# shenyunhang/APE

Measured on AMD Instinct MI355X. Metric: images/sec @1024^2 APE-L_D fwd, higher is better.
Workload: dtype bf16

## Files before the change

### ape_amd/_lib.py

```python
import ctypes
import os
from ctypes import POINTER, Structure, c_char_p, c_double, c_float, c_int, c_int32, c_int64, c_void_p

_HERE = os.path.dirname(os.path.abspath(__file__))
LIB_PATH = os.path.join(_HERE, "lib", "libape_hip.so")

DT_F32 = 0
DT_BF16 = 1
DT_F16 = 2
ACT_NONE, ACT_RELU, ACT_GELU, ACT_SWIGLU, ACT_SILU = 0, 1, 2, 3, 4
MASK_NONE, MASK_ZERO_INPUT, MASK_ZERO_OUTPUT = 0, 1, 2


class GemmArgs(Structure):
    _fields_ = [
        ("A", c_void_p), ("W", c_void_p), ("C", c_void_p), ("bias", c_void_p), ("residual", c_void_p),
        ("rowmask", c_void_p), ("rope_cos", c_void_p), ("rope_sin", c_void_p),
        ("M", c_int32), ("N", c_int32), ("K", c_int32),
        ("lda", c_int32), ("ldw", c_int32), ("ldc", c_int32), ("ldr", c_int32),
        ("in_dt", c_int32), ("out_dt", c_int32), ("res_dt", c_int32),
        ("act", c_int32), ("mask_mode", c_int32), ("trans_out", c_int32),
        ("rope_rows", c_int32), ("rope_hd", c_int32), ("rope_cols", c_int32), ("vec_ok", c_int32),
        ("alpha", c_float), ("clamp", c_float),
        ("splitk", c_int32), ("tile64", c_int32), ("workspace", c_void_p),
        ("rowscale", c_void_p), ("rowshift", c_void_p), ("colvec", c_void_p), ("rope_cs", c_void_p),
        ("ln_w", c_void_p), ("ln_b", c_void_p), ("ln_eps", c_float), ("reserved0", c_int32),
        ("conv_perm", c_void_p), ("conv_zero", c_void_p), ("conv_h", c_int32), ("conv_w", c_int32),
        ("rowstat_cols", c_int32), ("rowstat_eps", c_float),
    ]


class LayerNormArgs(Structure):
    _fields_ = [
        ("x", c_void_p), ("w", c_void_p), ("b", c_void_p), ("y", c_void_p), ("add", c_void_p), ("y2", c_void_p),
        ("M", c_int32), ("C", c_int32), ("Cpad", c_int32),
        ("ldx", c_int32), ("ldy", c_int32), ("ldadd", c_int32), ("ldy2", c_int32),
        ("x_dt", c_int32), ("y_dt", c_int32), ("add_dt", c_int32), ("act", c_int32), ("eps", c_float),
    ]


class GroupNormArgs(Structure):
    _fields_ = [
        ("x", c_void_p), ("w", c_void_p), ("b", c_void_p), ("y", c_void_p), ("add", c_void_p), ("workspace", c_void_p),
        ("HW", c_int32), ("C", c_int32), ("G", c_int32),
        ("ldx", c_int32), ("ldy", c_int32), ("ldadd", c_int32),
        ("x_dt", c_int32), ("y_dt", c_int32), ("add_dt", c_int32), ("act", c_int32), ("eps", c_float),
    ]


SIGNATURES = {
    "ape_hip_last_error": (c_char_p, []),
    "ape_hip_abi_version": (c_int, []),
    "ape_hip_sizeof_args": (c_int, [c_int]),
    "ape_hip_gemm": (c_int, [POINTER(GemmArgs), c_void_p]),
    "ape_hip_gemm_last_kernel": (c_char_p, []),
    "ape_hip_meter_begin": (c_int, []),
    "ape_hip_meter_count": (c_int, []),
    "ape_hip_meter_end": (c_int, []),
    "ape_hip_meter_read": (c_int, [c_int, POINTER(c_char_p), POINTER(c_float)]),
    "ape_hip_zero": (c_int, [c_void_p, ctypes.c_size_t, c_void_p]),
    "ape_hip_stuff_collapse": (c_int, [c_void_p, c_int, c_int, c_int, c_int, c_void_p, c_int, c_void_p]),
    "ape_hip_sem_class_weights": (c_int, [c_void_p, c_int, c_void_p, c_void_p, c_int, c_int, c_int, c_float, c_void_p, c_int, c_int, c_void_p]),
    "ape_hip_pan_class_scores": (c_int, [c_void_p, c_int, c_void_p, c_void_p, c_int, c_int, c_float, c_int, c_float, c_void_p, c_void_p,
                                         c_void_p, c_void_p, c_void_p]),
    "ape_hip_argmax_labels": (c_int, [c_void_p, ctypes.c_size_t, c_int, ctypes.c_size_t, c_float, c_void_p, c_void_p]),
    "ape_hip_sdma_usable": (c_int, [c_void_p, c_void_p]),
    "ape_hip_sdma_d2h": (c_int, [c_void_p, c_void_p, ctypes.c_size_t]),
    "ape_hip_sdma_d2h_multi": (c_int, [c_int, ctypes.POINTER(c_void_p), ctypes.POINTER(c_void_p), ctypes.POINTER(ctypes.c_size_t), c_int]),
    "ape_hip_sdma_engines": (c_int, [c_void_p, c_void_p]),
    "ape_hip_row_stats": (c_int, [c_void_p, c_int, c_int, c_int, c_int, c_float, c_void_p, c_void_p, c_void_p]),
    "ape_hip_gemv": (c_int, [c_void_p, c_int, c_void_p, c_int, c_int, c_void_p, c_void_p, c_int, c_int, c_int, c_int,
                             c_float, c_void_p]),
    "ape_hip_gemv_affine": (c_int, [c_void_p, c_int, c_void_p, c_int, c_int, c_void_p, c_void_p, c_int, c_int, c_int, c_int,
                                    c_float, c_void_p, c_void_p, c_int, c_void_p, c_int, c_void_p]),
    "ape_hip_layernorm": (c_int, [POINTER(LayerNormArgs), c_void_p]),
    "ape_hip_postnorm_residual": (c_int, [c_void_p, c_int, c_int, c_void_p, c_void_p, c_float, c_void_p, c_int, c_void_p, c_int, c_int,
                                          c_int, c_int, c_void_p]),
    "ape_hip_groupnorm_workspace_floats": (c_int, [c_int, c_int]),
    "ape_hip_groupnorm": (c_int, [POINTER(GroupNormArgs), c_void_p]),
    "ape_hip_ms_deform_attn_forward": (c_int, [c_void_p, c_int, POINTER(c_int64), POINTER(c_int64), c_void_p, c_void_p,
                                               c_void_p, c_int, c_int, c_int, c_int, c_int, c_int, c_void_p]),
    "ape_hip_msda_fused": (c_int, [c_void_p, c_int, c_int, POINTER(c_int64), POINTER(c_int64), c_void_p, c_int, c_void_p,
                                   c_int, c_void_p, c_int, c_int, c_int, c_int, c_int, c_int, c_void_p]),
    "ape_hip_msda_fused_h": (c_int, [c_void_p, c_int, c_int, POINTER(c_int64), POINTER(c_int64), c_void_p, c_int, c_void_p,
                                     c_int, c_void_p, c_int, c_int, c_int, c_int, c_int, c_int, c_void_p]),
    "ape_hip_attention": (c_int, [c_void_p, c_int, c_void_p, c_int, c_void_p, c_int, c_void_p, c_int, c_int, c_int, c_int,
                                  c_int, c_float, c_int, c_void_p]),
    "ape_hip_geometry": (c_int, [c_int, c_int, c_int, c_int, POINTER(c_int), c_void_p, c_int, c_void_p, c_float, c_float, c_float,
                                 c_void_p, c_int, c_void_p, c_void_p, c_void_p, c_void_p, c_void_p, c_void_p, c_void_p, c_void_p,
                                 c_void_p]),
    "ape_hip_head_gemv": (c_int, [c_void_p, c_int, c_void_p, c_void_p, c_void_p, c_int, c_int, c_int, c_int, c_float, c_void_p, c_int,
                                  c_int, c_void_p]),
    "ape_hip_attention_strided": (c_int, [c_void_p, c_int, c_void_p, c_int, c_void_p, c_int, c_void_p, c_int, c_int, c_int, c_int,
                                          c_int, c_int, c_float, c_int, c_void_p]),
    "ape_hip_attention_causal": (c_int, [c_void_p, c_int, c_void_p, c_int, c_void_p, c_int, c_void_p, c_int, c_int, c_int, c_int,
                                         c_int, c_int, c_float, c_int, c_void_p]),
    "ape_hip_embed_tokens": (c_int, [c_void_p, c_int, c_void_p, c_int, c_void_p, c_int, c_int, c_void_p, c_int, c_int, c_int, c_int,
                                     c_int, c_int, c_void_p]),
    "ape_hip_patchify": (c_int, [c_void_p, c_int, c_int, c_void_p, c_int, c_int, POINTER(c_float), POINTER(c_float), c_void_p,
                                 c_int, c_int, c_void_p]),
    "ape_hip_im2col3x3": (c_int, [c_void_p, c_int, c_void_p, c_int, c_int, c_int, c_void_p, c_int, c_int, c_void_p]),
    "ape_hip_maxpool2x2": (c_int, [c_void_p, c_int, c_void_p, c_int, c_int, c_int, c_void_p, c_int, c_int, c_void_p]),
    "ape_hip_gather_rows": (c_int, [c_void_p, c_int, c_void_p, c_int, c_int, c_void_p, c_int, c_int, c_void_p]),
    "ape_hip_gather_rows_i64": (c_int, [c_void_p, c_int, c_void_p, c_int, c_int, c_void_p, c_int, c_int, c_void_p]),
    "ape_hip_nms_mask_words": (c_int, [c_int]),
    "ape_hip_nms_mask": (c_int, [c_void_p, c_void_p, c_int, c_float, c_void_p, c_void_p]),
    "ape_hip_nms_scan_segments": (c_int, [c_void_p, c_int, c_void_p, c_int, c_int, c_void_p, c_void_p, c_void_p]),
    "ape_hip_nms_scan_classes": (c_int, [c_void_p, c_int, c_void_p, c_int, c_void_p, c_void_p, c_void_p]),
    "ape_hip_vl_pool_workspace_floats": (c_int, [c_int, c_int]),
    "ape_hip_vl_pool": (c_int, [c_void_p, c_int, c_void_p, c_int, c_int, c_int, c_int, c_void_p, c_void_p, c_void_p, c_void_p]),
    "ape_hip_segment_softmax": (c_int, [c_void_p, c_int, c_int, c_int, c_int, c_void_p, c_void_p, c_int, c_int, c_void_p]),
    "ape_hip_colstats_workspace_floats": (c_int, [c_int, c_int]),
    "ape_hip_colstats": (c_int, [c_void_p, c_int, c_int, c_int, c_void_p, c_void_p, c_void_p, c_void_p, c_void_p]),
    "ape_hip_transpose": (c_int, [c_void_p, c_int, c_int, c_int, c_int, c_void_p, c_void_p, c_void_p, c_void_p, c_int, c_int,
                                  c_void_p]),
    "ape_hip_mask_upsample_bits": (c_int, [c_void_p, c_int, c_int, c_int, c_int, c_int, c_int, c_void_p, c_void_p]),
    "ape_hip_roi_align_bits": (c_int, [c_void_p, c_int, c_int, c_void_p, c_int, c_int, c_void_p, c_void_p]),
    "ape_hip_paste_bits": (c_int, [c_void_p, c_int, c_void_p, c_int, c_int, c_int, c_void_p, c_void_p]),
    "ape_hip_mask_upsample_sigmoid": (c_int, [c_void_p, c_int, c_int, c_int, c_int, c_int, c_int, c_int, c_int, c_void_p, c_int, c_int,
                                              c_void_p]),
    "ape_hip_box_refine": (c_int, [c_void_p, c_int, c_void_p, c_void_p, c_int, c_int, c_float, c_void_p, c_void_p, c_void_p]),
    "ape_hip_det_records": (c_int, [c_void_p, c_void_p, c_void_p, c_void_p, c_void_p, c_int, c_void_p, c_void_p, c_void_p, c_void_p]),
    "ape_hip_query_init": (c_int, [c_void_p, c_void_p, c_int, c_void_p, c_int, c_float, c_int, c_void_p, c_void_p, c_int, c_int, c_void_p,
                                   c_void_p]),
    "ape_hip_query_finish": (c_int, [c_void_p, c_int, c_void_p, c_int, c_int, c_int, c_void_p, c_void_p, c_float, c_void_p, c_void_p,
                                     c_float, c_void_p, c_void_p, c_void_p, c_int, c_int, c_void_p]),
    "ape_hip_bilinear_resize": (c_int, [c_void_p, c_int, c_int, c_int, c_int, c_int, c_void_p, c_int, c_int, c_void_p]),
    "ape_hip_panoptic_pixels": (c_int, [c_void_p, c_int, c_int, c_int, c_int, c_int, c_void_p, c_void_p, c_float, c_int, c_int, c_void_p, c_void_p,
                                        c_void_p, c_void_p]),
    "ape_hip_panoptic_decide": (c_int, [c_void_p, c_void_p, c_void_p, c_int, c_void_p, c_int, c_double, c_int, c_void_p, c_void_p, c_void_p, c_void_p]),
    "ape_hip_panoptic_write": (c_int, [c_void_p, c_void_p, c_void_p, c_int, c_int, c_void_p, c_void_p]),
    "ape_hip_enc_finalize": (c_int, [c_void_p, c_void_p, c_void_p, c_int, c_void_p, c_void_p, c_void_p, c_void_p]),
    "ape_hip_topk_workspace_words": (c_int, [c_int]),
    "ape_hip_proposal_topk": (c_int, [c_void_p, c_int, POINTER(c_int), POINTER(c_int), c_int, c_int, c_int, c_void_p, c_void_p, c_void_p,
                                      c_void_p]),
    "ape_hip_proposal_order": (c_int, [c_void_p, c_int, c_void_p, c_void_p, POINTER(c_int), POINTER(c_int), c_int, c_void_p, c_void_p,
                                       c_void_p, c_void_p, c_void_p, c_void_p, c_void_p]),
    "ape_hip_proposal_quota": (c_int, [c_void_p, c_void_p, c_void_p, c_void_p, c_int, c_void_p, c_int, POINTER(c_int), POINTER(c_int),
                                       c_int, c_int, c_void_p, c_void_p]),
    "ape_hip_det_sort": (c_int, [c_void_p, c_int, c_int, c_int, c_void_p, c_void_p, c_float, c_void_p, c_void_p, c_void_p, c_void_p,
                                 c_void_p, c_void_p]),
    "ape_hip_det_topk": (c_int, [c_void_p, c_void_p, c_void_p, c_void_p, c_int, c_int, c_int, c_void_p, c_void_p, c_void_p, c_void_p,
                                 c_void_p, c_void_p]),
    "ape_hip_ffn_fused": (c_int, [c_void_p, c_int, c_void_p, c_int, c_void_p, c_void_p, c_int, c_void_p, c_void_p, c_int, c_void_p, c_int,
                                  c_int, c_int, c_int, c_int, c_int, c_int, c_void_p, c_void_p, c_float, c_void_p]),
    "ape_hip_attention_ext": (c_int, [c_void_p, c_int, c_void_p, c_int, c_void_p, c_int, c_void_p, c_int, c_int, c_int, c_int, c_int, c_int,
                                      c_int, c_float, c_int, c_void_p]),
    "ape_hip_relpos_extend": (c_int, [c_void_p, c_void_p, c_int, c_void_p, c_int, c_int, c_void_p, c_void_p, c_int, c_void_p, c_void_p, c_int, c_int,
                                      c_int, c_int, c_int, c_int, c_int, c_int, c_float, c_int, c_void_p]),
    "ape_hip_resize_coeffs": (c_int, [c_int, c_int, c_void_p, c_void_p, c_int]),
    "ape_hip_resize_tile_rows": (c_int, [c_void_p, c_int, POINTER(c_int)]),
    "ape_hip_resize_bilinear_u8": (c_int, [c_void_p, c_int, c_int, c_int, c_void_p, c_void_p, c_int, c_void_p, c_void_p, c_int,
                                           c_int, c_int, c_int, c_int, c_void_p, c_int, c_int, c_int, c_int, c_void_p]),
    "ape_hip_rle_workspace_words": (c_int, [c_int, c_int, c_int, c_int]),
    "ape_hip_rle_encode": (c_int, [c_void_p, c_int, c_int, c_int, c_void_p, c_void_p, c_int, c_void_p, c_void_p]),
    "ape_hip_rle_to_string": (c_int, [c_void_p, c_int, c_void_p, c_int]),
}

_lib = None


def load():
    global _lib
    if _lib is not None:
        return _lib
    if not os.path.exists(LIB_PATH):
        raise RuntimeError(
            f"{LIB_PATH} not found: the HIP extension is not built (run `python -m ape_amd.build` or "
            "__graft_entry__.build()).  ape_amd has no CPU/PyTorch fallback."
        )
    lib = ctypes.CDLL(LIB_PATH)
    for name, (res, args) in SIGNATURES.items():
        fn = getattr(lib, name)
        fn.restype = res
        fn.argtypes = args
    _lib = lib
    return lib


def check(rc, what):
    if rc != 0:
        msg = load().ape_hip_last_error()
        raise RuntimeError(f"{what} failed (rc={rc}): {msg.decode() if msg else '?'}")
```

### ape_amd/csrc/boxes.hip

```cpp
#include "common.h"
#include "../../include/ape_hip.h"

__global__ __launch_bounds__(256) void box_refine_kernel(const float* __restrict__ delta, int ldd, const float* __restrict__ ref,
                                                         const float* __restrict__ vr4, int L, int Q, float eps,
                                                         float* __restrict__ new_ref, float* __restrict__ ref_in) {
  const int gid = blockIdx.x * 256 + threadIdx.x;
  if (gid >= Q * 4) return;
  const int q = gid >> 2, c = gid & 3;
  float x = ref[gid];
  x = fminf(fmaxf(x, 0.f), 1.f);
  const float x1 = fmaxf(x, eps), x2 = fmaxf(1.f - x, eps);
  float z = logf(x1 / x2);
  if (delta != nullptr) z += delta[(size_t)q * ldd + c];
  const float r = delta != nullptr ? 1.f / (1.f + expf(-z)) : ref[gid];
  if (new_ref != nullptr) new_ref[gid] = r;
  if (ref_in != nullptr)
    for (int l = 0; l < L; ++l) ref_in[((size_t)q * L + l) * 4 + c] = r * vr4[l * 4 + c];
}

extern "C" int ape_hip_box_refine(const float* delta, int ldd, const float* ref, const float* vr4, int L, int Q, float eps,
                                  float* new_ref, float* ref_in, void* stream) {
  APE_CHECK_ARG(ref && Q > 0 && (ref_in == nullptr || (vr4 != nullptr && L > 0)) && (new_ref || ref_in),
                "ape_hip_box_refine: bad args");
  APE_LAUNCH(box_refine_kernel, dim3(ceil_div(Q * 4, 256)), dim3(256), 0, (hipStream_t)stream, delta, ldd, ref, vr4, L, Q, eps,
                     new_ref, ref_in);
  APE_CHECK_LAUNCH("ape_hip_box_refine");
  return 0;
}

template <typename T> __device__ __forceinline__ float round_to(float v);
template <> __device__ __forceinline__ float round_to<float>(float v) { return v; }
template <> __device__ __forceinline__ float round_to<bf16_t>(float v) { return bf2f(f2bf(v)); }
template <> __device__ __forceinline__ float round_to<f16_t>(float v) { return (float)(f16_t)sat_h(v); }

template <typename TO>
__global__ __launch_bounds__(256) void query_init_kernel(const float* __restrict__ coords, const int64_t* __restrict__ topk, int T,
                                                         const float* __restrict__ dim_t, int P, float scale, int Q,
                                                         float* __restrict__ reference, TO* __restrict__ pe, int ldpe,
                                                         int32_t* __restrict__ topk32) {
  const int q = blockIdx.x;
  int64_t t = topk[q];
  t = t < 0 ? 0 : (t >= T ? T - 1 : t);
  if (threadIdx.x == 0 && topk32 != nullptr) topk32[q] = (int32_t)t;
  for (int j = threadIdx.x; j < 4 * P; j += 256) {
    const int c = j / P, i = j % P;
    const float x = coords[(size_t)t * 4 + c];
    const float s = 1.f / (1.f + expf(-x));
    if (i == 0) reference[q * 4 + c] = s;
    const float v = (s * scale) / dim_t[i];
    stf<TO>(pe + (size_t)q * ldpe + j, (i & 1) ? cosf(v) : sinf(v));
  }
}

extern "C" int ape_hip_query_init(const float* coords, const int64_t* topk, int T, const float* dim_t, int P, float scale, int Q,
                                  float* reference, void* pe, int ldpe, int pe_dt, int32_t* topk32, void* stream) {
  APE_CHECK_ARG(coords && topk && dim_t && reference && pe && T > 0 && P > 0 && Q > 0 && ldpe >= 4 * P, "ape_hip_query_init: bad args");
  hipStream_t s = (hipStream_t)stream;
  if (pe_dt == APE_DT_F16) APE_LAUNCH(query_init_kernel<f16_t>, dim3(Q), dim3(256), 0, s, coords, topk, T, dim_t, P, scale, Q, reference, (f16_t*)pe, ldpe, topk32);
  else if (pe_dt == APE_DT_BF16) APE_LAUNCH(query_init_kernel<bf16_t>, dim3(Q), dim3(256), 0, s, coords, topk, T, dim_t, P, scale, Q, reference, (bf16_t*)pe, ldpe, topk32);
  else if (pe_dt == APE_DT_F32)
    APE_LAUNCH(query_init_kernel<float>, dim3(Q), dim3(256), 0, s, coords, topk, T, dim_t, P, scale, Q, reference, (float*)pe, ldpe, topk32);
  else
    APE_CHECK_ARG(false, "ape_hip_query_init: pe must be f32, bf16 or f16");
  APE_CHECK_LAUNCH("ape_hip_query_init");
  return 0;
}

template <typename TO>
__global__ __launch_bounds__(256) void query_finish_kernel(const float* __restrict__ pos, int ldpos, const float* __restrict__ pix,
                                                           int ldpix, int Q, int E, const float* __restrict__ wpos,
                                                           const float* __restrict__ bpos, float eps_pos,
                                                           const float* __restrict__ wpix, const float* __restrict__ bpix,
                                                           float eps_pix, TO* __restrict__ query_pos, TO* __restrict__ query,
                                                           TO* __restrict__ query_sum, int ldo) {
  const int lane = threadIdx.x & 63;
  const int q = blockIdx.x * 4 + (threadIdx.x >> 6);
  if (q >= Q) return;
  constexpr int MAXP = 16, MAXX = 8;
  float vp[MAXP], vx[MAXX];
  const float* pr = pos + (size_t)q * ldpos;
  const float* xr = pix + (size_t)q * ldpix;
  float sp = 0.f, sx = 0.f;
#pragma unroll
  for (int k = 0; k < MAXP; ++k) { const int c = lane + 64 * k; vp[k] = c < 2 * E ? pr[c] : 0.f; sp += vp[k]; }
#pragma unroll
  for (int k = 0; k < MAXX; ++k) { const int c = lane + 64 * k; vx[k] = c < E ? xr[c] : 0.f; sx += vx[k]; }
  const float mp = wave_sum(sp) / (float)(2 * E), mx = wave_sum(sx) / (float)E;
  float qp = 0.f, qx = 0.f;
#pragma unroll
  for (int k = 0; k < MAXP; ++k) { const int c = lane + 64 * k; const float d = c < 2 * E ? vp[k] - mp : 0.f; qp += d * d; }
#pragma unroll
  for (int k = 0; k < MAXX; ++k) { const int c = lane + 64 * k; const float d = c < E ? vx[k] - mx : 0.f; qx += d * d; }
  const float rp = rsqrtf(wave_sum(qp) / (float)(2 * E) + eps_pos), rx = rsqrtf(wave_sum(qx) / (float)E + eps_pix);
  const int kE = E / 64;
#pragma unroll
  for (int k = 0; k < MAXX; ++k) {
    const int c = lane + 64 * k;
    if (c < E) {
      const float a = (vp[k] - mp) * rp * wpos[c] + bpos[c];
      float hi = 0.f;
#pragma unroll
      for (int kk = 0; kk < MAXP; ++kk) if (kk == k + kE) hi = (vp[kk] - mp) * rp * wpos[E + c] + bpos[E + c];
      const float b = hi + ((vx[k] - mx) * rx * wpix[c] + bpix[c]);
      const float ar = round_to<TO>(a), br = round_to<TO>(b);
      stf<TO>(query_pos + (size_t)q * ldo + c, ar);
      stf<TO>(query + (size_t)q * ldo + c, br);
      stf<TO>(query_sum + (size_t)q * ldo + c, ar + br);
    }
  }
}

extern "C" int ape_hip_query_finish(const float* pos, int ldpos, const float* pix, int ldpix, int Q, int E, const float* wpos,
                                    const float* bpos, float eps_pos, const float* wpix, const float* bpix, float eps_pix,
                                    void* query_pos, void* query, void* query_sum, int ldo, int out_dt, void* stream) {
  APE_CHECK_ARG(pos && pix && wpos && bpos && wpix && bpix && query_pos && query && query_sum && Q > 0, "ape_hip_query_finish: bad args");
  APE_CHECK_ARG(E > 0 && E <= 512 && E % 64 == 0 && ldpos >= 2 * E && ldpix >= E && ldo >= E, "ape_hip_query_finish: E must be a multiple of 64, <= 512");
  hipStream_t s = (hipStream_t)stream;
  const dim3 grid(ceil_div(Q, 4)), block(256);
  if (out_dt == APE_DT_F16) APE_LAUNCH(query_finish_kernel<f16_t>, grid, block, 0, s, pos, ldpos, pix, ldpix, Q, E, wpos, bpos, eps_pos, wpix, bpix, eps_pix,
                       (f16_t*)query_pos, (f16_t*)query, (f16_t*)query_sum, ldo);
  else if (out_dt == APE_DT_BF16) APE_LAUNCH(query_finish_kernel<bf16_t>, grid, block, 0, s, pos, ldpos, pix, ldpix, Q, E, wpos, bpos, eps_pos, wpix, bpix, eps_pix,
                       (bf16_t*)query_pos, (bf16_t*)query, (bf16_t*)query_sum, ldo);
  else if (out_dt == APE_DT_F32)
    APE_LAUNCH(query_finish_kernel<float>, grid, block, 0, s, pos, ldpos, pix, ldpix, Q, E, wpos, bpos, eps_pos, wpix, bpix, eps_pix,
                       (float*)query_pos, (float*)query, (float*)query_sum, ldo);
  else
    APE_CHECK_ARG(false, "ape_hip_query_finish: outputs must be f32, bf16 or f16");
  APE_CHECK_LAUNCH("ape_hip_query_finish");
  return 0;
}

__global__ __launch_bounds__(1024) void det_records_kernel(const float* __restrict__ boxes, const float* __restrict__ scores,
                                                            const int64_t* __restrict__ classes, const int64_t* __restrict__ query,
                                                            const float* __restrict__ frame, int k, float* __restrict__ rec,
                                                            float* __restrict__ boxes_out, int32_t* __restrict__ order) {
  __shared__ int wtot[16];
  __shared__ int total_keep;
  const int tid = threadIdx.x, lane = tid & 63, wave = tid >> 6;
  float f[8];
#pragma unroll
  for (int i = 0; i < 8; ++i) f[i] = frame[i];
  int cnt = 0;
  for (int i = tid; i < k; i += 1024) {
    float b[4];
#pragma unroll
    for (int c = 0; c < 4; ++c) b[c] = fminf(fmaxf(boxes[i * 4 + c] * f[c], 0.f), f[4 + c]);
    cnt += (scores[i] >= 0.f && (b[2] - b[0]) > 0.f && (b[3] - b[1]) > 0.f) ? 1 : 0;
  }
  cnt = (int)wave_sum((float)cnt);
  if (lane == 0) wtot[wave] = cnt;
  __syncthreads();
  if (tid == 0) { int s = 0; for (int w = 0; w < 16; ++w) s += wtot[w]; total_keep = s; }
  __syncthreads();
  int kbase = 0, dbase = total_keep;
  for (int i0 = 0; i0 < k; i0 += 1024) {
    const int i = i0 + tid;
    const bool in = i < k;
    float b[4] = {0.f, 0.f, 0.f, 0.f};
    bool keep = false;
    float sc = -1.f;
    if (in) {
#pragma unroll
      for (int c = 0; c < 4; ++c) b[c] = fminf(fmaxf(boxes[i * 4 + c] * f[c], 0.f), f[4 + c]);
      sc = scores[i];
      keep = sc >= 0.f && (b[2] - b[0]) > 0.f && (b[3] - b[1]) > 0.f;
    }
    const unsigned long long m = __ballot(keep);
    const int before = __popcll(m & ((1ull << lane) - 1ull));
    __syncthreads();
    if (lane == 0) wtot[wave] = __popcll(m);
    __syncthreads();
    int wbase = 0, chunk_keep = 0;
    for (int w = 0; w < 16; ++w) { const int t = wtot[w]; if (w < wave) wbase += t; chunk_keep += t; }
    if (in) {
      const int kept_before = wbase + before;
      const int pos = keep ? kbase + kept_before : dbase + (tid - kept_before);
      float* r = rec + (size_t)pos * 8;
      r[0] = b[0]; r[1] = b[1]; r[2] = b[2]; r[3] = b[3];
      r[4] = keep ? sc : -1.f;
      r[5] = (float)classes[i];
      r[6] = (float)query[i];
      r[7] = keep ? 1.f : 0.f;
      float* bo = boxes_out + (size_t)pos * 4;
      bo[0] = b[0]; bo[1] = b[1]; bo[2] = b[2]; bo[3] = b[3];
      order[pos] = i;
    }
    const int nin = min(1024, k - i0);
    kbase += chunk_keep;
    dbase += nin - chunk_keep;
  }
}

extern "C" int ape_hip_det_records(const float* boxes, const float* scores, const int64_t* classes, const int64_t* query,
                                   const float* frame, int k, float* rec, float* boxes_out, int32_t* order, void* stream) {
  APE_CHECK_ARG(boxes && scores && classes && query && frame && rec && boxes_out && order && k > 0, "ape_hip_det_records: bad args");
  APE_LAUNCH(det_records_kernel, dim3(1), dim3(1024), 0, (hipStream_t)stream, boxes, scores, classes, query, frame, k, rec,
                     boxes_out, order);
  APE_CHECK_LAUNCH("ape_hip_det_records");
  return 0;
}
```

### ape_amd/csrc/common.h

```cpp
#pragma once
#include <hip/hip_runtime.h>
#include <stdint.h>
#include <stdio.h>
#include <string.h>

typedef uint16_t bf16_t;

typedef __attribute__((ext_vector_type(8))) __bf16 bf16x8_t;
typedef __attribute__((ext_vector_type(8))) short short8_t;
typedef __attribute__((ext_vector_type(4))) float f32x4_t;

#define APE_DT_F32 0
#define APE_DT_BF16 1
#define APE_DT_F16 2
typedef _Float16 f16_t;

__device__ __forceinline__ float bf2f(bf16_t v) { return __uint_as_float(((uint32_t)v) << 16); }
typedef __attribute__((ext_vector_type(2))) float f32x2_t;
typedef __attribute__((ext_vector_type(2))) __bf16 bf16x2_t;
__device__ __forceinline__ uint32_t pack2bf(float a, float b) {
  const f32x2_t v = {a, b};
  return __builtin_bit_cast(uint32_t, __builtin_convertvector(v, bf16x2_t));
}
__device__ __forceinline__ bf16_t f2bf(float f) { return (bf16_t)(pack2bf(f, 0.f) & 0xffffu); }

template <typename T> __device__ __forceinline__ float ldf(const T* p);
template <> __device__ __forceinline__ float ldf<float>(const float* p) { return *p; }
template <> __device__ __forceinline__ float ldf<bf16_t>(const bf16_t* p) { return bf2f(*p); }
template <typename T> __device__ __forceinline__ void stf(T* p, float v);
template <> __device__ __forceinline__ void stf<float>(float* p, float v) { *p = v; }
template <> __device__ __forceinline__ void stf<bf16_t>(bf16_t* p, float v) { *p = f2bf(v); }

template <> __device__ __forceinline__ float ldf<f16_t>(const f16_t* p) { return (float)*p; }
#define APE_HALF_MAX 65504.f
__device__ __forceinline__ float sat_h(float v) { return __builtin_amdgcn_fmed3f(v, -APE_HALF_MAX, APE_HALF_MAX); }
template <> __device__ __forceinline__ void stf<f16_t>(f16_t* p, float v) { *p = (f16_t)sat_h(v); }

template <typename T> __device__ __forceinline__ void ld4(const T* p, float v[4]);
template <> __device__ __forceinline__ void ld4<float>(const float* p, float v[4]) {
  float4 t = *reinterpret_cast<const float4*>(p); v[0] = t.x; v[1] = t.y; v[2] = t.z; v[3] = t.w;
}
template <> __device__ __forceinline__ void ld4<bf16_t>(const bf16_t* p, float v[4]) {
  uint2 t = *reinterpret_cast<const uint2*>(p);
  v[0] = __uint_as_float(t.x << 16); v[1] = __uint_as_float(t.x & 0xffff0000u);
  v[2] = __uint_as_float(t.y << 16); v[3] = __uint_as_float(t.y & 0xffff0000u);
}
template <typename T> __device__ __forceinline__ void st4(T* p, const float v[4]);
template <> __device__ __forceinline__ void st4<float>(float* p, const float v[4]) {
  *reinterpret_cast<float4*>(p) = make_float4(v[0], v[1], v[2], v[3]);
}
template <> __device__ __forceinline__ void st4<bf16_t>(bf16_t* p, const float v[4]) {
  *reinterpret_cast<uint2*>(p) = make_uint2(pack2bf(v[0], v[1]), pack2bf(v[2], v[3]));
}
template <typename T> __device__ __forceinline__ void ld8(const T* p, float v[8]);
template <> __device__ __forceinline__ void ld8<float>(const float* p, float v[8]) {
  ld4<float>(p, v); ld4<float>(p + 4, v + 4);
}
template <> __device__ __forceinline__ void ld8<bf16_t>(const bf16_t* p, float v[8]) {
  uint4 t = *reinterpret_cast<const uint4*>(p);
  v[0] = __uint_as_float(t.x << 16); v[1] = __uint_as_float(t.x & 0xffff0000u);
  v[2] = __uint_as_float(t.y << 16); v[3] = __uint_as_float(t.y & 0xffff0000u);
  v[4] = __uint_as_float(t.z << 16); v[5] = __uint_as_float(t.z & 0xffff0000u);
  v[6] = __uint_as_float(t.w << 16); v[7] = __uint_as_float(t.w & 0xffff0000u);
}
typedef __attribute__((ext_vector_type(8))) _Float16 f16x8_t;
template <> __device__ __forceinline__ void ld8<f16_t>(const f16_t* p, float v[8]) {
  const f16x8_t t = *reinterpret_cast<const f16x8_t*>(p);
#pragma unroll
  for (int i = 0; i < 8; ++i) v[i] = (float)t[i];
}
template <typename T> __device__ __forceinline__ void st8(T* p, const float v[8]);
template <> __device__ __forceinline__ void st8<float>(float* p, const float v[8]) {
  st4<float>(p, v); st4<float>(p + 4, v + 4);
}
template <> __device__ __forceinline__ void st8<bf16_t>(bf16_t* p, const float v[8]) {
  *reinterpret_cast<uint4*>(p) = make_uint4(pack2bf(v[0], v[1]), pack2bf(v[2], v[3]),
                                            pack2bf(v[4], v[5]), pack2bf(v[6], v[7]));
}

typedef __attribute__((ext_vector_type(2))) _Float16 f16x2_t;
__device__ __forceinline__ uint32_t pack2h(float a, float b) {
  const f32x2_t v = {sat_h(a), sat_h(b)};
  return __builtin_bit_cast(uint32_t, __builtin_convertvector(v, f16x2_t));
}
template <> __device__ __forceinline__ void ld4<f16_t>(const f16_t* p, float v[4]) {
  const uint2 t = *reinterpret_cast<const uint2*>(p);
  const f16x2_t a = __builtin_bit_cast(f16x2_t, t.x), b = __builtin_bit_cast(f16x2_t, t.y);
  v[0] = (float)a[0]; v[1] = (float)a[1]; v[2] = (float)b[0]; v[3] = (float)b[1];
}
template <> __device__ __forceinline__ void st4<f16_t>(f16_t* p, const float v[4]) {
  *reinterpret_cast<uint2*>(p) = make_uint2(pack2h(v[0], v[1]), pack2h(v[2], v[3]));
}
template <> __device__ __forceinline__ void st8<f16_t>(f16_t* p, const float v[8]) {
  *reinterpret_cast<uint4*>(p) = make_uint4(pack2h(v[0], v[1]), pack2h(v[2], v[3]), pack2h(v[4], v[5]), pack2h(v[6], v[7]));
}

template <typename H> struct h16;
template <> struct h16<bf16_t> {
  static constexpr int dt = APE_DT_BF16;
  static __device__ __forceinline__ uint32_t pack2(float a, float b) { return pack2bf(a, b); }
  static __device__ __forceinline__ f32x4_t mfma(bf16x8_t a, bf16x8_t b, f32x4_t c) {
    return __builtin_amdgcn_mfma_f32_16x16x32_bf16(a, b, c, 0, 0, 0);
  }
};
template <> struct h16<f16_t> {
  static constexpr int dt = APE_DT_F16;
  static __device__ __forceinline__ uint32_t pack2(float a, float b) { return pack2h(a, b); }
  static __device__ __forceinline__ f32x4_t mfma(bf16x8_t a, bf16x8_t b, f32x4_t c) {
    return __builtin_amdgcn_mfma_f32_16x16x32_f16(__builtin_bit_cast(f16x8_t, a), __builtin_bit_cast(f16x8_t, b), c, 0, 0, 0);
  }
};
template <typename H> __device__ __forceinline__ float dot2acc(uint32_t a, uint32_t b, float c);
typedef __attribute__((ext_vector_type(2))) __bf16 bf16x2_t;
template <> __device__ __forceinline__ float dot2acc<bf16_t>(uint32_t a, uint32_t b, float c) {
  return __builtin_amdgcn_fdot2_f32_bf16(__builtin_bit_cast(bf16x2_t, a), __builtin_bit_cast(bf16x2_t, b), c, false);
}
template <> __device__ __forceinline__ float dot2acc<f16_t>(uint32_t a, uint32_t b, float c) {
  return __builtin_amdgcn_fdot2(__builtin_bit_cast(f16x2_t, a), __builtin_bit_cast(f16x2_t, b), c, false);
}
template <typename H> __device__ __forceinline__ void dot2acc_pinned(float& acc, uint32_t a, uint32_t b);
template <> __device__ __forceinline__ void dot2acc_pinned<bf16_t>(float& acc, uint32_t a, uint32_t b) {
  asm volatile("v_dot2c_f32_bf16 %0, %1, %2" : "+v"(acc) : "v"(a), "v"(b));
}
template <> __device__ __forceinline__ void dot2acc_pinned<f16_t>(float& acc, uint32_t a, uint32_t b) {
  asm volatile("v_dot2c_f32_f16 %0, %1, %2" : "+v"(acc) : "v"(a), "v"(b));
}
template <typename H> struct ones2;
template <> struct ones2<bf16_t> { static constexpr uint32_t v = 0x3f803f80u; };
template <> struct ones2<f16_t> { static constexpr uint32_t v = 0x3c003c00u; };
template <typename H> __device__ __forceinline__ void unpack2(uint32_t u, float& a, float& b);
template <> __device__ __forceinline__ void unpack2<bf16_t>(uint32_t u, float& a, float& b) {
  a = __uint_as_float(u << 16); b = __uint_as_float(u & 0xffff0000u);
}
template <> __device__ __forceinline__ void unpack2<f16_t>(uint32_t u, float& a, float& b) {
  const f16x2_t t = __builtin_bit_cast(f16x2_t, u);
  a = (float)t[0]; b = (float)t[1];
}

__device__ __forceinline__ float wave_sum(float v) {
#pragma unroll
  for (int o = 32; o > 0; o >>= 1) v += __shfl_xor(v, o, 64);
  return v;
}
__device__ __forceinline__ float wave_max(float v) {
#pragma unroll
  for (int o = 32; o > 0; o >>= 1) v = fmaxf(v, __shfl_xor(v, o, 64));
  return v;
}

extern "C" const char* ape_hip_last_error(void);
void ape_set_error(const char* fmt, ...);

#include <hip/hip_ext.h>
hipEvent_t* ape_meter_pair(const char* kernel, hipStream_t stream);
#define APE_LAUNCH(KERNEL, GRID, BLOCK, LDS, STREAM, ...)                                                                  \
  do {                                                                                                                     \
    hipEvent_t* ev__ = ape_meter_pair(#KERNEL, STREAM);                                                                           \
    if (ev__ != nullptr) hipExtLaunchKernelGGL(KERNEL, GRID, BLOCK, LDS, STREAM, ev__[0], ev__[1], 0, __VA_ARGS__);        \
    else hipLaunchKernelGGL(KERNEL, GRID, BLOCK, LDS, STREAM, __VA_ARGS__);                                                \
  } while (0)

#define APE_CHECK_ARG(cond, ...)            \
  do {                                      \
    if (!(cond)) {                          \
      ape_set_error(__VA_ARGS__);           \
      return -1;                            \
    }                                       \
  } while (0)
#define APE_CHECK_LAUNCH(name)                                                    \
  do {                                                                            \
    hipError_t e__ = hipGetLastError();                                           \
    if (e__ != hipSuccess) {                                                      \
      ape_set_error("%s: launch failed: %s", name, hipGetErrorString(e__));       \
      return -2;                                                                  \
    }                                                                             \
  } while (0)

static inline int ceil_div(int a, int b) { return (a + b - 1) / b; }
constexpr int APE_MAX_DEVICES = 64;
static inline int ape_current_device() {
  int d = 0;
  if (hipGetDevice(&d) != hipSuccess || d < 0 || d >= APE_MAX_DEVICES) d = 0;
  return d;
}
struct ApeOncePerDevice {
  bool done[APE_MAX_DEVICES] = {};
  bool first() { const int d = ape_current_device(); const bool f = !done[d]; done[d] = true; return f; }
};
static inline int ape_cu_count() {
  static int n[APE_MAX_DEVICES] = {};
  const int d = ape_current_device();
  if (n[d] == 0) {
    int c = 0;
    if (hipDeviceGetAttribute(&c, hipDeviceAttributeMultiprocessorCount, d) != hipSuccess || c < 8) c = 256;
    n[d] = c & ~7;
  }
  return n[d];
}
static inline bool ape_is16(int dt) { return dt == APE_DT_BF16 || dt == APE_DT_F16; }
static inline int ape_h16_kind(const int* dts, int n) {
  int k = 0;
  for (int i = 0; i < n; ++i) {
    const int d = dts[i];
    if (d == APE_DT_F32) continue;
    if (!ape_is16(d)) return -1;
    if (k != 0 && k != d) return -1;
    k = d;
  }
  return k;
}
#define APE_H16_KIND(...) ([&]() { const int d__[] = {__VA_ARGS__}; return ape_h16_kind(d__, (int)(sizeof(d__) / sizeof(int))); }())
```

### ape_amd/csrc/msda.hip

```cpp
#include <type_traits>

#include "common.h"
#include "../../include/ape_hip.h"

#define MS_HEADS 8
#define MS_D 32
#define MS_P 4

struct MsdaParams {
  const void* value; int ldv;
  const void* loc;
  const void* attn;
  const void* offw; int ldoffw;
  int offw_f16;
  const float* ref; int refdim;
  void* out; int ldout;
  int S, Q;
  int H[8], W[8], start[8];
  float invW[8], invH[8];
  int pow2;
};

template <typename TV>
__device__ __forceinline__ void corner_acc(const TV* __restrict__ vbase, int ldv, int idx, float wgt, float acc[8]) {
  float v[8];
  ld8<TV>(vbase + (size_t)idx * ldv, v);
#pragma unroll
  for (int c = 0; c < 8; ++c) acc[c] = fmaf(wgt, v[c], acc[c]);
}

template <typename TV>
__device__ __forceinline__ void sample_acc(const TV* __restrict__ vlvl, int ldv, int H, int W, float lx, float ly,
                                           float aw, float acc[8]) {
  const float h_im = ly * (float)H - 0.5f;
  const float w_im = lx * (float)W - 0.5f;
  if (!(h_im > -1.f && w_im > -1.f && h_im < (float)H && w_im < (float)W)) return;
  const float hf = floorf(h_im), wf = floorf(w_im);
  const int h_low = (int)hf, w_low = (int)wf;
  const int h_high = h_low + 1, w_high = w_low + 1;
  const float lh = h_im - hf, lw = w_im - wf;
  const float hh = 1.f - lh, hw = 1.f - lw;
  if (h_low >= 0 && w_low >= 0) corner_acc<TV>(vlvl, ldv, h_low * W + w_low, aw * hh * hw, acc);
  if (h_low >= 0 && w_high <= W - 1) corner_acc<TV>(vlvl, ldv, h_low * W + w_high, aw * hh * lw, acc);
  if (h_high <= H - 1 && w_low >= 0) corner_acc<TV>(vlvl, ldv, h_high * W + w_low, aw * lh * hw, acc);
  if (h_high <= H - 1 && w_high <= W - 1) corner_acc<TV>(vlvl, ldv, h_high * W + w_high, aw * lh * lw, acc);
}

template <typename TV, typename TO, int L, bool FUSED>
__global__ __launch_bounds__(256) void msda_kernel(const MsdaParams p) {
  const int lane = threadIdx.x & 63;
  const int wave = threadIdx.x >> 6;
  int chunk;
  {
    const int nblk = gridDim.x, b = blockIdx.x;
    const int q = nblk >> 3, r = nblk & 7;
    const int xcd = b & 7, j = b >> 3;
    chunk = (xcd < r ? xcd * (q + 1) : r * (q + 1) + (xcd - r) * q) + j;
  }
  const int batch = blockIdx.y;
  const int g = lane >> 2, sub = lane & 3;
  const int qi = chunk * 8 + wave * 2 + (g >> 3);
  const int h = g & 7;
  if (qi >= p.Q) return;
  const size_t qg = (size_t)batch * p.Q + qi;
  const TV* vb = reinterpret_cast<const TV*>(p.value) + (size_t)batch * p.S * p.ldv + h * MS_D + sub * 8;

  float acc[8];
#pragma unroll
  for (int c = 0; c < 8; ++c) acc[c] = 0.f;

  constexpr int LP = L * MS_P;
  if (FUSED) {
    const float* lg = reinterpret_cast<const float*>(p.offw) + qg * p.ldoffw + MS_HEADS * LP * 2 + h * LP;
    float w[LP];
    float mx = -INFINITY;
#pragma unroll
    for (int s = 0; s < LP; s += 4) {
      const float4 t = *reinterpret_cast<const float4*>(lg + s);
      w[s] = t.x; w[s + 1] = t.y; w[s + 2] = t.z; w[s + 3] = t.w;
      mx = fmaxf(mx, fmaxf(fmaxf(t.x, t.y), fmaxf(t.z, t.w)));
    }
    float sum = 0.f;
#pragma unroll
    for (int s = 0; s < LP; ++s) { w[s] = expf(w[s] - mx); sum += w[s]; }
    const float inv = 1.f / sum;
    const float* of = reinterpret_cast<const float*>(p.offw) + qg * p.ldoffw + h * LP * 2;
    const float* rf = p.ref + qg * L * p.refdim;
#pragma unroll
    for (int l = 0; l < L; ++l) {
      const int H = p.H[l], W = p.W[l];
      const TV* vl = vb + (size_t)p.start[l] * p.ldv;
      const float4 o01 = *reinterpret_cast<const float4*>(of + l * 8);
      const float4 o23 = *reinterpret_cast<const float4*>(of + l * 8 + 4);
      const float ox[4] = {o01.x, o01.z, o23.x, o23.z};
      const float oy[4] = {o01.y, o01.w, o23.y, o23.w};
      const float rx = rf[l * p.refdim], ry = rf[l * p.refdim + 1];
      float sx, sy;
      if (p.refdim == 2) {
        sx = 1.f / (float)W; sy = 1.f / (float)H;
#pragma unroll
        for (int pt = 0; pt < MS_P; ++pt)
          sample_acc<TV>(vl, p.ldv, H, W, rx + ox[pt] / (float)W, ry + oy[pt] / (float)H, w[l * MS_P + pt] * inv, acc);
        (void)sx; (void)sy;
      } else {
        const float rw = rf[l * p.refdim + 2], rh = rf[l * p.refdim + 3];
#pragma unroll
        for (int pt = 0; pt < MS_P; ++pt)
          sample_acc<TV>(vl, p.ldv, H, W, rx + ox[pt] / (float)MS_P * rw * 0.5f, ry + oy[pt] / (float)MS_P * rh * 0.5f,
                         w[l * MS_P + pt] * inv, acc);
      }
    }
  } else {
    const TV* loc = reinterpret_cast<const TV*>(p.loc) + (qg * MS_HEADS + h) * LP * 2;
    const TV* aw = reinterpret_cast<const TV*>(p.attn) + (qg * MS_HEADS + h) * LP;
#pragma unroll
    for (int l = 0; l < L; ++l) {
      const int H = p.H[l], W = p.W[l];
      const TV* vl = vb + (size_t)p.start[l] * p.ldv;
#pragma unroll
      for (int pt = 0; pt < MS_P; ++pt) {
        const float lx = ldf<TV>(loc + (l * MS_P + pt) * 2), ly = ldf<TV>(loc + (l * MS_P + pt) * 2 + 1);
        sample_acc<TV>(vl, p.ldv, H, W, lx, ly, ldf<TV>(aw + l * MS_P + pt), acc);
      }
    }
  }
  TO* o = reinterpret_cast<TO*>(p.out) + qg * p.ldout + h * MS_D + sub * 8;
  st8<TO>(o, acc);
}

template <int P> __device__ __forceinline__ float quad_bcast_f(float v) {
  return __int_as_float(__builtin_amdgcn_mov_dpp(__float_as_int(v), P * 0x55, 0xf, 0xf, true));
}
template <int P> __device__ __forceinline__ int quad_bcast_i(int v) { return __builtin_amdgcn_mov_dpp(v, P * 0x55, 0xf, 0xf, true); }
__device__ __forceinline__ float quad_xor1(float v) { return __int_as_float(__builtin_amdgcn_mov_dpp(__float_as_int(v), 0xB1, 0xf, 0xf, true)); }
__device__ __forceinline__ float quad_xor2(float v) { return __int_as_float(__builtin_amdgcn_mov_dpp(__float_as_int(v), 0x4E, 0xf, 0xf, true)); }

__device__ __forceinline__ float quad_pick_f(int P, float v) {
  return P == 0 ? quad_bcast_f<0>(v) : (P == 1 ? quad_bcast_f<1>(v) : (P == 2 ? quad_bcast_f<2>(v) : quad_bcast_f<3>(v)));
}
__device__ __forceinline__ int quad_pick_i(int P, int v) {
  return P == 0 ? quad_bcast_i<0>(v) : (P == 1 ? quad_bcast_i<1>(v) : (P == 2 ? quad_bcast_i<2>(v) : quad_bcast_i<3>(v)));
}

template <typename TV>
struct CornerGroup {
  uint4 raw[4];
  float w[4];
};

template <typename TV, int L>
__device__ __forceinline__ void group_load(const unsigned char* __restrict__ vbase, uint32_t lane_off, const float (&cw)[L][4],
                                           const int (&ci)[L][4], int s, CornerGroup<TV>& g) {
  const int l = s >> 2, P = s & 3;
#pragma unroll
  for (int c = 0; c < 4; ++c) {
    g.w[c] = quad_pick_f(P, cw[l][c]);
    uint32_t off = (uint32_t)quad_pick_i(P, ci[l][c]) + lane_off;
    asm volatile("" : "+v"(off));
    g.raw[c] = *reinterpret_cast<const uint4*>(vbase + (size_t)off);
  }
}

__device__ __forceinline__ void fma_mix_lo(float& acc, uint32_t d, float w) {
  asm volatile("v_fma_mix_f32 %0, %1, %2, %0 op_sel:[0,0,0] op_sel_hi:[1,0,0]" : "+v"(acc) : "v"(d), "v"(w));
}
__device__ __forceinline__ void fma_mix_hi(float& acc, uint32_t d, float w) {
  asm volatile("v_fma_mix_f32 %0, %1, %2, %0 op_sel:[1,0,0] op_sel_hi:[1,0,0]" : "+v"(acc) : "v"(d), "v"(w));
}
template <typename TV>
__device__ __forceinline__ void group_fma_half(const CornerGroup<TV>& g, float (&acc)[8]) {
#pragma unroll
  for (int c = 0; c < 4; ++c) {
    const uint32_t d[4] = {g.raw[c].x, g.raw[c].y, g.raw[c].z, g.raw[c].w};
#pragma unroll
    for (int e = 0; e < 4; ++e) {
      fma_mix_lo(acc[2 * e], d[e], g.w[c]);
      fma_mix_hi(acc[2 * e + 1], d[e], g.w[c]);
    }
  }
}

template <typename TV>
__device__ __forceinline__ void group_fma(const CornerGroup<TV>& g, f32x2_t (&a2)[4]) {
#pragma unroll
  for (int c = 0; c < 4; ++c) {
    const f32x2_t ww = {g.w[c], g.w[c]};
    const uint32_t d[4] = {g.raw[c].x, g.raw[c].y, g.raw[c].z, g.raw[c].w};
#pragma unroll
    for (int e = 0; e < 4; ++e) {
      const f32x2_t v2 = {__uint_as_float(d[e] << 16), __uint_as_float(d[e] & 0xffff0000u)};
      a2[e] = __builtin_elementwise_fma(ww, v2, a2[e]);
    }
  }
#pragma unroll
  for (int e = 0; e < 4; ++e) asm volatile("" : "+v"(a2[e]));
}

template <typename TV, typename TO, int L, typename TW = float>
__global__ __launch_bounds__(256) __attribute__((amdgpu_waves_per_eu(4, 8))) void msda_fused_quad_kernel(const MsdaParams p) {
  const int lane = threadIdx.x & 63;
  const int wave = threadIdx.x >> 6;
  int chunk;
  {
    const int nblk = gridDim.x, b = blockIdx.x;
    const int q = nblk >> 3, r = nblk & 7;
    const int xcd = b & 7, j = b >> 3;
    chunk = (xcd < r ? xcd * (q + 1) : r * (q + 1) + (xcd - r) * q) + j;
  }
  const int batch = blockIdx.y;
  const int g = lane >> 2, sub = lane & 3;
  int qi = chunk * 8 + wave * 2 + (g >> 3);
  const bool live = qi < p.Q;
  qi = live ? qi : p.Q - 1;
  const int h = g & 7;
  const size_t qg = (size_t)batch * p.Q + qi;
  const TV* vb = reinterpret_cast<const TV*>(p.value) + (size_t)batch * p.S * p.ldv + h * MS_D + sub * 8;
  const unsigned char* vbase = reinterpret_cast<const unsigned char*>(reinterpret_cast<const TV*>(p.value) + (size_t)batch * p.S * p.ldv);
  const uint32_t lane_off = (uint32_t)((h * MS_D + sub * 8) * sizeof(TV));
  const uint32_t rowb = (uint32_t)(p.ldv * (int)sizeof(TV));
  constexpr int LP = L * MS_P;

  const TW* lg = reinterpret_cast<const TW*>(p.offw) + qg * p.ldoffw + MS_HEADS * LP * 2 + h * LP;
  float wv[L];
  float mx = -INFINITY;
#pragma unroll
  for (int l = 0; l < L; ++l) { wv[l] = ldf<TW>(lg + l * MS_P + sub); mx = fmaxf(mx, wv[l]); }
  mx = fmaxf(mx, quad_xor1(mx));
  mx = fmaxf(mx, quad_xor2(mx));
  float sum = 0.f;
#pragma unroll
  for (int l = 0; l < L; ++l) { wv[l] = expf(wv[l] - mx); sum += wv[l]; }
  sum += quad_xor1(sum);
  sum += quad_xor2(sum);
  const float inv = 1.f / sum;
  const TW* of = reinterpret_cast<const TW*>(p.offw) + qg * p.ldoffw + h * LP * 2 + sub * 2;
  const float* rf = p.ref + qg * L * p.refdim;
  float cw[L][4];
  int ci[L][4];
#pragma unroll
  for (int l = 0; l < L; ++l) {
    const int H = p.H[l], W = p.W[l];
    float2 o;
    if (sizeof(TW) == 4) {
      o = *reinterpret_cast<const float2*>(of + l * 8);
    } else {
      typedef __attribute__((ext_vector_type(2))) _Float16 h2_t;
      const h2_t t = *reinterpret_cast<const h2_t*>(of + l * 8);
      o = make_float2((float)t[0], (float)t[1]);
    }
    const float rx = rf[l * p.refdim], ry = rf[l * p.refdim + 1];
    float lx, ly;
    if (p.refdim == 2) {
      if (p.pow2) { lx = rx + o.x * p.invW[l]; ly = ry + o.y * p.invH[l]; }
      else { lx = rx + o.x / (float)W; ly = ry + o.y / (float)H; }
    } else {
      const float rw = rf[l * p.refdim + 2], rh = rf[l * p.refdim + 3];
      lx = rx + o.x / (float)MS_P * rw * 0.5f; ly = ry + o.y / (float)MS_P * rh * 0.5f;
    }
    const float aw = wv[l] * inv;
    const float h_im = ly * (float)H - 0.5f, w_im = lx * (float)W - 0.5f;
    const bool inside = h_im > -1.f && w_im > -1.f && h_im < (float)H && w_im < (float)W;
    const float hf = floorf(h_im), wf = floorf(w_im);
    const int h_low = (int)hf, w_low = (int)wf;
    const int h_high = h_low + 1, w_high = w_low + 1;
    const float lh = h_im - hf, lw = w_im - wf;
    const float hh = 1.f - lh, hw = 1.f - lw;
    const bool t_ok = inside && h_low >= 0, b_ok = inside && h_high <= H - 1;
    const bool l_ok = w_low >= 0, r_ok = w_high <= W - 1;
    const int base = p.start[l];
    cw[l][0] = (t_ok && l_ok) ? aw * hh * hw : 0.f; ci[l][0] = (t_ok && l_ok) ? base + h_low * W + w_low : 0;
    cw[l][1] = (t_ok && r_ok) ? aw * hh * lw : 0.f; ci[l][1] = (t_ok && r_ok) ? base + h_low * W + w_high : 0;
    cw[l][2] = (b_ok && l_ok) ? aw * lh * hw : 0.f; ci[l][2] = (b_ok && l_ok) ? base + h_high * W + w_low : 0;
    cw[l][3] = (b_ok && r_ok) ? aw * lh * lw : 0.f; ci[l][3] = (b_ok && r_ok) ? base + h_high * W + w_high : 0;
    if (sizeof(TV) == 2) {
#pragma unroll
      for (int c = 0; c < 4; ++c) ci[l][c] = (int)__umul24((unsigned)ci[l][c], rowb);
    }
  }
  float acc[8];
  if (std::is_same<TV, f16_t>::value) {
#pragma unroll
    for (int c = 0; c < 8; ++c) acc[c] = 0.f;
    CornerGroup<TV> g0, g1;
    group_load<TV, L>(vbase, lane_off, cw, ci, 0, g0);
#pragma unroll
    for (int s = 0; s < L * 4; s += 2) {
      group_load<TV, L>(vbase, lane_off, cw, ci, s + 1, g1);
      __builtin_amdgcn_sched_barrier(0);
      group_fma_half<TV>(g0, acc);
      __builtin_amdgcn_sched_barrier(0);
      if (s + 2 < L * 4) group_load<TV, L>(vbase, lane_off, cw, ci, s + 2, g0);
      __builtin_amdgcn_sched_barrier(0);
      group_fma_half<TV>(g1, acc);
      __builtin_amdgcn_sched_barrier(0);
    }
  } else if (sizeof(TV) == 2) {
    f32x2_t a2[4];
#pragma unroll
    for (int e = 0; e < 4; ++e) a2[e] = (f32x2_t){0.f, 0.f};
    CornerGroup<TV> g0, g1;
    group_load<TV, L>(vbase, lane_off, cw, ci, 0, g0);
#pragma unroll
    for (int s = 0; s < L * 4; s += 2) {
      group_load<TV, L>(vbase, lane_off, cw, ci, s + 1, g1);
      __builtin_amdgcn_sched_barrier(0);
      group_fma<TV>(g0, a2);
      __builtin_amdgcn_sched_barrier(0);
      if (s + 2 < L * 4) group_load<TV, L>(vbase, lane_off, cw, ci, s + 2, g0);
      __builtin_amdgcn_sched_barrier(0);
      group_fma<TV>(g1, a2);
      __builtin_amdgcn_sched_barrier(0);
    }
#pragma unroll
    for (int e = 0; e < 4; ++e) { acc[2 * e] = a2[e][0]; acc[2 * e + 1] = a2[e][1]; }
  } else {
#pragma unroll
    for (int c = 0; c < 8; ++c) acc[c] = 0.f;
#pragma unroll
    for (int s = 0; s < L * 4; ++s) {
      const int l = s >> 2, P = s & 3;
#pragma unroll
      for (int c = 0; c < 4; ++c) {
        const float w = quad_pick_f(P, cw[l][c]);
        const int idx = quad_pick_i(P, ci[l][c]);
        if (w != 0.f) corner_acc<TV>(vb, p.ldv, idx, w, acc);
      }
    }
  }
  if (live) {
    TO* o = reinterpret_cast<TO*>(p.out) + qg * p.ldout + h * MS_D + sub * 8;
    st8<TO>(o, acc);
  }
}

constexpr int ML_T = 16;
constexpr int ML_HALO = 6;
constexpr int ML_RMAX = ML_T + 2 * ML_HALO + 2;
constexpr int ML_ROWS = ML_RMAX * ML_RMAX;

template <typename TO, typename TW, int L>
__global__ __launch_bounds__(256) void msda_lds_kernel(const MsdaParams p) {
  __shared__ uint4 sV[ML_ROWS * 4];
  const int t = threadIdx.x;
  const int h = blockIdx.x & 7;
  const int tile = blockIdx.x >> 3;
  const int batch = blockIdx.y;
  const int W0 = p.W[0];
  const int tiles_x = W0 / ML_T;
  const int ty = tile / tiles_x, tx = tile - ty * tiles_x;
  const int qi = p.start[0] + (ty * ML_T + (t >> 4)) * W0 + tx * ML_T + (t & 15);
  const size_t qg = (size_t)batch * p.Q + qi;
  const size_t q_first = (size_t)batch * p.Q + p.start[0] + (size_t)(ty * ML_T) * W0 + tx * ML_T;
  const size_t q_last = q_first + (size_t)(ML_T - 1) * W0 + (ML_T - 1);
  const uint32_t rowb = (uint32_t)p.ldv * 2u;
  const unsigned char* vhead = reinterpret_cast<const unsigned char*>(p.value) + (size_t)batch * p.S * rowb + h * (MS_D * 2);
  constexpr int LP = L * MS_P;

  float e[LP];
  {
    const TW* lg = reinterpret_cast<const TW*>(p.offw) + qg * p.ldoffw + MS_HEADS * LP * 2 + h * LP;
    float mx = -INFINITY;
#pragma unroll
    for (int i = 0; i < LP; ++i) { e[i] = ldf<TW>(lg + i); mx = fmaxf(mx, e[i]); }
    float sum = 0.f;
#pragma unroll
    for (int i = 0; i < LP; ++i) { e[i] = expf(e[i] - mx); sum += e[i]; }
    const float inv = 1.f / sum;
#pragma unroll
    for (int i = 0; i < LP; ++i) e[i] *= inv;
  }
  float acc[32];
#pragma unroll
  for (int c = 0; c < 32; ++c) acc[c] = 0.f;
  const TW* of = reinterpret_cast<const TW*>(p.offw) + qg * p.ldoffw + h * LP * 2;
  const float* rf = p.ref + qg * L * 2;
  const float* rfa = p.ref + q_first * L * 2;
  const float* rfb = p.ref + q_last * L * 2;

#pragma unroll 1
  for (int l = 0; l < L; ++l) {
    const int H = p.H[l], W = p.W[l];
    const float ax = rfa[l * 2] * (float)W - 0.5f, ay = rfa[l * 2 + 1] * (float)H - 0.5f;
    const float bx = rfb[l * 2] * (float)W - 0.5f, by = rfb[l * 2 + 1] * (float)H - 0.5f;
    int x_lo = max(0, (int)floorf(fminf(ax, bx)) - ML_HALO), x_hi = min(W - 1, (int)floorf(fmaxf(ax, bx)) + ML_HALO + 1);
    int y_lo = max(0, (int)floorf(fminf(ay, by)) - ML_HALO), y_hi = min(H - 1, (int)floorf(fmaxf(ay, by)) + ML_HALO + 1);
    x_lo = __builtin_amdgcn_readfirstlane(x_lo); x_hi = __builtin_amdgcn_readfirstlane(x_hi);
    y_lo = __builtin_amdgcn_readfirstlane(y_lo); y_hi = __builtin_amdgcn_readfirstlane(y_hi);
    const int rw = max(0, min(ML_RMAX, x_hi - x_lo + 1)), rh = max(0, min(ML_RMAX, y_hi - y_lo + 1));
    const unsigned char* vl = vhead + (size_t)p.start[l] * rowb;
    if (l > 0) __syncthreads();
    {
      const int n = rw * rh * 4;
      if (n == 0 && t < 4) sV[t] = make_uint4(0u, 0u, 0u, 0u);
      const float inv_rw = 1.f / (float)max(rw, 1);
      for (int i0 = 0; i0 < n; i0 += 1024) {
        uint4 v[4];
        int ii[4];
#pragma unroll
        for (int u = 0; u < 4; ++u) {
          const int i = i0 + u * 256 + t;
          ii[u] = i;
          if (i < n) {
            const int r = i >> 2, sl = i & 3;
            const int ry = (int)(((float)r + 0.5f) * inv_rw);
            const int rx = r - ry * rw;
            v[u] = *reinterpret_cast<const uint4*>(vl + (size_t)((y_lo + ry) * W + x_lo + rx) * rowb + ((sl ^ (rx & 3)) << 4));
          }
        }
#pragma unroll
        for (int u = 0; u < 4; ++u)
          if (ii[u] < n) sV[ii[u]] = v[u];
      }
    }
    __syncthreads();
    float off[8];
    if (sizeof(TW) == 4) {
      const float4 o0 = *reinterpret_cast<const float4*>(of + l * 8), o1 = *reinterpret_cast<const float4*>(of + l * 8 + 4);
      off[0] = o0.x; off[1] = o0.y; off[2] = o0.z; off[3] = o0.w; off[4] = o1.x; off[5] = o1.y; off[6] = o1.z; off[7] = o1.w;
    } else {
      typedef __attribute__((ext_vector_type(8))) _Float16 h8_t;
      const h8_t tq = *reinterpret_cast<const h8_t*>(of + l * 8);
#pragma unroll
      for (int u = 0; u < 8; ++u) off[u] = (float)tq[u];
    }
    const float rx0 = rf[l * 2], ry0 = rf[l * 2 + 1];
    float ew[MS_P];
#pragma unroll
    for (int pt = 0; pt < MS_P; ++pt) {
      ew[pt] = e[pt];
#pragma unroll
      for (int ll = 1; ll < L; ++ll) ew[pt] = (l == ll) ? e[ll * MS_P + pt] : ew[pt];
    }
#pragma unroll
    for (int pt = 0; pt < MS_P; ++pt) {
      float lx, ly;
      if (p.pow2) { lx = rx0 + off[2 * pt] * p.invW[l]; ly = ry0 + off[2 * pt + 1] * p.invH[l]; }
      else { lx = rx0 + off[2 * pt] / (float)W; ly = ry0 + off[2 * pt + 1] / (float)H; }
      const float aw = ew[pt];
      const float h_im = ly * (float)H - 0.5f, w_im = lx * (float)W - 0.5f;
      const bool inside = h_im > -1.f && w_im > -1.f && h_im < (float)H && w_im < (float)W;
      const float hf = floorf(h_im), wf = floorf(w_im);
      const int h_low = (int)hf, w_low = (int)wf;
      const float lh = h_im - hf, lw = w_im - wf;
      const float hh = 1.f - lh, hw = 1.f - lw;
#pragma unroll
      for (int c = 0; c < 4; ++c) {
        const int cy = h_low + (c >> 1), cx = w_low + (c & 1);
        const bool ok = inside && cy >= 0 && cy <= H - 1 && cx >= 0 && cx <= W - 1;
        const float wgt = ok ? aw * ((c >> 1) ? lh : hh) * ((c & 1) ? lw : hw) : 0.f;
        const int ry = cy - y_lo, rx = cx - x_lo;
        const bool staged = ok && ry >= 0 && ry < rh && rx >= 0 && rx < rw;
        const int row = staged ? ry * rw + rx : 0;
        const float wl = staged ? wgt : 0.f;
        const int sw = rx & 3;
#pragma unroll
        for (int k = 0; k < 4; ++k) {
          const uint4 d = sV[row * 4 + (k ^ sw)];
          fma_mix_lo(acc[8 * k + 0], d.x, wl); fma_mix_hi(acc[8 * k + 1], d.x, wl);
          fma_mix_lo(acc[8 * k + 2], d.y, wl); fma_mix_hi(acc[8 * k + 3], d.y, wl);
          fma_mix_lo(acc[8 * k + 4], d.z, wl); fma_mix_hi(acc[8 * k + 5], d.z, wl);
          fma_mix_lo(acc[8 * k + 6], d.w, wl); fma_mix_hi(acc[8 * k + 7], d.w, wl);
        }
        if (ok && !staged) {
          const unsigned char* g = vl + (size_t)(cy * W + cx) * rowb;
#pragma unroll
          for (int k = 0; k < 4; ++k) {
            const uint4 d = *reinterpret_cast<const uint4*>(g + (k << 4));
            fma_mix_lo(acc[8 * k + 0], d.x, wgt); fma_mix_hi(acc[8 * k + 1], d.x, wgt);
            fma_mix_lo(acc[8 * k + 2], d.y, wgt); fma_mix_hi(acc[8 * k + 3], d.y, wgt);
            fma_mix_lo(acc[8 * k + 4], d.z, wgt); fma_mix_hi(acc[8 * k + 5], d.z, wgt);
            fma_mix_lo(acc[8 * k + 6], d.w, wgt); fma_mix_hi(acc[8 * k + 7], d.w, wgt);
          }
        }
      }
    }
  }
  TO* o = reinterpret_cast<TO*>(p.out) + qg * p.ldout + h * MS_D;
#pragma unroll
  for (int k = 0; k < 4; ++k) st8<TO>(o + 8 * k, acc + 8 * k);
}

template <typename TV, typename TO, bool FUSED>
static int launch_msda(const MsdaParams& p, int B, int L, hipStream_t s) {
  const dim3 grid(ceil_div(p.Q, 8), B), block(256);
  if constexpr (FUSED) {
    if (p.offw_f16) {
      switch (L) {
        case 1: APE_LAUNCH((msda_fused_quad_kernel<TV, TO, 1, f16_t>), grid, block, 0, s, p); return 0;
        case 2: APE_LAUNCH((msda_fused_quad_kernel<TV, TO, 2, f16_t>), grid, block, 0, s, p); return 0;
        case 3: APE_LAUNCH((msda_fused_quad_kernel<TV, TO, 3, f16_t>), grid, block, 0, s, p); return 0;
        case 4: APE_LAUNCH((msda_fused_quad_kernel<TV, TO, 4, f16_t>), grid, block, 0, s, p); return 0;
        case 5: APE_LAUNCH((msda_fused_quad_kernel<TV, TO, 5, f16_t>), grid, block, 0, s, p); return 0;
        default: ape_set_error("msda: num_levels %d not in 1..5", L); return -1;
      }
    }
    switch (L) {
      case 1: APE_LAUNCH((msda_fused_quad_kernel<TV, TO, 1>), grid, block, 0, s, p); return 0;
      case 2: APE_LAUNCH((msda_fused_quad_kernel<TV, TO, 2>), grid, block, 0, s, p); return 0;
      case 3: APE_LAUNCH((msda_fused_quad_kernel<TV, TO, 3>), grid, block, 0, s, p); return 0;
      case 4: APE_LAUNCH((msda_fused_quad_kernel<TV, TO, 4>), grid, block, 0, s, p); return 0;
      case 5: APE_LAUNCH((msda_fused_quad_kernel<TV, TO, 5>), grid, block, 0, s, p); return 0;
      default: ape_set_error("msda: num_levels %d not in 1..5", L); return -1;
    }
  } else {
  switch (L) {
    case 1: APE_LAUNCH((msda_kernel<TV, TO, 1, FUSED>), grid, block, 0, s, p); break;
    case 2: APE_LAUNCH((msda_kernel<TV, TO, 2, FUSED>), grid, block, 0, s, p); break;
    case 3: APE_LAUNCH((msda_kernel<TV, TO, 3, FUSED>), grid, block, 0, s, p); break;
    case 4: APE_LAUNCH((msda_kernel<TV, TO, 4, FUSED>), grid, block, 0, s, p); break;
    case 5: APE_LAUNCH((msda_kernel<TV, TO, 5, FUSED>), grid, block, 0, s, p); break;
    default: ape_set_error("msda: num_levels %d not in 1..5", L); return -1;
  }
  }
  return 0;
}

static int fill_levels(MsdaParams& p, const int64_t* shapes, const int64_t* starts, int L, int S) {
  if (L < 1 || L > 5) { ape_set_error("msda: num_levels %d not in 1..5", L); return -1; }
  int64_t tot = 0;
  for (int l = 0; l < L; ++l) {
    p.H[l] = (int)shapes[2 * l]; p.W[l] = (int)shapes[2 * l + 1]; p.start[l] = (int)starts[l];
    if (p.H[l] <= 0 || p.W[l] <= 0 || starts[l] != tot) { ape_set_error("msda: inconsistent level %d (h=%d w=%d start=%lld)", l, p.H[l], p.W[l], (long long)starts[l]); return -1; }
    tot += (int64_t)p.H[l] * p.W[l];
  }
  if (tot != S) { ape_set_error("msda: sum(h*w)=%lld != num_value=%d", (long long)tot, S); return -1; }
  return 0;
}

extern "C" int ape_hip_ms_deform_attn_forward(const void* value, int ldv, const int64_t* spatial_shapes,
                                              const int64_t* level_start_index, const void* sampling_loc,
                                              const void* attn_weight, void* out, int ldout, int B, int S, int Q, int L,
                                              int dt, void* stream) {
  APE_CHECK_ARG(value && spatial_shapes && level_start_index && sampling_loc && attn_weight && out, "ms_deform_attn_forward: null pointer");
  APE_CHECK_ARG(B > 0 && S > 0 && Q > 0, "ms_deform_attn_forward: bad sizes");
  APE_CHECK_ARG(ldv % 8 == 0 && ldout % 8 == 0 && ((uintptr_t)value) % 16 == 0 && ((uintptr_t)out) % 16 == 0,
                "ms_deform_attn_forward: value/out must be 16-byte aligned with ld %% 8 == 0");
  MsdaParams p;
  memset(&p, 0, sizeof(p));
  p.value = value; p.ldv = ldv; p.loc = sampling_loc; p.attn = attn_weight; p.out = out; p.ldout = ldout; p.S = S; p.Q = Q;
  if (fill_levels(p, spatial_shapes, level_start_index, L, S)) return -1;
  int rc;
  APE_CHECK_ARG(dt == APE_DT_F32 || dt == APE_DT_BF16 || dt == APE_DT_F16, "ms_deform_attn_forward: dtype code %d (0 = f32, 1 = bf16, 2 = f16)", dt);
  if (dt == APE_DT_BF16) rc = launch_msda<bf16_t, bf16_t, false>(p, B, L, (hipStream_t)stream);
  else if (dt == APE_DT_F16) rc = launch_msda<f16_t, f16_t, false>(p, B, L, (hipStream_t)stream);
  else rc = launch_msda<float, float, false>(p, B, L, (hipStream_t)stream);
  if (rc) return rc;
  APE_CHECK_LAUNCH("ape_hip_ms_deform_attn_forward");
  return 0;
}

static int msda_fused_launch(const void* value, int ldv, int v_dt, const int64_t* spatial_shapes, const int64_t* level_start_index,
                             const void* offw, int ldoffw, int offw_f16, const float* ref, int refdim, void* out, int ldout, int out_dt,
                             int B, int S, int Q, int L, void* stream) {
  APE_CHECK_ARG(value && spatial_shapes && level_start_index && offw && ref && out, "msda_fused: null pointer");
  APE_CHECK_ARG(refdim == 2 || refdim == 4, "msda_fused: reference points must have 2 or 4 coordinates, got %d", refdim);
  APE_CHECK_ARG(B > 0 && S > 0 && Q > 0, "msda_fused: bad sizes");
  APE_CHECK_ARG(ldv % 8 == 0 && ldout % 8 == 0 && ldoffw % 4 == 0 && ((uintptr_t)value) % 16 == 0 &&
                    ((uintptr_t)out) % 16 == 0 && ((uintptr_t)offw) % 16 == 0,
                "msda_fused: alignment (value/out 16 B, ld %% 8; offw 16 B, ld %% 4)");
  MsdaParams p;
  memset(&p, 0, sizeof(p));
  p.value = value; p.ldv = ldv; p.offw = offw; p.ldoffw = ldoffw; p.offw_f16 = offw_f16; p.ref = ref; p.refdim = refdim;
  p.out = out; p.ldout = ldout; p.S = S; p.Q = Q;
  if (fill_levels(p, spatial_shapes, level_start_index, L, S)) return -1;
  APE_CHECK_ARG(v_dt == APE_DT_F32 || ((uint64_t)S * (uint64_t)ldv * 2 < (1ull << 32) && S < (1 << 24) && ldv * 2 < (1 << 24)),
                "msda_fused: a batch element's value tensor must stay below 4 GiB (S = %d rows of %d elements)", S, ldv);
  p.pow2 = 1;
  for (int l = 0; l < L; ++l) {
    p.pow2 &= ((p.W[l] & (p.W[l] - 1)) == 0 && (p.H[l] & (p.H[l] - 1)) == 0) ? 1 : 0;
    p.invW[l] = 1.f / (float)p.W[l]; p.invH[l] = 1.f / (float)p.H[l];
  }
  int rc;
  hipStream_t s = (hipStream_t)stream;
  {
    const char* le = getenv("APE_MSDA_LDS");
    const int n0 = p.H[0] * p.W[0];
    if ((le != nullptr && atoi(le) == 1) && L == 5 && refdim == 2 && Q == S && v_dt == APE_DT_F16 && p.start[0] == 0 && p.W[0] % ML_T == 0 &&
        p.H[0] % ML_T == 0 && n0 < Q && (out_dt == APE_DT_BF16 || out_dt == APE_DT_F16)) {
      const dim3 grid((p.H[0] / ML_T) * (p.W[0] / ML_T) * 8, B), block(256);
      if (out_dt == APE_DT_BF16) {
        if (offw_f16) APE_LAUNCH((msda_lds_kernel<bf16_t, f16_t, 5>), grid, block, 0, s, p);
        else APE_LAUNCH((msda_lds_kernel<bf16_t, float, 5>), grid, block, 0, s, p);
      } else {
        if (offw_f16) APE_LAUNCH((msda_lds_kernel<f16_t, f16_t, 5>), grid, block, 0, s, p);
        else APE_LAUNCH((msda_lds_kernel<f16_t, float, 5>), grid, block, 0, s, p);
      }
      APE_CHECK_LAUNCH("ape_hip_msda_fused (LDS-staged level-0 queries)");
      APE_CHECK_ARG(B == 1, "msda_fused: the LDS-staged encoder path takes one batch element per call");
      MsdaParams r = p;
      r.Q = Q - n0;
      r.offw = reinterpret_cast<const unsigned char*>(offw) + (size_t)n0 * ldoffw * (offw_f16 ? 2 : 4);
      r.ref = ref + (size_t)n0 * L * refdim;
      r.out = reinterpret_cast<unsigned char*>(out) + (size_t)n0 * ldout * 2;
      if (out_dt == APE_DT_BF16) rc = launch_msda<f16_t, bf16_t, true>(r, B, L, s);
      else rc = launch_msda<f16_t, f16_t, true>(r, B, L, s);
      if (rc) return rc;
      APE_CHECK_LAUNCH("ape_hip_msda_fused");
      return 0;
    }
  }
  if (v_dt == APE_DT_BF16 && out_dt == APE_DT_BF16) rc = launch_msda<bf16_t, bf16_t, true>(p, B, L, s);
  else if (v_dt == APE_DT_BF16 && out_dt == APE_DT_F32) rc = launch_msda<bf16_t, float, true>(p, B, L, s);
  else if (v_dt == APE_DT_F16 && out_dt == APE_DT_BF16) rc = launch_msda<f16_t, bf16_t, true>(p, B, L, s);
  else if (v_dt == APE_DT_F16 && out_dt == APE_DT_F32) rc = launch_msda<f16_t, float, true>(p, B, L, s);
  else if (v_dt == APE_DT_F16 && out_dt == APE_DT_F16) rc = launch_msda<f16_t, f16_t, true>(p, B, L, s);
  else if (v_dt == APE_DT_F32 && out_dt == APE_DT_F32) rc = launch_msda<float, float, true>(p, B, L, s);
  else { ape_set_error("msda_fused: unsupported dtype combination v=%d out=%d", v_dt, out_dt); return -1; }
  if (rc) return rc;
  APE_CHECK_LAUNCH("ape_hip_msda_fused");
  return 0;
}

extern "C" int ape_hip_msda_fused(const void* value, int ldv, int v_dt, const int64_t* spatial_shapes,
                                  const int64_t* level_start_index, const float* offw, int ldoffw, const float* ref,
                                  int refdim, void* out, int ldout, int out_dt, int B, int S, int Q, int L, void* stream) {
  return msda_fused_launch(value, ldv, v_dt, spatial_shapes, level_start_index, offw, ldoffw, 0, ref, refdim, out, ldout, out_dt, B, S, Q, L,
                           stream);
}

extern "C" int ape_hip_msda_fused_h(const void* value, int ldv, int v_dt, const int64_t* spatial_shapes,
                                    const int64_t* level_start_index, const void* offw_f16, int ldoffw, const float* ref,
                                    int refdim, void* out, int ldout, int out_dt, int B, int S, int Q, int L, void* stream) {
  APE_CHECK_ARG(v_dt == APE_DT_BF16 || v_dt == APE_DT_F16, "msda_fused_h: bf16 or f16 values (the production modes)");
  return msda_fused_launch(value, ldv, v_dt, spatial_shapes, level_start_index, offw_f16, ldoffw, 1, ref, refdim, out, ldout, out_dt, B, S, Q,
                           L, stream);
}
```

### ape_amd/modeling/ape_deta/_containers.py

```python
import os

import torch
import torch.nn as nn

from ... import ops
from ...packing import attach_cache, f32, pack_matrix, permute_ffn_w2


class FFN(nn.Module):
    def __init__(self, embed_dim=256, feedforward_dim=1024, output_dim=None, num_fcs=2, ffn_drop=0.0, **kwargs):
        super().__init__()
        assert num_fcs == 2
        output_dim = embed_dim if output_dim is None else output_dim
        self.layers = nn.Sequential(nn.Sequential(nn.Linear(embed_dim, feedforward_dim), nn.ReLU(inplace=True), nn.Dropout(ffn_drop)),
                                    nn.Linear(feedforward_dim, output_dim), nn.Dropout(ffn_drop))
        self.embed_dim = embed_dim
        attach_cache(self)

    def packed(self, dt):
        def build(dt):
            l0, l1 = self.layers[0][0], self.layers[1]
            d = dict(w1=pack_matrix(l0.weight, dt), b1=f32(l0.bias), w2=pack_matrix(l1.weight, dt), b2=f32(l1.bias))
            if dt in ops.HALF16 and l0.weight.shape[0] % 64 == 0:
                d["w2p"] = permute_ffn_w2(d["w2"])
            return d
        return self._pack.get(self, dt, build)

    FUSED_MIN_ROWS = 2048

    def forward_tokens(self, x, dt, out_dtype=None, norm=None):
        P = self.packed(dt)
        mode = os.environ.get("APE_FFN_FUSED", "1")
        if (mode != "0" and "w2p" in P and (out_dtype or dt) in ops.HALF16 and (out_dtype or dt) == dt and x.shape[0] >= self.FUSED_MIN_ROWS
                and x.shape[1] == 256 and P["w2"].shape[0] == 256 and P["w1"].shape[0] <= 4096):
            fuse_ln = norm if os.environ.get("APE_FFN_LN") != "0" else None
            if mode == "b64":
                y = ops.ffn_fused(x, P["w1"], P["b1"], P["w2"], P["b2"], residual=x, norm=fuse_ln)
            else:
                y = ops.ffn_fused(x, P["w1"], P["b1"], P["w2p"], P["b2"], residual=x, w2_permuted=True, norm=fuse_ln)
            return y if (norm is None or fuse_ln is not None) else ops.layernorm(y, norm[0], norm[1], norm[2], out_dtype=dt)
        h = ops.gemm(x, P["w1"], P["b1"], act=ops.ACT_RELU)
        y = ops.gemm(h, P["w2"], P["b2"], residual=x, out_dtype=out_dtype or dt)
        return y if norm is None else ops.layernorm(y, norm[0], norm[1], norm[2], out_dtype=dt)


class MLP(nn.Module):
    def __init__(self, input_dim, hidden_dim, output_dim, num_layers):
        super().__init__()
        self.num_layers = num_layers
        h = [hidden_dim] * (num_layers - 1)
        self.layers = nn.ModuleList(nn.Linear(n, k) for n, k in zip([input_dim] + h, h + [output_dim]))
        attach_cache(self)

    def packed(self, dt):
        def build(dt):
            return [(pack_matrix(l.weight, dt), f32(l.bias)) for l in self.layers]
        return self._pack.get(self, dt, build)

    def forward_tokens(self, x, dt, out_dtype=torch.float32):
        P = self.packed(dt)
        for i, (w, b) in enumerate(P):
            last = i == len(P) - 1
            x = ops.gemm(x, w, b, act=ops.ACT_NONE if last else ops.ACT_RELU, out_dtype=out_dtype if last else dt)
        return x


class SelfAttention(nn.Module):

    def __init__(self, embed_dim, num_heads, attn_drop=0.0, proj_drop=0.0, batch_first=False, **kwargs):
        super().__init__()
        self.embed_dim, self.num_heads, self.batch_first = embed_dim, num_heads, batch_first
        self.attn = nn.MultiheadAttention(embed_dim=embed_dim, num_heads=num_heads, dropout=attn_drop, batch_first=batch_first)
        self.proj_drop = nn.Dropout(proj_drop)
        attach_cache(self)

    def packed(self, dt):
        def build(dt):
            E = self.embed_dim
            w, b = self.attn.in_proj_weight, self.attn.in_proj_bias
            return dict(wqk=pack_matrix(w[:2 * E], dt), bqk=f32(b[:2 * E]), wv=pack_matrix(w[2 * E:], dt), bv=f32(b[2 * E:]),
                        wo=pack_matrix(self.attn.out_proj.weight, dt), bo=f32(self.attn.out_proj.bias))
        return self._pack.get(self, dt, build)

    def forward_tokens(self, x, x_pos, dt, vt_buf, out_dtype=None):
        P = self.packed(dt)
        E, nh = self.embed_dim, self.num_heads
        hd = E // nh
        vjob = ops.fork(lambda: ops.gemm(x, P["wv"], P["bv"], trans_out=True, out=vt_buf))
        qk = ops.gemm(x_pos, P["wqk"], P["bqk"])
        vt = vjob.join()
        o = ops.attention(qk[:, :E], qk[:, E:], vt, batch=1, n=x.shape[0], heads=nh, head_dim=hd, scale=hd ** -0.5)
        return ops.gemm(o, P["wo"], P["bo"], residual=x, out_dtype=out_dtype or dt)


class TransformerLayer(nn.Module):

    def __init__(self, attentions, ffn, num_norms, embed_dim=256):
        super().__init__()
        self.attentions = nn.ModuleList(attentions)
        self.ffns = nn.ModuleList([ffn])
        self.norms = nn.ModuleList([nn.LayerNorm(embed_dim) for _ in range(num_norms)])
        self.embed_dim = embed_dim
        self.pre_norm = False

    def norm_params(self, i):
        n = self.norms[i]
        return f32(n.weight), f32(n.bias), n.eps


class ConvNormAct(nn.Module):
    def __init__(self, in_channels, out_channels, kernel_size=1, bias=True, norm_layer=None):
        super().__init__()
        self.conv = nn.Conv2d(in_channels, out_channels, kernel_size=kernel_size, padding=(kernel_size - 1) // 2, bias=bias)
        self.norm = norm_layer


class ChannelMapper(nn.Module):

    def __init__(self, input_shapes, in_features, out_channels, kernel_size=1, stride=1, bias=True, groups=1, dilation=1,
                 norm_layer=None, activation=None, num_outs=None, **kwargs):
        super().__init__()
        import copy
        assert kernel_size == 1 and activation is None
        chans = [getattr(input_shapes[f], "channels", input_shapes[f]) for f in in_features]
        assert num_outs is None or num_outs == len(chans), "extra downsampling convs are not used by the APE configs"
        self.convs = nn.ModuleList(ConvNormAct(c, out_channels, 1, bias, copy.deepcopy(norm_layer)) for c in chans)
        self.in_features, self.out_channels, self.input_shapes = in_features, out_channels, input_shapes


class PositionEmbeddingSine(nn.Module):

    def __init__(self, num_pos_feats=64, temperature=10000, scale=2 * 3.141592653589793, eps=1e-6, offset=0.0, normalize=False):
        super().__init__()
        self.num_pos_feats, self.temperature, self.scale, self.eps, self.offset, self.normalize = (
            num_pos_feats, temperature, scale, eps, offset, normalize)
```

### ape_amd/modeling/ape_deta/deformable_transformer_vl.py

```python
import copy

import torch
import torch.nn as nn

from ... import ops
from ...layers import MultiScaleDeformableAttention
from ...packing import attach_cache, f32, pack_matrix, round_up
from ...stagetap import forcing, tap
from . import geometry as G
from ._containers import FFN, SelfAttention, TransformerLayer


class DeformableDetrTransformerEncoderVL(nn.Module):
    def __init__(self, embed_dim=256, num_heads=8, feedforward_dim=1024, attn_dropout=0.1, ffn_dropout=0.1, num_layers=6,
                 post_norm=False, num_feature_levels=4, vl_layer=None, use_act_checkpoint=False, pytorch_attn=False):
        super().__init__()
        self.layers = nn.ModuleList([
            TransformerLayer([MultiScaleDeformableAttention(embed_dim=embed_dim, num_heads=num_heads, dropout=attn_dropout,
                                                            batch_first=True, num_levels=num_feature_levels,
                                                            pytorch_attn=pytorch_attn)],
                             FFN(embed_dim=embed_dim, feedforward_dim=feedforward_dim, output_dim=embed_dim, num_fcs=2,
                                 ffn_drop=ffn_dropout), 2, embed_dim) for _ in range(num_layers)])
        self.num_layers = num_layers
        self.embed_dim = embed_dim
        self.pre_norm = False
        self.post_norm_layer = nn.LayerNorm(embed_dim) if post_norm else None
        self.vl_layers = nn.ModuleList([copy.deepcopy(vl_layer) for _ in range(num_layers)]) if vl_layer is not None else None
        self.use_checkpoint = use_act_checkpoint

    def forward_tokens(self, x, geo, lvl_pos, l, dt, stages=None):
        xp = None
        for i, layer in enumerate(self.layers):
            if self.vl_layers is None:
                v_new, qp, ljob = x, (xp if xp is not None else (x.float() + lvl_pos.float()).to(dt)), ops._Joined(l)
            else:
                v_new, qp, ljob = self.vl_layers[i].b_attn.forward_tokens(x, lvl_pos, l, dt, defer_language=True)
            x2 = layer.attentions[0].forward_tokens(qp, v_new, geo.enc_ref, geo.shapes, geo.starts, dt, value_src=v_new,
                                                    mask=geo.mask_u8, norm=layer.norm_params(0))
            x, xp = layer.ffns[0].forward_tokens(x2, dt, norm=layer.norm_params(1)), None
            l = ljob.join()
            if stages is not None:
                if self.vl_layers is not None:
                    stages[f"enc{i}_fused_v"] = v_new
                    l = tap(stages, f"enc{i}_fused_l", l)
                x = tap(stages, f"enc{i}_out", x)
        if self.post_norm_layer is not None:
            x = ops.layernorm(x, f32(self.post_norm_layer.weight), f32(self.post_norm_layer.bias), self.post_norm_layer.eps, out_dtype=dt)
        return x, l


class DeformableDetrTransformerDecoderVL(nn.Module):
    def __init__(self, embed_dim=256, num_heads=8, feedforward_dim=1024, attn_dropout=0.1, ffn_dropout=0.1, num_layers=6,
                 return_intermediate=True, num_feature_levels=4, use_act_checkpoint=False, look_forward_twice=False,
                 pytorch_attn=False):
        super().__init__()
        self.layers = nn.ModuleList([
            TransformerLayer([SelfAttention(embed_dim=embed_dim, num_heads=num_heads, attn_drop=attn_dropout, batch_first=True),
                              MultiScaleDeformableAttention(embed_dim=embed_dim, num_heads=num_heads, dropout=attn_dropout,
                                                            batch_first=True, num_levels=num_feature_levels,
                                                            pytorch_attn=pytorch_attn)],
                             FFN(embed_dim=embed_dim, feedforward_dim=feedforward_dim, output_dim=embed_dim, ffn_drop=ffn_dropout),
                             3, embed_dim) for _ in range(num_layers)])
        self.num_layers = num_layers
        self.embed_dim = embed_dim
        self.return_intermediate = return_intermediate
        self.bbox_embed = None
        self.class_embed = None
        self.use_checkpoint = use_act_checkpoint
        self.look_forward_twice = look_forward_twice
        attach_cache(self)

    def packed(self, dt):
        def build(dt):
            ws = [l.attentions[1].value_proj.weight for l in self.layers]
            bs = [l.attentions[1].value_proj.bias.detach().float() for l in self.layers]
            return dict(wval=pack_matrix(torch.cat(ws, 0), dt), bval=torch.cat(bs).contiguous())
        return self._pack.get(self, dt, build)

    def forward_tokens(self, query, query_pos, memory, geo, reference, dt, stages=None, query_sum=None):
        P = self.packed(dt)
        E = self.embed_dim
        from ...layers.multi_scale_deform_attn import half_value_kwargs
        value_all = ops.gemm(memory, P["wval"], P["bval"], rowmask=geo.mask_u8, mask_mode=ops.MASK_ZERO_OUTPUT,
                             **half_value_kwargs(dt, memory.shape[0]))
        Q = query.shape[0]
        vt_buf = ops.zeros((E, round_up(Q, 64)), dt, query.device)
        vr4 = geo.vr4
        out = query
        outp = query_sum if query_sum is not None else (query.float() + query_pos.float()).to(dt)
        inter, inter_ref = [], []
        _, ref_in = ops.box_refine(None, reference.contiguous(), vr4)
        refjob = ops._Joined((reference, ref_in))
        for i, layer in enumerate(self.layers):
            x1 = layer.attentions[0].forward_tokens(out, outp, dt, vt_buf)
            x2, x2p = ops.layernorm(x1, *layer.norm_params(0), out_dtype=dt, add=query_pos)
            reference, ref_in = refjob.join()
            if i > 0:
                if stages is not None:
                    forced = tap(stages, f"dec{i - 1}_ref", reference)
                    if forced is not reference:
                        reference = forced
                        _, ref_in = ops.box_refine(None, reference.contiguous(), vr4)
                inter_ref.append(reference)
            x3 = layer.attentions[1].forward_tokens(x2p, x2, ref_in, geo.shapes, geo.starts, dt,
                                                    value=value_all[:, i * E:(i + 1) * E])
            x4 = ops.layernorm(x3, *layer.norm_params(1), out_dtype=dt)
            x5 = layer.ffns[0].forward_tokens(x4, dt)
            out, outp = ops.layernorm(x5, *layer.norm_params(2), out_dtype=dt, add=query_pos)
            if stages is not None:
                forced = tap(stages, f"dec{i}_out", out)
                if forced is not out:
                    out, outp = forced, (forced.float() + query_pos.float()).to(dt)
            if self.bbox_embed is not None:
                def refine(i=i, out=out, reference=reference):
                    tmp = self.bbox_embed[i].forward_tokens(out, dt, out_dtype=torch.float32)
                    if stages is not None:
                        stages[f"dec{i}_delta"] = tmp
                    return ops.box_refine(tmp, reference, vr4)
                refjob = ops.fork(refine)
            inter.append(out)
        reference, _ = refjob.join()
        reference = tap(stages, f"dec{len(self.layers) - 1}_ref", reference)
        inter_ref.append(reference)
        return inter, inter_ref


class DeformableDetrTransformerVL(nn.Module):
    def __init__(self, encoder=None, decoder=None, num_feature_levels=4, as_two_stage=False, two_stage_num_proposals=300,
                 assign_first_stage=False, pre_nms_topk=1000, nms_thresh_enc=0.9, proposal_ambiguous=0):
        super().__init__()
        assert as_two_stage and assign_first_stage, "ape_amd implements the two-stage DETA selection used by every APE config"
        self.encoder, self.decoder = encoder, decoder
        self.num_feature_levels = num_feature_levels
        self.as_two_stage = as_two_stage
        self.two_stage_num_proposals = two_stage_num_proposals
        self.assign_first_stage = assign_first_stage
        self.pre_nms_topk, self.nms_thresh_enc = pre_nms_topk, nms_thresh_enc
        self.proposal_ambiguous = proposal_ambiguous
        self.compute_dtype = torch.bfloat16
        self.embed_dim = self.encoder.embed_dim
        self.level_embeds = nn.Parameter(torch.Tensor(self.num_feature_levels, self.embed_dim))
        self.enc_output = nn.Linear(self.embed_dim, self.embed_dim)
        self.enc_output_norm = nn.LayerNorm(self.embed_dim)
        self.pos_trans = nn.Linear(self.embed_dim * 2, self.embed_dim * 2)
        self.pos_trans_norm = nn.LayerNorm(self.embed_dim * 2)
        self.pix_trans = nn.Linear(self.embed_dim, self.embed_dim)
        self.pix_trans_norm = nn.LayerNorm(self.embed_dim)
        nn.init.normal_(self.level_embeds)
        attach_cache(self)

    def packed(self, dt):
        def build(dt):
            dec = self.decoder
            nd = dec.num_layers
            amb = bool(self.proposal_ambiguous)
            be, bea = dec.bbox_embed[nd], (dec.bbox_embed_ambiguous[0] if amb else dec.bbox_embed[nd])
            ce, cea = dec.class_embed[nd], (dec.class_embed_ambiguous[0] if amb else dec.class_embed[nd])
            return dict(
                wenc=pack_matrix(self.enc_output.weight, dt), benc=f32(self.enc_output.bias),
                nenc=(f32(self.enc_output_norm.weight), f32(self.enc_output_norm.bias), self.enc_output_norm.eps),
                wpos=pack_matrix(self.pos_trans.weight, dt), bpos=f32(self.pos_trans.bias),
                npos=(f32(self.pos_trans_norm.weight), f32(self.pos_trans_norm.bias), self.pos_trans_norm.eps),
                wpix=pack_matrix(self.pix_trans.weight, dt), bpix=f32(self.pix_trans.bias),
                npix=(f32(self.pix_trans_norm.weight), f32(self.pix_trans_norm.bias), self.pix_trans_norm.eps),
                w1=pack_matrix(torch.cat([be.layers[0].weight, bea.layers[0].weight], 0), dt),
                b1=torch.cat([be.layers[0].bias, bea.layers[0].bias]).detach().float().contiguous(),
                w2=(pack_matrix(be.layers[1].weight, dt), pack_matrix(bea.layers[1].weight, dt)),
                b2=(f32(be.layers[1].bias), f32(bea.layers[1].bias)),
                w3=(pack_matrix(be.layers[2].weight, dt), pack_matrix(bea.layers[2].weight, dt)),
                b3=(f32(be.layers[2].bias), f32(bea.layers[2].bias)),
                wcls=pack_matrix(torch.cat([ce.weight, cea.weight], 0), dt),
                bcls=torch.cat([ce.bias, cea.bias]).detach().float().contiguous(),
                level_embeds=f32(self.level_embeds))
        return self._pack.get(self, dt, build)

    def lvl_pos(self, geo, dt):
        key = (dt, self.level_embeds.data_ptr(), self.level_embeds._version)
        if key not in geo._lvl_pos:
            geo._lvl_pos.clear()
            geo._lvl_pos[key] = (geo.pos + self.level_embeds.detach().float()[geo.level_ids]).to(dt).contiguous()
        return geo._lvl_pos[key]

    def forward_tokens(self, src, geo, l, dt, forced_topk=None, stages=None, after_encoder=None, mask_prompt=None):
        P = self.packed(dt)
        lvl_pos = self.lvl_pos(geo, dt)
        memory, l_out = self.encoder.forward_tokens(src, geo, lvl_pos, l, dt, stages)
        memory = tap(stages, "memory", memory)
        if after_encoder is not None:
            after_encoder(memory)
        invalid, anchors = geo.invalid_u8, geo.proposals
        if mask_prompt is not None:
            outside = ~mask_prompt.reshape(-1).to(device=memory.device, dtype=torch.bool)
            invalid = (invalid.reshape(-1).bool() | outside).to(torch.uint8).reshape(invalid.shape).contiguous()
            anchors = anchors.masked_fill(outside[:, None], float("inf")).contiguous()
        om = ops.gemm(memory, P["wenc"], P["benc"], rowmask=invalid, mask_mode=ops.MASK_ZERO_INPUT)
        om = tap(stages, "output_memory", ops.layernorm(om, *P["nenc"], out_dtype=dt))
        E = self.embed_dim
        T = om.shape[0]
        h1 = ops.gemm(om, P["w1"], P["b1"], act=ops.ACT_RELU)
        h2 = torch.empty((T, 2 * E), dtype=dt, device=om.device)
        ops.gemm(h1[:, :E], P["w2"][0], P["b2"][0], act=ops.ACT_RELU, out=h2[:, :E])
        ops.gemm(h1[:, E:], P["w2"][1], P["b2"][1], act=ops.ACT_RELU, out=h2[:, E:])
        d = torch.empty((T, 8), dtype=torch.float32, device=om.device)
        ops.gemm(h2[:, :E], P["w3"][0], P["b3"][0], out=d[:, :4])
        ops.gemm(h2[:, E:], P["w3"][1], P["b3"][1], out=d[:, 4:])
        cls2 = ops.gemm(om, P["wcls"], P["bcls"], out_dtype=torch.float32)
        if stages is not None:
            cls2, d = tap(stages, "enc_cls2", cls2), tap(stages, "enc_delta8", d)
        enc_class, enc_coord, xyxy = ops.enc_finalize(cls2, d, anchors)
        if stages is not None:
            stages["query_l"] = l_out
            enc_class, enc_coord = tap(stages, "enc_class", enc_class), tap(stages, "enc_coord_unact", enc_coord)
        if forced_topk is not None:
            topk = forced_topk.to(om.device).long()
        else:
            topk = ops.select_proposals(enc_class, xyxy, geo.shapes, self.pre_nms_topk, self.two_stage_num_proposals,
                                        self.nms_thresh_enc)
        reference, pe, topk32 = ops.query_init(enc_coord, topk, G.dim_t_table(128, 10000, om.device), dt)
        pos_raw = ops.gemm(pe, P["wpos"], P["bpos"], out_dtype=torch.float32)
        pix_raw = ops.gemm(ops.gather_rows(om, topk32), P["wpix"], P["bpix"], out_dtype=torch.float32)
        query_pos, query, query_sum = ops.query_finish(pos_raw, pix_raw, P["npos"], P["npix"], dt)
        if stages is not None:
            stages["topk_proposals"] = topk
            q0, p0 = query, query_pos
            query, query_pos = tap(stages, "query_init", query), tap(stages, "query_pos", query_pos)
            if query is not q0 or query_pos is not p0:
                query_sum = None
            reference = tap(stages, "init_reference", reference)
        inter, inter_ref = self.decoder.forward_tokens(query, query_pos, memory, geo, reference, dt, stages, query_sum=query_sum)
        return dict(inter_states=inter, init_reference=reference, inter_references=inter_ref, enc_class=enc_class,
                    enc_coord_unact=enc_coord, memory=memory, query_l=l_out, topk_proposals=topk)

    def forward(self, multi_level_feats, multi_level_masks, multi_level_pos_embeds, query_embed=None, query_l=None, attention_mask_l=None,
                multi_level_masks_prompt=None, **kwargs):
        if not self.as_two_stage or query_embed is not None:
            raise NotImplementedError("ape_amd: the two-stage transformer of the APE configs (as_two_stage=True, no query_embed)")
        if attention_mask_l is not None:
            raise NotImplementedError("ape_amd: language masks (un-reduced text tokens, text_feature_reduce_before_fusion=False) are not implemented")
        dt = getattr(self, "compute_dtype", torch.bfloat16)
        B = multi_level_feats[0].shape[0]
        rows = []
        for b in range(B):
            masks = [m[b].bool() for m in multi_level_masks]
            pos = [p[b].flatten(1).t() for p in multi_level_pos_embeds]
            geo = G.geometry_from_masks(masks, pos)
            src = torch.cat([f[b].flatten(1).t() for f in multi_level_feats]).to(dt).contiguous()
            mp = None if multi_level_masks_prompt is None else torch.cat([m[b].reshape(-1) for m in multi_level_masks_prompt]).to(torch.bool)
            tr = self.forward_tokens(src, geo, query_l[b].float().contiguous(), dt, mask_prompt=mp)
            anchors = geo.proposals if mp is None else geo.proposals.masked_fill(~mp.to(geo.proposals.device)[:, None], float("inf"))
            rows.append((torch.stack(tr["inter_states"]), tr["init_reference"], torch.stack(tr["inter_references"]),
                         tr["enc_class"][:, None], tr["enc_coord_unact"], anchors.sigmoid(), tr["memory"], tr["query_l"]))
        odt = multi_level_feats[0].dtype
        cat = lambda i, dim: torch.stack([r[i] for r in rows], dim)
        return (cat(0, 1).to(odt), cat(1, 0).to(odt), cat(2, 1).to(odt), cat(3, 0).to(odt), cat(4, 0).to(odt), cat(5, 0).to(odt),
                cat(6, 0).to(odt), cat(7, 0).to(query_l.dtype))
```

### ape_amd/ops.py

```python
import ctypes
import math
import os

import torch

from . import _lib
from ._lib import (ACT_GELU, ACT_NONE, ACT_RELU, ACT_SILU, ACT_SWIGLU, DT_BF16, DT_F32, MASK_NONE,
                   MASK_ZERO_INPUT, MASK_ZERO_OUTPUT)

_DT = {torch.float32: DT_F32, torch.bfloat16: DT_BF16, torch.float16: _lib.DT_F16}
HALF16 = (torch.bfloat16, torch.float16)


def _dt(t):
    try:
        return _DT[t.dtype]
    except KeyError:
        raise TypeError(f"ape_amd: unsupported dtype {t.dtype} (float32 / bfloat16 / float16 only)")


def _dev(*ts):
    for t in ts:
        if t is not None and not t.is_cuda:
            raise RuntimeError("ape_amd.ops: tensor is not on a HIP device; the HIP path has no CPU fallback")
# ... 788 lines not shown
        raise ValueError("ape_amd.ops.query_init: coords must be contiguous float32 [T,4]")
    if topk.dtype != torch.int64 or not topk.is_contiguous():
        raise ValueError("ape_amd.ops.query_init: topk must be contiguous int64")
    T, Q, P = coords_unact.shape[0], topk.numel(), dim_t.numel()
    dev = coords_unact.device
    reference = torch.empty((Q, 4), dtype=torch.float32, device=dev)
    pe = torch.empty((Q, 4 * P), dtype=out_dtype, device=dev)
    topk32 = torch.empty((Q,), dtype=torch.int32, device=dev)
    rc = _lib.load().ape_hip_query_init(_p(coords_unact), _p(topk), T, _p(_f32vec(dim_t, "dim_t")), P, float(scale), Q, _p(reference),
                                       _p(pe), 4 * P, _dt(pe), _p(topk32), _stream())
    _lib.check(rc, "ape_hip_query_init")
    return reference, pe, topk32


def query_finish(pos, pix, norm_pos, norm_pix, out_dtype):
    _dev(pos, pix)
    _rowmajor(pos, "pos"), _rowmajor(pix, "pix")
    Q, E = pix.shape
    if pos.dtype != torch.float32 or pix.dtype != torch.float32 or pos.shape != (Q, 2 * E):
        raise ValueError("ape_amd.ops.query_finish: pos [Q, 2E] / pix [Q, E] float32")
    outs = [torch.empty((Q, E), dtype=out_dtype, device=pos.device) for _ in range(3)]
    rc = _lib.load().ape_hip_query_finish(_p(pos), _ld(pos), _p(pix), _ld(pix), Q, E, _p(_f32vec(norm_pos[0], "w")), _p(_f32vec(norm_pos[1], "b")),
                                         float(norm_pos[2]), _p(_f32vec(norm_pix[0], "w")), _p(_f32vec(norm_pix[1], "b")), float(norm_pix[2]),
                                         _p(outs[0]), _p(outs[1]), _p(outs[2]), E, _dt(outs[0]), _stream())
    _lib.check(rc, "ape_hip_query_finish")
    return tuple(outs)


_SIDE_STREAMS = {}
_FORK_DEPTH = [0]


class _Joined:
    def __init__(self, result, done=None, keep=None):
        self.result, self.done, self.keep = result, done, keep

    def join(self):
        if self.done is not None:
            torch.cuda.current_stream().wait_event(self.done)
            self.done = None
        self.keep = None
        return self.result


_FORK_INLINE = [False]
_FORK_NEST = [0]


class inline_forks:

    def __enter__(self):
        self.prev = _FORK_INLINE[0]
        _FORK_INLINE[0] = True

    def __exit__(self, *exc):
        _FORK_INLINE[0] = self.prev


def fork(fn, force=False):
    if not torch.cuda.is_available() or os.environ.get("APE_NO_FORK") == "1" or (_FORK_INLINE[0] and not force):
        return _Joined(fn())
    if _FORK_NEST[0] > 0 and os.environ.get("APE_FORK_NESTED") != "1":
        return _Joined(fn())
    dev = torch.cuda.current_device()
    cur = torch.cuda.current_stream()
    pool = _SIDE_STREAMS.setdefault((dev, cur.cuda_stream), [torch.cuda.Stream(device=dev) for _ in range(8)])
    side = pool[_FORK_DEPTH[0] % len(pool)]
    _FORK_DEPTH[0] += 1
    start = torch.cuda.Event()
    start.record(cur)
    side.wait_event(start)
    with torch.cuda.stream(side):
        _FORK_NEST[0] += 1
        try:
            result = fn()
        finally:
            _FORK_NEST[0] -= 1
        done = torch.cuda.Event()
        done.record(side)
    return _Joined(result, done, keep=fn)


def resize_coeffs(in_size, out_size):
    lib = _lib.load()
    ks = lib.ape_hip_resize_coeffs(int(in_size), int(out_size), None, None, 0)
    if ks <= 0:
        _lib.check(ks, "ape_hip_resize_coeffs")
    bounds = torch.empty((out_size, 2), dtype=torch.int32)
    kk = torch.empty((out_size, ks), dtype=torch.int32)
    rc = lib.ape_hip_resize_coeffs(int(in_size), int(out_size), ctypes.c_void_p(bounds.data_ptr()), ctypes.c_void_p(kk.data_ptr()), ks)
    if rc != ks:
        _lib.check(rc if rc < 0 else -1, "ape_hip_resize_coeffs")
    return bounds, kk


class _ResizePlan:

    def __init__(self, H, W, newh, neww, device):
        self.key = (H, W, newh, neww)
        self.bh = self.kh = self.bv = self.kv = None
        self.ks_h = self.ks_v = 0
        self.tile_h, self.lds_rows = 32, 32
        if neww != W:
            b, k = resize_coeffs(W, neww)
            self.bh, self.kh, self.ks_h = b.to(device), k.to(device), k.shape[1]
        if newh != H:
            b, k = resize_coeffs(H, newh)
            th = ctypes.c_int(0)
            rows = _lib.load().ape_hip_resize_tile_rows(ctypes.c_void_p(b.data_ptr()), newh, ctypes.byref(th))
            if rows <= 0:
                _lib.check(rows if rows < 0 else -1, "ape_hip_resize_tile_rows")
            self.tile_h, self.lds_rows = th.value, rows
            self.bv, self.kv, self.ks_v = b.to(device), k.to(device), k.shape[1]


_RESIZE_PLANS = {}


def resize_bilinear_u8(src, newh, neww, *, out=None, float_chw=False, flip=False):
    _dev(src, out)
    if src.dtype != torch.uint8 or src.dim() != 3 or src.shape[2] != 3 or src.stride(2) != 1 or src.stride(1) != 3:
        raise ValueError("ape_amd.ops.resize_bilinear_u8: src must be uint8 [H, W, 3] with packed pixels")
    H, W = src.shape[:2]
    key = (H, W, newh, neww, src.device.index)
    plan = _RESIZE_PLANS.get(key)
    if plan is None:
        if len(_RESIZE_PLANS) > 256:
            _RESIZE_PLANS.clear()
        plan = _RESIZE_PLANS[key] = _ResizePlan(H, W, newh, neww, src.device)
    if float_chw:
        if out is None:
            out = torch.empty((3, newh, neww), dtype=torch.float32, device=src.device)
        if out.dtype != torch.float32 or tuple(out.shape) != (3, newh, neww) or out.stride(2) != 1:
            raise ValueError("ape_amd.ops.resize_bilinear_u8: out must be float32 [3, newh, neww] with contiguous rows")
        kind, ld, plane = 1, out.stride(1), out.stride(0)
    else:
        if out is None:
            out = torch.empty((newh, neww, 3), dtype=torch.uint8, device=src.device)
        if out.dtype != torch.uint8 or tuple(out.shape) != (newh, neww, 3) or out.stride(2) != 1 or out.stride(1) != 3:
            raise ValueError("ape_amd.ops.resize_bilinear_u8: out must be uint8 [newh, neww, 3] with packed pixels")
        kind, ld, plane = 0, out.stride(0), 0
    rc = _lib.load().ape_hip_resize_bilinear_u8(_p(src), H, W, src.stride(0), _p(plan.bh), _p(plan.kh), plan.ks_h, _p(plan.bv),
                                                _p(plan.kv), plan.ks_v, newh, neww, plan.tile_h, plan.lds_rows, _p(out), kind,
                                                ld, plane, int(bool(flip)), _stream())
    _lib.check(rc, "ape_hip_resize_bilinear_u8")
    return out


def rle_encode(masks, cap=4096, counts=None, nruns=None):
    _dev(masks)
    if masks.dtype == torch.bool:
        masks = masks.view(torch.uint8)
    if masks.dtype != torch.uint8 or masks.dim() != 3 or not masks.is_contiguous():
        raise ValueError("ape_amd.ops.rle_encode: masks must be contiguous uint8 / bool [n, H, W]")
    n, H, W = masks.shape
    if counts is None:
        counts = torch.empty((n, cap), dtype=torch.int32, device=masks.device)
    if nruns is None:
        nruns = torch.zeros((n,), dtype=torch.int32, device=masks.device)
    _dev(counts, nruns)
    if (counts.dtype != torch.int32 or nruns.dtype != torch.int32 or tuple(counts.shape) != (n, cap) or tuple(nruns.shape) != (n,)
            or not counts.is_contiguous() or not nruns.is_contiguous()):
        raise ValueError("ape_amd.ops.rle_encode: counts / nruns must be contiguous int32 [n, cap] / [n]")
    if n == 0:
        return counts, nruns
    lib = _lib.load()
    words = lib.ape_hip_rle_workspace_words(n, H, W, cap)
    if words <= 0:
        raise ValueError("ape_amd.ops.rle_encode: workspace exceeds 2^31 words; encode fewer masks per call")
    ws = torch.empty((words,), dtype=torch.int32, device=masks.device)
    rc = lib.ape_hip_rle_encode(_p(masks), n, H, W, _p(ws), _p(counts), cap, _p(nruns), _stream())
    _lib.check(rc, "ape_hip_rle_encode")
    return counts, nruns


def rle_to_string(counts):
    c = torch.as_tensor(counts, dtype=torch.int64).to(torch.int32).contiguous() if not isinstance(counts, torch.Tensor) \
        else counts.contiguous()
    if c.is_cuda or c.dtype not in (torch.int32,):
        raise ValueError("ape_amd.ops.rle_to_string: counts must be a host int32 tensor")
    n = c.numel()
    buf = ctypes.create_string_buffer(max(8, 7 * n))
    rc = _lib.load().ape_hip_rle_to_string(ctypes.c_void_p(c.data_ptr()), n, buf, len(buf))
    if rc < 0:
        raise RuntimeError("ape_hip_rle_to_string: buffer too small")
    return buf.raw[:rc]


def _level_arrays(level_shapes):
    L = len(level_shapes)
    ns = [int(h) * int(w) for h, w in level_shapes]
    starts = [sum(ns[:i]) for i in range(L)]
    return (ctypes.c_int * L)(*starts), (ctypes.c_int * L)(*ns), L, starts, ns


def _f32c(t, name, shape=None):
    if t.dtype != torch.float32 or not t.is_contiguous() or (shape is not None and tuple(t.shape) != tuple(shape)):
        raise ValueError(f"ape_amd.ops: {name} must be contiguous float32" + (f" {tuple(shape)}" if shape is not None else ""))
    return t


def enc_finalize(cls2, d, anchors):
    _dev(cls2, d, anchors)
    T = cls2.shape[0]
    _f32c(cls2, "cls2", (T, 2)), _f32c(d, "d", (T, 8)), _f32c(anchors, "anchors", (T, 4))
    enc_class = torch.empty((T,), dtype=torch.float32, device=cls2.device)
    enc_coord = torch.empty((T, 4), dtype=torch.float32, device=cls2.device)
    xyxy = torch.empty((T, 4), dtype=torch.float32, device=cls2.device)
    rc = _lib.load().ape_hip_enc_finalize(_p(cls2), _p(d), _p(anchors), T, _p(enc_class), _p(enc_coord), _p(xyxy), _stream())
    _lib.check(rc, "ape_hip_enc_finalize")
    return enc_class, enc_coord, xyxy


def select_proposals(logit, xyxy, level_shapes, pre_nms_topk, num_queries, iou_thr):
    _dev(logit, xyxy)
    T = logit.numel()
    _f32c(logit, "logit", (T,)), _f32c(xyxy, "xyxy", (T, 4))
    starts_c, ns_c, L, starts, ns = _level_arrays(level_shapes)
    if sum(ns) != T:
        raise ValueError("ape_amd.ops.select_proposals: level shapes do not add up to the token count")
    k, k_alt = min(int(pre_nms_topk), T), min(int(num_queries), T)
    n = L * k
    dev = logit.device
    lib = _lib.load()
    cand = torch.empty((n,), dtype=torch.int32, device=dev)
    alt = torch.empty((k_alt,), dtype=torch.int32, device=dev)
    ws = torch.empty((lib.ape_hip_topk_workspace_words(T),), dtype=torch.int64, device=dev)
    _lib.check(lib.ape_hip_proposal_topk(_p(logit), T, starts_c, ns_c, L, k, k_alt, _p(ws), _p(cand), _p(alt), _stream()), "ape_hip_proposal_topk")
    boxes_b = torch.empty((n, 4), dtype=torch.float32, device=dev)
    ints = torch.empty((4 * n + L + 1,), dtype=torch.int32, device=dev)
    groups_b, cand_a, lv_a, pos_b, seg = ints[:n], ints[n:2 * n], ints[2 * n:3 * n], ints[3 * n:4 * n], ints[4 * n:]
    rc = lib.ape_hip_proposal_order(_p(cand), n, _p(logit), _p(xyxy), starts_c, ns_c, L, _p(boxes_b), _p(groups_b), _p(seg), _p(cand_a),
                                    _p(lv_a), _p(pos_b), _stream())
    _lib.check(rc, "ape_hip_proposal_order")
    max_seg = min(n, k + sum(max(0, k - m) for m in ns))
    mask = torch.empty((n, lib.ape_hip_nms_mask_words(n)), dtype=torch.int64, device=dev)
    keep = torch.zeros((n,), dtype=torch.uint8, device=dev)
    _lib.check(lib.ape_hip_nms_mask(_p(boxes_b), _p(groups_b), n, float(iou_thr), _p(mask), _stream()), "ape_hip_nms_mask")
    _lib.check(lib.ape_hip_nms_scan_segments(_p(mask), n, _p(seg), L, int(max_seg), None, _p(keep), _stream()), "ape_hip_nms_scan_segments")
    out = torch.empty((int(num_queries),), dtype=torch.int64, device=dev)
    rc = lib.ape_hip_proposal_quota(_p(cand_a), _p(lv_a), _p(pos_b), _p(keep), n, _p(alt), k_alt, starts_c, ns_c, L, int(num_queries),
                                    _p(out), _stream())
    _lib.check(rc, "ape_hip_proposal_quota")
    return out


def detections(logits, boxes, scale, score_thresh, iou_thr, topk):
    _dev(logits, boxes, scale)
    _rowmajor(logits, "logits")
    Q, K = logits.shape
    if logits.dtype != torch.float32:
        raise TypeError("ape_amd.ops.detections: logits must be float32")
    _f32c(boxes, "boxes", (Q, 4)), _f32c(scale, "scale", (4,))
    dev = logits.device
    lib = _lib.load()
    xyxy = torch.empty((Q, 4), dtype=torch.float32, device=dev)
    finite = torch.empty((Q,), dtype=torch.uint8, device=dev)
    sorted_scores = torch.empty((K, Q), dtype=torch.float32, device=dev)
    order = torch.empty((K, Q), dtype=torch.int32, device=dev)
    valid = torch.empty((K, Q), dtype=torch.uint8, device=dev)
    rc = lib.ape_hip_det_sort(_p(logits), _ld(logits), Q, K, _p(boxes), _p(scale), float(score_thresh), _p(xyxy), _p(finite),
                              _p(sorted_scores), _p(order), _p(valid), _stream())
    _lib.check(rc, "ape_hip_det_sort")
    keep = nms_classes(xyxy, order, iou_thr, valid)
    k = min(int(topk), K * Q)
    det = dict(det_boxes=torch.empty((k, 4), dtype=torch.float32, device=dev), det_scores=torch.empty((k,), dtype=torch.float32, device=dev),
               det_classes=torch.empty((k,), dtype=torch.int64, device=dev), det_query=torch.empty((k,), dtype=torch.int64, device=dev))
    ws = torch.empty((lib.ape_hip_topk_workspace_words(K * Q),), dtype=torch.int64, device=dev)
    rc = lib.ape_hip_det_topk(_p(sorted_scores), _p(keep), _p(order), _p(xyxy), K, Q, k, _p(ws), _p(det["det_boxes"]), _p(det["det_scores"]),
                              _p(det["det_classes"]), _p(det["det_query"]), _stream())
    _lib.check(rc, "ape_hip_det_topk")
    return det


def ffn_fused(x, w1, b1, w2, b2, residual=None, out=None, w2_permuted=False, norm=None):
    _dev(x, w1, w2, b1, b2, residual, out)
    for t, name in ((x, "x"), (w1, "w1"), (w2, "w2")):
        _rowmajor(t, name)
        if t.dtype not in HALF16 or t.dtype != x.dtype:
            raise TypeError(f"ape_amd.ops.ffn_fused: {name} must be bfloat16 or float16, one type per call")
    M, K = x.shape
    HID, N = w1.shape[0], w2.shape[0]
    if w1.shape[1] != K or w2.shape[1] != HID:
        raise ValueError("ape_amd.ops.ffn_fused: weight shapes do not chain")
    if out is None:
        out = torch.empty((M, N), dtype=x.dtype, device=x.device)
    if out.dtype != x.dtype:
        raise TypeError("ape_amd.ops.ffn_fused: out must have x's dtype")
    if residual is not None:
        _rowmajor(residual, "residual")
        if residual.dtype != x.dtype or tuple(residual.shape) != (M, N):
            raise TypeError("ape_amd.ops.ffn_fused: residual must be [M, N] in x's dtype")
    if norm is not None:
        _dev(norm[0], norm[1])
        if norm[0].numel() != N or norm[1].numel() != N:
            raise ValueError("ape_amd.ops.ffn_fused: norm = (weight [N], bias [N], eps)")
    rc = _lib.load().ape_hip_ffn_fused(_p(x), _ld(x), _p(w1), _ld(w1), _p(_f32vec(b1, "b1")), _p(w2), _ld(w2), _p(_f32vec(b2, "b2")),
                                      _p(residual), _ld(residual) if residual is not None else 0, _p(out), _ld(out), M, K, HID, N,
                                      1 if w2_permuted else 0, _dt(x), _p(_f32vec(norm[0], "norm weight")) if norm is not None else None,
                                      _p(_f32vec(norm[1], "norm bias")) if norm is not None else None,
                                      float(norm[2]) if norm is not None else 0.0, _stream())
    _lib.check(rc, "ape_hip_ffn_fused")
    return out
```

### include/ape_hip.h

```cpp
#ifndef APE_HIP_H
#define APE_HIP_H
#include <stdint.h>

#ifdef __cplusplus
extern "C" {
#endif

#define APE_DT_F32 0
#define APE_DT_BF16 1
#define APE_DT_F16 2

#define APE_ACT_NONE 0
#define APE_ACT_RELU 1
#define APE_ACT_GELU 2
#define APE_ACT_SWIGLU 3
#define APE_ACT_SILU 4

#define APE_MASK_NONE 0
#define APE_MASK_ZERO_INPUT 1
#define APE_MASK_ZERO_OUTPUT 2

const char* ape_hip_last_error(void);
int ape_hip_abi_version(void);
int ape_hip_sizeof_args(int which);

typedef struct ApeGemmArgs {
  const void* A;
  const void* W;
  void* C;
  const float* bias;
  const void* residual;
  const uint8_t* rowmask;
  const float* rope_cos;
  const float* rope_sin;
  int32_t M, N, K;
  int32_t lda, ldw, ldc, ldr;
  int32_t in_dt, out_dt, res_dt;
  int32_t act;
  int32_t mask_mode;
  int32_t trans_out;
  int32_t rope_rows, rope_hd, rope_cols;
  int32_t vec_ok;
  float alpha;
  float clamp;
  int32_t splitk;
  int32_t tile64;
  float* workspace;
  const float* rowscale;
  const float* rowshift;
  const float* colvec;
  const float* rope_cs;
  const float* ln_w;
  const float* ln_b;
  float ln_eps;
  int32_t reserved0;
  const int32_t* conv_perm;
  const void* conv_zero;
  int32_t conv_h, conv_w;
  int32_t rowstat_cols;
  float rowstat_eps;
} ApeGemmArgs;
int ape_hip_gemm(const ApeGemmArgs* args, void* stream);
const char* ape_hip_gemm_last_kernel(void);

int ape_hip_meter_begin(void);
int ape_hip_meter_count(void);
int ape_hip_meter_end(void);
int ape_hip_meter_read(int i, const char** name, float* ms);
int ape_hip_zero(void* ptr, size_t nbytes, void* stream);
int ape_hip_sdma_usable(const void* host_dst, const void* dev_src);
int ape_hip_sdma_d2h(void* host_dst, const void* dev_src, size_t nbytes);
int ape_hip_sdma_d2h_multi(int n, void* const* host_dst, const void* const* dev_src, const size_t* nbytes, int parts);
int ape_hip_sdma_engines(const void* host_dst, const void* dev_src);

int ape_hip_row_stats(const void* x, int ldx, int dt, int M, int C, float eps, float* rowscale, float* rowshift, void* stream);

int ape_hip_gemv(const float* x, int ldx, const void* W, int ldw, int w_dt, const float* bias, float* out, int ldo,
                 int M, int N, int K, float alpha, void* stream);
int ape_hip_gemv_affine(const float* x, int ldx, const void* W, int ldw, int w_dt, const float* bias, float* out, int ldo,
                        int M, int N, int K, float alpha, const float* scale, const float* add, int ldadd, float* out2, int ldo2,
                        void* stream);

typedef struct ApeLayerNormArgs {
  const void* x;
  const float* w;
  const float* b;
  void* y;
  const void* add;
  void* y2;
  int32_t M, C, Cpad;
  int32_t ldx, ldy, ldadd, ldy2;
  int32_t x_dt, y_dt, add_dt;
  int32_t act;
  float eps;
} ApeLayerNormArgs;
int ape_hip_layernorm(const ApeLayerNormArgs* args, void* stream);

int ape_hip_postnorm_residual(const void* t, int ldt, int t_dt, const float* w, const float* b, float eps, float* stream, int lds,
                              void* copy, int ldc, int copy_dt, int M, int C, void* hip_stream);


typedef struct ApeGroupNormArgs {
  const void* x;
  const float* w;
  const float* b;
  void* y;
  const void* add;
  float* workspace;
  int32_t HW, C, G;
  int32_t ldx, ldy, ldadd;
  int32_t x_dt, y_dt, add_dt;
  int32_t act;
  float eps;
} ApeGroupNormArgs;
int ape_hip_groupnorm_workspace_floats(int HW, int G);
int ape_hip_groupnorm(const ApeGroupNormArgs* args, void* stream);

int ape_hip_ms_deform_attn_forward(const void* value, int ldv, const int64_t* spatial_shapes,
                                   const int64_t* level_start_index, const void* sampling_loc,
                                   const void* attn_weight, void* out, int ldout, int B, int S, int Q, int L,
                                   int dt, void* stream);
int ape_hip_msda_fused(const void* value, int ldv, int v_dt, const int64_t* spatial_shapes,
                       const int64_t* level_start_index, const float* offw, int ldoffw, const float* ref,
                       int refdim, void* out, int ldout, int out_dt, int B, int S, int Q, int L, void* stream);
int ape_hip_msda_fused_h(const void* value, int ldv, int v_dt, const int64_t* spatial_shapes,
                       const int64_t* level_start_index, const void* offw_f16, int ldoffw, const float* ref,
                       int refdim, void* out, int ldout, int out_dt, int B, int S, int Q, int L, void* stream);

int ape_hip_attention(const void* Q, int ldq, const void* K, int ldk, const void* Vt, int ldvt, void* O, int ldo,
                      int B, int N, int H, int HD, float scale, int dt, void* stream);
int ape_hip_attention_strided(const void* Q, int ldq, const void* K, int ldk, const void* Vt, int ldvt, void* O, int ldo,
                              int B, int N, int bstride, int H, int HD, float scale, int dt, void* stream);
int ape_hip_attention_causal(const void* Q, int ldq, const void* K, int ldk, const void* Vt, int ldvt, void* O, int ldo,
                              int B, int N, int bstride, int H, int HD, float scale, int dt, void* stream);


int ape_hip_patchify(const float* img, int h, int w, const int32_t* tok2raster, int Ht, int Wt, const float* mean3,
                     const float* std3, void* out, int ldo, int out_dt, void* stream);
int ape_hip_im2col3x3(const void* x, int ldx, const int32_t* perm, int H, int W, int C, void* out, int ldo, int dt, void* stream);
int ape_hip_maxpool2x2(const void* x, int ldx, const int32_t* perm, int H, int W, int C, void* out, int ldo, int dt, void* stream);
int ape_hip_gather_rows(const void* x, int ldx, const int32_t* idx, int n, int C, void* out, int ldo, int dt, void* stream);
int ape_hip_gather_rows_i64(const void* x, int ldx, const int64_t* idx, int n, int C, void* out, int ldo, int dt, void* stream);

int ape_hip_nms_mask_words(int n);
int ape_hip_nms_mask(const float* boxes_xyxy, const int32_t* groups, int n, float iou_thr, uint64_t* mask, void* stream);
int ape_hip_nms_scan_segments(const uint64_t* mask, int n, const int32_t* seg_offsets, int num_segments, int max_segment,
                              const uint8_t* valid, uint8_t* keep, void* stream);
int ape_hip_nms_scan_classes(const uint64_t* mask, int n, const int32_t* order, int num_classes, const uint8_t* valid,
                             uint8_t* keep, void* stream);

int ape_hip_vl_pool_workspace_floats(int T, int C);
int ape_hip_vl_pool(const float* S, int lds, const void* x, int ldx, int x_dt, int T, int C, float* workspace, const float* sub,
                    float* out, void* stream);
int ape_hip_head_gemv(const float* x, int ldx, const float* W, const float* bias, float* out, int ldo, int H, int N, int D,
                      float alpha, void* out_bf16, int ldob, int copy_dt, void* stream);

int ape_hip_segment_softmax(const float* S, int lds, int T, int nseg, int L, const float* gmax, void* out, int ldo, int out_dt,
                            void* stream);
int ape_hip_colstats_workspace_floats(int T, int C);
int ape_hip_colstats(const float* S, int lds, int T, int C, const float* gmax, float* workspace, float* colmax, float* colsum,
                     void* stream);
int ape_hip_transpose(const void* S, int lds, int in_dt, int T, int C, const float* gmax, const float* colmax,
                      const float* colsum, void* out, int ldo, int out_dt, void* stream);
int ape_hip_stuff_collapse(const float* logits, int ldl, int Q, int K, int nt, float* out, int ldo, void* stream);
int ape_hip_sem_class_weights(const float* logits, int ldl, const int64_t* qidx, const float* valid_score, int k, int kp, int K, float temp,
                              void* A, int lda, int out_dt, void* stream);
int ape_hip_pan_class_scores(const float* logits, int ldl, const int64_t* qidx, const float* valid_score, int k, int K, float thresh, int transform,
                             float temp, float* score, int64_t* label, int32_t* label32 , uint8_t* keep, void* stream);
int ape_hip_argmax_labels(const float* x, size_t ld_class, int C, size_t n, float class0, int16_t* out, void* stream);


int ape_hip_mask_upsample_bits(const void* logits, int ldl, int dt, int h0, int w0, int S, int n, uint8_t* out, void* stream);
int ape_hip_roi_align_bits(const uint8_t* bits, int H, int W, const float* boxes, int n, int P, uint8_t* out, void* stream);
int ape_hip_paste_bits(const uint8_t* masks, int P, const float* boxes, int n, int Ho, int Wo, uint8_t* out, void* stream);

int ape_hip_mask_upsample_sigmoid(const void* logits, int ldl, int in_dt, int h0, int w0, int S, int crop_h, int crop_w, int n,
                                  void* out, int ldo, int out_dt, void* stream);
int ape_hip_bilinear_resize(const float* in, int ld_channel, int ld_row, int h, int w, int C, float* out, int H, int W,
                            void* stream);

int ape_hip_panoptic_pixels(const float* masks, int ld_query, int ld_row, int h, int w, int k, const float* scores, const uint8_t* keep,
                            float prob, int H, int W, int16_t* owner, uint8_t* conf, int* areas, void* stream);
int ape_hip_panoptic_decide(const int* areas, const int* classes, const uint8_t* keep, int k, const uint8_t* isthing, int num_classes,
                            double overlap_threshold, int stuff_offset, int* seg_id, int* info, int* count, void* stream);
int ape_hip_panoptic_write(const int16_t* owner, const uint8_t* conf, const int* seg_id, int H, int W, int* out, void* stream);

int ape_hip_box_refine(const float* delta, int ldd, const float* ref, const float* vr4, int L, int Q, float eps, float* new_ref,
                       float* ref_in, void* stream);

int ape_hip_det_records(const float* boxes, const float* scores, const int64_t* classes, const int64_t* query, const float* frame,
                        int k, float* rec, float* boxes_out, int32_t* order, void* stream);
int ape_hip_query_init(const float* coords, const int64_t* topk, int T, const float* dim_t, int P, float scale, int Q,
                       float* reference, void* pe, int ldpe, int pe_dt, int32_t* topk32, void* stream);
int ape_hip_query_finish(const float* pos, int ldpos, const float* pix, int ldpix, int Q, int E, const float* wpos,
                         const float* bpos, float eps_pos, const float* wpix, const float* bpix, float eps_pix, void* query_pos,
                         void* query, void* query_sum, int ldo, int out_dt, void* stream);

int ape_hip_geometry(int S, int h, int w, int L, const int* level_hw, const float* dim_t, int npf, const float* level_embeds,
                     float offset, float eps, float scale, void* lvl_pos, int lvl_pos_dt, uint8_t* mask_u8, uint8_t* mask_bool,
                     uint8_t* invalid_u8, float* enc_ref, float* proposals, float* valid_ratios, float* vr4, float* box_scale,
                     void* stream);

int ape_hip_resize_coeffs(int in_size, int out_size, int32_t* bounds, int32_t* kk, int ksize_cap);
int ape_hip_resize_tile_rows(const int32_t* bounds_v_host, int newh, int* tile_h);
int ape_hip_resize_bilinear_u8(const uint8_t* src, int H, int W, int src_ld, const int32_t* bounds_h, const int32_t* kk_h,
                               int ks_h, const int32_t* bounds_v, const int32_t* kk_v, int ks_v, int newh, int neww, int tile_h,
                               int lds_rows, void* dst, int dst_kind, int dst_ld, int dst_plane, int flip, void* stream);

int ape_hip_rle_workspace_words(int n, int H, int W, int cap);
int ape_hip_rle_encode(const uint8_t* masks, int n, int H, int W, uint32_t* workspace, uint32_t* counts, int cap, uint32_t* nruns,
                       void* stream);
int ape_hip_rle_to_string(const uint32_t* counts, int n, char* out, int cap);

int ape_hip_embed_tokens(const int32_t* tokens, int ldt, const void* table, int ldtab, const void* pos, int ldpos, int dt, float* out,
                         int ldo, int B, int L, int Lp, int W, int vocab, void* stream);

int ape_hip_enc_finalize(const float* cls2, const float* d, const float* anchors, int T, float* enc_class, float* enc_coord,
                         float* xyxy, void* stream);
int ape_hip_topk_workspace_words(int n_total);
int ape_hip_proposal_topk(const float* logit, int T, const int* level_start, const int* level_n, int L, int k, int k_alt,
                          uint64_t* workspace, int32_t* cand, int32_t* alt, void* stream);
int ape_hip_proposal_order(const int32_t* cand, int n, const float* logit, const float* xyxy, const int* level_start,
                           const int* level_n, int L, float* boxes_b, int32_t* groups_b, int32_t* seg, int32_t* cand_a,
                           int32_t* lv_a, int32_t* pos_b, void* stream);
int ape_hip_proposal_quota(const int32_t* cand_a, const int32_t* lv_a, const int32_t* pos_b, const uint8_t* keep_b, int n,
                           const int32_t* alt, int n_alt, const int* level_start, const int* level_n, int L, int nq, int64_t* out,
                           void* stream);
int ape_hip_det_sort(const float* logits, int ldl, int Q, int K, const float* boxes, const float* scale, float thresh, float* xyxy,
                     uint8_t* finite, float* sorted, int32_t* order, uint8_t* valid, void* stream);
int ape_hip_det_topk(const float* sorted, const uint8_t* keep, const int32_t* order, const float* xyxy, int K, int Q, int k,
                     uint64_t* workspace, float* det_boxes, float* det_scores, int64_t* det_classes, int64_t* det_query, void* stream);

int ape_hip_attention_ext(const void* Q, int ldq, const void* K, int ldk, const void* Vt, int ldvt, void* O, int ldo, int B, int N,
                          int bstride, int H, int HDQ, int HDV, float scale, int dt, void* stream);
int ape_hip_relpos_extend(const void* q, const void* k, int ldqk, const void* t, int ldt, int tper, const int* ty, const int* tx, int period,
                          void* q_ext, void* k_ext, int lde, int rows, int nh, int hs, int hd, int Hk, int Wk, int hdq, float scale, int dt,
                          void* stream);

int ape_hip_ffn_fused(const void* X, int ldx, const void* W1, int ldw1, const float* b1, const void* W2, int ldw2, const float* b2,
                      const void* residual, int ldr, void* Y, int ldy, int M, int K, int HID, int N, int w2_permuted, int dt,
                      const float* ln_weight, const float* ln_bias, float ln_eps, void* stream);

#ifdef __cplusplus
}
#endif
#endif
```

Measured before the change: 115.4.

## Fuse deformable-DETR decoder layer stages into three per-query-tile HIP kernels

Adds three fused HIP kernels for the transformer decoder. One handles the self-attention output projection, residual, layernorm and query-pos add. One chains cross-attention offset projection, deformable sampling, output projection, layernorm, FFN and a second layernorm. The third runs the 3-layer bbox MLP together with box refinement. Each block keeps a 16-query tile in LDS across stages, which removes many small kernel launches and global round trips of intermediate activations. The trade-off is low parallelism for small query counts, since weights are re-read by every tile. The path is on by default through an env flag.

```diff
diff --git a/ape_amd/_lib.py b/ape_amd/_lib.py
--- a/ape_amd/_lib.py
+++ b/ape_amd/_lib.py
@@ -155,6 +155,14 @@
     "ape_hip_rle_workspace_words": (c_int, [c_int, c_int, c_int, c_int]),
     "ape_hip_rle_encode": (c_int, [c_void_p, c_int, c_int, c_int, c_void_p, c_void_p, c_int, c_void_p, c_void_p]),
     "ape_hip_rle_to_string": (c_int, [c_void_p, c_int, c_void_p, c_int]),
+    "ape_hip_dec_attn_out": (c_int, [c_void_p, c_int, c_void_p, c_int, c_void_p, c_int, c_void_p, c_int, c_void_p, c_void_p, c_void_p, c_float,
+                                     c_void_p, c_void_p, c_int, c_int, c_int, c_void_p]),
+    "ape_hip_dec_cross_ffn": (c_int, [c_void_p, c_int, c_void_p, c_int, c_void_p, c_int, c_void_p, c_int, c_int, POINTER(c_int64), POINTER(c_int64),
+                                      c_int, c_int, c_void_p, c_void_p, c_int, c_void_p, c_void_p, c_int, c_void_p, c_void_p, c_void_p, c_float,
+                                      c_void_p, c_int, c_void_p, c_void_p, c_int, c_void_p, c_int, c_void_p, c_void_p, c_float, c_void_p, c_void_p,
+                                      c_int, c_int, c_int, c_void_p]),
+    "ape_hip_dec_box": (c_int, [c_void_p, c_int, c_void_p, c_int, c_void_p, c_void_p, c_int, c_void_p, c_void_p, c_int, c_void_p, c_void_p,
+                                c_void_p, c_int, c_float, c_void_p, c_void_p, c_void_p, c_int, c_int, c_void_p]),
 }
 
 _lib = None
diff --git a/ape_amd/csrc/boxes.hip b/ape_amd/csrc/boxes.hip
--- a/ape_amd/csrc/boxes.hip
+++ b/ape_amd/csrc/boxes.hip
@@ -7,12 +7,7 @@
   const int gid = blockIdx.x * 256 + threadIdx.x;
   if (gid >= Q * 4) return;
   const int q = gid >> 2, c = gid & 3;
-  float x = ref[gid];
-  x = fminf(fmaxf(x, 0.f), 1.f);
-  const float x1 = fmaxf(x, eps), x2 = fmaxf(1.f - x, eps);
-  float z = logf(x1 / x2);
-  if (delta != nullptr) z += delta[(size_t)q * ldd + c];
-  const float r = delta != nullptr ? 1.f / (1.f + expf(-z)) : ref[gid];
+  const float r = delta != nullptr ? box_refine_value(ref[gid], delta[(size_t)q * ldd + c], eps) : ref[gid];
   if (new_ref != nullptr) new_ref[gid] = r;
   if (ref_in != nullptr)
     for (int l = 0; l < L; ++l) ref_in[((size_t)q * L + l) * 4 + c] = r * vr4[l * 4 + c];
diff --git a/ape_amd/csrc/common.h b/ape_amd/csrc/common.h
--- a/ape_amd/csrc/common.h
+++ b/ape_amd/csrc/common.h
@@ -146,6 +146,13 @@
 #pragma unroll
   for (int o = 32; o > 0; o >>= 1) v = fmaxf(v, __shfl_xor(v, o, 64));
   return v;
+}
+
+__device__ __forceinline__ float box_refine_value(float ref, float delta, float eps) {
+  const float x = fminf(fmaxf(ref, 0.f), 1.f);
+  const float x1 = fmaxf(x, eps), x2 = fmaxf(1.f - x, eps);
+  const float z = logf(x1 / x2) + delta;
+  return 1.f / (1.f + expf(-z));
 }
 
 extern "C" const char* ape_hip_last_error(void);
diff --git a/ape_amd/csrc/decoder_fused.hip b/ape_amd/csrc/decoder_fused.hip
--- /dev/null
+++ b/ape_amd/csrc/decoder_fused.hip
@@ -0,0 +1,426 @@
+#include "common.h"
+#include "msda_sample.h"
+#include "../../include/ape_hip.h"
+
+constexpr int DF_Q = 16;
+constexpr int DF_NW = 8;
+constexpr int DF_THREADS = DF_NW * 64;
+constexpr int DF_E = 256;
+constexpr int DF_LDX = DF_E + 8;
+
+struct EpiIn { float b[4], r[4]; };
+template <typename H, int TN, typename Pre, typename Epi>
+__device__ __forceinline__ void tile_gemm(const H* __restrict__ W, int ldw, int N, int K, const H* sX, int ldx, Pre&& pre, Epi&& epi) {
+  const int lane = threadIdx.x & 63, wave = threadIdx.x >> 6;
+  const int arow = lane & 15, kq = lane >> 4;
+  const int KC = (K + 255) >> 8;
+  const int NG = (N + 16 * TN - 1) / (16 * TN);
+  const H* xb = sX + arow * ldx + kq * 8;
+  bf16x8_t a[TN][8], an[TN][8];
+  auto load_a = [&](int g, int kc, bf16x8_t (&d)[TN][8]) {
+    const int nks = min(8, (K - (kc << 8)) >> 5);
+#pragma unroll
+    for (int t = 0; t < TN; ++t) {
+      const int n = min((g * TN + t) * 16 + arow, N - 1);
+      const H* src = W + (size_t)n * ldw + (kc << 8) + kq * 8;
+#pragma unroll
+      for (int ks = 0; ks < 8; ++ks)
+        if (ks < nks) d[t][ks] = *reinterpret_cast<const bf16x8_t*>(src + ks * 32);
+    }
+  };
+  if (wave >= NG) return;
+  int g = wave, kc = 0;
+  int rem = ((NG - 1 - wave) / DF_NW + 1) * KC;
+  f32x4_t acc[TN];
+  EpiIn ein[TN];
+  auto preload = [&]() {
+    if (kc == KC - 1) {
+#pragma unroll
+      for (int t = 0; t < TN; ++t) ein[t] = pre((g * TN + t) * 16 + kq * 4, arow);
+    }
+  };
+  auto compute = [&](bf16x8_t (&cur)[TN][8]) {
+    if (kc == 0) {
+#pragma unroll
+      for (int t = 0; t < TN; ++t) acc[t] = (f32x4_t){0.f, 0.f, 0.f, 0.f};
+    }
+    const int nks = min(8, (K - (kc << 8)) >> 5);
+#pragma unroll
+    for (int ks = 0; ks < 8; ++ks) {
+      if (ks < nks) {
+        const bf16x8_t b = *reinterpret_cast<const bf16x8_t*>(xb + (kc << 8) + ks * 32);
+#pragma unroll
+        for (int t = 0; t < TN; ++t) acc[t] = h16<H>::mfma(cur[t][ks], b, acc[t]);
+      }
+    }
+    if (kc == KC - 1) {
+#pragma unroll
+      for (int t = 0; t < TN; ++t) {
+        float v[4] = {acc[t][0], acc[t][1], acc[t][2], acc[t][3]};
+        epi((g * TN + t) * 16 + kq * 4, arow, v, ein[t]);
+      }
+    }
+  };
+  auto step = [&](bf16x8_t (&cur)[TN][8], bf16x8_t (&nxt)[TN][8]) {
+    int gn = g, kn = kc + 1;
+    if (kn == KC) { kn = 0; gn = g + DF_NW; }
+    preload();
+    load_a(gn, kn, nxt);
+    __builtin_amdgcn_sched_barrier(0);
+    compute(cur);
+    g = gn; kc = kn; --rem;
+  };
+  load_a(g, 0, a);
+  __builtin_amdgcn_sched_barrier(0);
+  for (;;) {
+    if (rem == 1) { preload(); compute(a); break; }
+    step(a, an);
+    if (rem == 1) { preload(); compute(an); break; }
+    step(an, a);
+  }
+}
+
+template <typename H>
+__device__ __forceinline__ void load_tile(const H* x, int ldx, int q0, int Q, H* sX) {
+  const int r = threadIdx.x >> 5, c = (threadIdx.x & 31) * 8;
+  uint4 v = make_uint4(0u, 0u, 0u, 0u);
+  if (q0 + r < Q) v = *reinterpret_cast<const uint4*>(x + (size_t)(q0 + r) * ldx + c);
+  *reinterpret_cast<uint4*>(sX + r * DF_LDX + c) = v;
+}
+
+template <typename H>
+__device__ __forceinline__ void st4_lds(H* dst, const float v[4]) {
+  *reinterpret_cast<uint2*>(dst) = make_uint2(h16<H>::pack2(v[0], v[1]), h16<H>::pack2(v[2], v[3]));
+}
+
+template <typename H>
+__device__ __forceinline__ void ln_row(const H* srow, const float* __restrict__ w, const float* __restrict__ b, float eps, int lane, float (&o)[4]) {
+  const float invC = 1.f / (float)DF_E;
+  float v[4];
+  ld4<H>(srow + lane * 4, v);
+  const float s = (v[0] + v[1]) + (v[2] + v[3]);
+  const float mean = wave_sum(s) * invC;
+  float q = 0.f;
+#pragma unroll
+  for (int r = 0; r < 4; ++r) { const float d = v[r] - mean; q = fmaf(d, d, q); }
+  const float rstd = rsqrtf(wave_sum(q) * invC + eps);
+  float w4[4], b4[4];
+  ld4<float>(w + lane * 4, w4);
+  ld4<float>(b + lane * 4, b4);
+#pragma unroll
+  for (int r = 0; r < 4; ++r) o[r] = (v[r] - mean) * rstd * w4[r] + b4[r];
+}
+
+__device__ __forceinline__ EpiIn pre_bias(const float* bias, int n0) {
+  EpiIn in;
+  ld4<float>(bias + n0, in.b);
+#pragma unroll
+  for (int e = 0; e < 4; ++e) in.r[e] = 0.f;
+  return in;
+}
+template <typename H>
+__device__ __forceinline__ EpiIn pre_bias_res(const float* bias, const H* res, int ldr, int row, int Q, int n0) {
+  EpiIn in = pre_bias(bias, n0);
+  if (row < Q) ld4<H>(res + (size_t)row * ldr + n0, in.r);
+  return in;
+}
+
+struct DecAttnOutParams {
+  const void *o, *x, *qpos, *wo;
+  const float *bo, *ln_w, *ln_b;
+  void *x2, *x2p;
+  int ldo, ldx, ldqpos, ldwo, ldy, Q;
+  float eps;
+};
+
+template <typename H>
+__global__ __launch_bounds__(DF_THREADS) void dec_attn_out_kernel(const DecAttnOutParams p) {
+  __shared__ __attribute__((aligned(16))) H sA[DF_Q * DF_LDX];
+  __shared__ __attribute__((aligned(16))) H sB[DF_Q * DF_LDX];
+  const int q0 = blockIdx.x * DF_Q;
+  const int lane = threadIdx.x & 63, wave = threadIdx.x >> 6;
+  load_tile<H>(reinterpret_cast<const H*>(p.o), p.ldo, q0, p.Q, sA);
+  __syncthreads();
+  const H* x = reinterpret_cast<const H*>(p.x);
+  tile_gemm<H, 2>(reinterpret_cast<const H*>(p.wo), p.ldwo, DF_E, DF_E, sA, DF_LDX,
+      [&](int n0, int q) { return pre_bias_res<H>(p.bo, x, p.ldx, q0 + q, p.Q, n0); },
+      [&](int n0, int q, float (&v)[4], const EpiIn& in) {
+#pragma unroll
+        for (int e = 0; e < 4; ++e) v[e] = v[e] + in.b[e] + in.r[e];
+        st4_lds<H>(sB + q * DF_LDX + n0, v);
+      });
+  __syncthreads();
+#pragma unroll
+  for (int rr = 0; rr < DF_Q / DF_NW; ++rr) {
+    const int q = wave + rr * DF_NW;
+    float o[4], o2[4];
+    ln_row<H>(sB + q * DF_LDX, p.ln_w, p.ln_b, p.eps, lane, o);
+    if (q0 + q < p.Q) {
+      const size_t row = (size_t)(q0 + q);
+      ld4<H>(reinterpret_cast<const H*>(p.qpos) + row * p.ldqpos + lane * 4, o2);
+#pragma unroll
+      for (int e = 0; e < 4; ++e) o2[e] += o[e];
+      st4<H>(reinterpret_cast<H*>(p.x2) + row * p.ldy + lane * 4, o);
+      st4<H>(reinterpret_cast<H*>(p.x2p) + row * p.ldy + lane * 4, o2);
+    }
+  }
+}
+
+struct DecCrossParams {
+  MsdaParams ms;
+  const void *x2p, *x2, *qpos;
+  const void *woffw, *wout, *w1, *w2;
+  const float *boffw, *bout, *b1, *b2, *ln1_w, *ln1_b, *ln2_w, *ln2_b;
+  void *out, *outp;
+  int ldx2p, ldx2, ldqpos, ldwoffw, ldwout, ldw1, ldw2, ldout, F;
+  float eps1, eps2;
+};
+
+static inline size_t dec_cross_lds(int L, int F, int hsize) {
+  const size_t offw = (size_t)DF_Q * (96 * L + 4) * 4, hid = (size_t)DF_Q * (F + 8) * hsize;
+  return 2 * (size_t)DF_Q * DF_LDX * hsize + (offw > hid ? offw : hid);
+}
+
+template <typename H, typename TV, int L>
+__global__ __launch_bounds__(DF_THREADS) void dec_cross_ffn_kernel(const DecCrossParams p) {
+  extern __shared__ __attribute__((aligned(16))) unsigned char df_smem[];
+  H* sA = reinterpret_cast<H*>(df_smem);
+  H* sB = sA + DF_Q * DF_LDX;
+  float* sOff = reinterpret_cast<float*>(sB + DF_Q * DF_LDX);
+  H* sHid = reinterpret_cast<H*>(sOff);
+  constexpr int NOFF = MS_HEADS * L * MS_P * 3;
+  constexpr int LDO = NOFF + 4;
+  const int q0 = blockIdx.x * DF_Q, Q = p.ms.Q;
+  const int lane = threadIdx.x & 63, wave = threadIdx.x >> 6;
+
+  load_tile<H>(reinterpret_cast<const H*>(p.x2p), p.ldx2p, q0, Q, sA);
+  __syncthreads();
+  tile_gemm<H, 2>(reinterpret_cast<const H*>(p.woffw), p.ldwoffw, NOFF, DF_E, sA, DF_LDX,
+      [&](int n0, int q) { return pre_bias(p.boffw, n0); },
+      [&](int n0, int q, float (&v)[4], const EpiIn& in) {
+        *reinterpret_cast<float4*>(sOff + q * LDO + n0) = make_float4(v[0] + in.b[0], v[1] + in.b[1], v[2] + in.b[2], v[3] + in.b[3]);
+      });
+  __syncthreads();
+  {
+    const int g = lane >> 2, sub = lane & 3;
+    const int ql = wave * 2 + (g >> 3), h = g & 7;
+    const int qi = min(q0 + ql, Q - 1);
+    const TV* vb = reinterpret_cast<const TV*>(p.ms.value) + h * MS_D + sub * 8;
+    const unsigned char* vbase = reinterpret_cast<const unsigned char*>(p.ms.value);
+    const uint32_t lane_off = (uint32_t)((h * MS_D + sub * 8) * sizeof(TV));
+    const uint32_t rowb = (uint32_t)(p.ms.ldv * (int)sizeof(TV));
+    const float* orow = sOff + ql * LDO;
+    float acc[8];
+    msda_quad_sample<TV, L, float>(p.ms, orow + MS_HEADS * L * MS_P * 2 + h * L * MS_P, orow + h * L * MS_P * 2 + sub * 2,
+                                   p.ms.ref + (size_t)qi * L * 4, vb, vbase, lane_off, rowb, sub, acc);
+    *reinterpret_cast<uint4*>(sA + ql * DF_LDX + h * MS_D + sub * 8) =
+        make_uint4(h16<H>::pack2(acc[0], acc[1]), h16<H>::pack2(acc[2], acc[3]), h16<H>::pack2(acc[4], acc[5]), h16<H>::pack2(acc[6], acc[7]));
+  }
+  __syncthreads();
+  const H* x2 = reinterpret_cast<const H*>(p.x2);
+  tile_gemm<H, 2>(reinterpret_cast<const H*>(p.wout), p.ldwout, DF_E, DF_E, sA, DF_LDX,
+      [&](int n0, int q) { return pre_bias_res<H>(p.bout, x2, p.ldx2, q0 + q, Q, n0); },
+      [&](int n0, int q, float (&v)[4], const EpiIn& in) {
+#pragma unroll
+        for (int e = 0; e < 4; ++e) v[e] = v[e] + in.b[e] + in.r[e];
+        st4_lds<H>(sB + q * DF_LDX + n0, v);
+      });
+  __syncthreads();
+#pragma unroll
+  for (int rr = 0; rr < DF_Q / DF_NW; ++rr) {
+    const int q = wave + rr * DF_NW;
+    float o[4];
+    ln_row<H>(sB + q * DF_LDX, p.ln1_w, p.ln1_b, p.eps1, lane, o);
+    st4_lds<H>(sA + q * DF_LDX + lane * 4, o);
+  }
+  __syncthreads();
+  const int ldh = p.F + 8;
+  tile_gemm<H, 2>(reinterpret_cast<const H*>(p.w1), p.ldw1, p.F, DF_E, sA, DF_LDX,
+      [&](int n0, int q) { return pre_bias(p.b1, n0); },
+      [&](int n0, int q, float (&v)[4], const EpiIn& in) {
+#pragma unroll
+        for (int e = 0; e < 4; ++e) v[e] = fmaxf(v[e] + in.b[e], 0.f);
+        st4_lds<H>(sHid + q * ldh + n0, v);
+      });
+  __syncthreads();
+  tile_gemm<H, 2>(reinterpret_cast<const H*>(p.w2), p.ldw2, DF_E, p.F, sHid, ldh,
+      [&](int n0, int q) { return pre_bias(p.b2, n0); },
+      [&](int n0, int q, float (&v)[4], const EpiIn& in) {
+        float r[4];
+        ld4<H>(sA + q * DF_LDX + n0, r);
+#pragma unroll
+        for (int e = 0; e < 4; ++e) v[e] = v[e] + in.b[e] + r[e];
+        st4_lds<H>(sB + q * DF_LDX + n0, v);
+      });
+  __syncthreads();
+#pragma unroll
+  for (int rr = 0; rr < DF_Q / DF_NW; ++rr) {
+    const int q = wave + rr * DF_NW;
+    float o[4], o2[4];
+    ln_row<H>(sB + q * DF_LDX, p.ln2_w, p.ln2_b, p.eps2, lane, o);
+    if (q0 + q < Q) {
+      const size_t row = (size_t)(q0 + q);
+      ld4<H>(reinterpret_cast<const H*>(p.qpos) + row * p.ldqpos + lane * 4, o2);
+#pragma unroll
+      for (int e = 0; e < 4; ++e) o2[e] += o[e];
+      st4<H>(reinterpret_cast<H*>(p.out) + row * p.ldout + lane * 4, o);
+      st4<H>(reinterpret_cast<H*>(p.outp) + row * p.ldout + lane * 4, o2);
+    }
+  }
+}
+
+struct DecBoxParams {
+  const void *x, *w1, *w2, *w3;
+  const float *b1, *b2, *b3, *ref, *vr4;
+  float *delta, *new_ref, *ref_in;
+  int ldx, ldw1, ldw2, ldw3, L, Q;
+  float eps;
+};
+
+template <typename H>
+__global__ __launch_bounds__(DF_THREADS) void dec_box_kernel(const DecBoxParams p) {
+  __shared__ __attribute__((aligned(16))) H sA[DF_Q * DF_LDX];
+  __shared__ __attribute__((aligned(16))) H sB[DF_Q * DF_LDX];
+  const int q0 = blockIdx.x * DF_Q;
+  load_tile<H>(reinterpret_cast<const H*>(p.x), p.ldx, q0, p.Q, sA);
+  __syncthreads();
+  tile_gemm<H, 2>(reinterpret_cast<const H*>(p.w1), p.ldw1, DF_E, DF_E, sA, DF_LDX,
+      [&](int n0, int q) { return pre_bias(p.b1, n0); },
+      [&](int n0, int q, float (&v)[4], const EpiIn& in) {
+#pragma unroll
+        for (int e = 0; e < 4; ++e) v[e] = fmaxf(v[e] + in.b[e], 0.f);
+        st4_lds<H>(sB + q * DF_LDX + n0, v);
+      });
+  __syncthreads();
+  tile_gemm<H, 2>(reinterpret_cast<const H*>(p.w2), p.ldw2, DF_E, DF_E, sB, DF_LDX,
+      [&](int n0, int q) { return pre_bias(p.b2, n0); },
+      [&](int n0, int q, float (&v)[4], const EpiIn& in) {
+#pragma unroll
+        for (int e = 0; e < 4; ++e) v[e] = fmaxf(v[e] + in.b[e], 0.f);
+        st4_lds<H>(sA + q * DF_LDX + n0, v);
+      });
+  __syncthreads();
+  tile_gemm<H, 1>(reinterpret_cast<const H*>(p.w3), p.ldw3, 4, DF_E, sA, DF_LDX, [&](int n0, int q) { return EpiIn(); }, [&](int n0, int q, float (&v)[4], const EpiIn&) {
+    if (n0 != 0 || q0 + q >= p.Q) return;
+    const size_t row = (size_t)(q0 + q);
+    float d[4], r[4], rf[4];
+    ld4<float>(p.ref + row * 4, rf);
+#pragma unroll
+    for (int c = 0; c < 4; ++c) {
+      d[c] = v[c] + p.b3[c];
+      r[c] = box_refine_value(rf[c], d[c], p.eps);
+    }
+    st4<float>(p.delta + row * 4, d);
+    st4<float>(p.new_ref + row * 4, r);
+    for (int l = 0; l < p.L; ++l) {
+      float o[4];
+#pragma unroll
+      for (int c = 0; c < 4; ++c) o[c] = r[c] * p.vr4[l * 4 + c];
+      st4<float>(p.ref_in + (row * p.L + l) * 4, o);
+    }
+  });
+}
+
+static inline bool al16(const void* p) { return ((uintptr_t)p) % 16 == 0; }
+
+extern "C" int ape_hip_dec_attn_out(const void* o, int ldo, const void* x, int ldx, const void* qpos, int ldqpos, const void* wo, int ldwo,
+                                    const float* bo, const float* ln_w, const float* ln_b, float ln_eps, void* x2, void* x2p, int ldy, int Q,
+                                    int dt, void* stream) {
+  APE_CHECK_ARG(o && x && qpos && wo && bo && ln_w && ln_b && x2 && x2p, "ape_hip_dec_attn_out: null pointer");
+  APE_CHECK_ARG(Q > 0 && (dt == APE_DT_BF16 || dt == APE_DT_F16), "ape_hip_dec_attn_out: Q >= 1, dtype bf16 (1) or f16 (2), got Q %d dt %d", Q, dt);
+  APE_CHECK_ARG(ldo % 8 == 0 && ldx % 4 == 0 && ldqpos % 4 == 0 && ldwo % 8 == 0 && ldy % 4 == 0 && ldo >= DF_E && ldx >= DF_E && ldqpos >= DF_E &&
+                    ldwo >= DF_E && ldy >= DF_E && al16(o) && al16(x) && al16(qpos) && al16(wo) && al16(bo) && al16(ln_w) && al16(ln_b) && al16(x2) && al16(x2p),
+                "ape_hip_dec_attn_out: 16-byte aligned pointers, rows of 256 channels (ld %% 8 == 0 for o / wo, %% 4 otherwise)");
+  DecAttnOutParams p;
+  p.o = o; p.x = x; p.qpos = qpos; p.wo = wo; p.bo = bo; p.ln_w = ln_w; p.ln_b = ln_b; p.x2 = x2; p.x2p = x2p;
+  p.ldo = ldo; p.ldx = ldx; p.ldqpos = ldqpos; p.ldwo = ldwo; p.ldy = ldy; p.Q = Q; p.eps = ln_eps;
+  const dim3 grid(ceil_div(Q, DF_Q)), block(DF_THREADS);
+  hipStream_t s = (hipStream_t)stream;
+  if (dt == APE_DT_F16) APE_LAUNCH(dec_attn_out_kernel<f16_t>, grid, block, 0, s, p);
+  else APE_LAUNCH(dec_attn_out_kernel<bf16_t>, grid, block, 0, s, p);
+  APE_CHECK_LAUNCH("ape_hip_dec_attn_out");
+  return 0;
+}
+
+template <typename H, typename TV>
+static void launch_dec_cross(const DecCrossParams& p, int L, size_t lds, hipStream_t s) {
+  const dim3 grid(ceil_div(p.ms.Q, DF_Q)), block(DF_THREADS);
+  static ApeOncePerDevice attr;
+  if (attr.first()) {
+    (void)hipFuncSetAttribute((const void*)dec_cross_ffn_kernel<H, TV, 1>, hipFuncAttributeMaxDynamicSharedMemorySize, 96 * 1024);
+    (void)hipFuncSetAttribute((const void*)dec_cross_ffn_kernel<H, TV, 2>, hipFuncAttributeMaxDynamicSharedMemorySize, 96 * 1024);
+    (void)hipFuncSetAttribute((const void*)dec_cross_ffn_kernel<H, TV, 3>, hipFuncAttributeMaxDynamicSharedMemorySize, 96 * 1024);
+    (void)hipFuncSetAttribute((const void*)dec_cross_ffn_kernel<H, TV, 4>, hipFuncAttributeMaxDynamicSharedMemorySize, 96 * 1024);
+    (void)hipFuncSetAttribute((const void*)dec_cross_ffn_kernel<H, TV, 5>, hipFuncAttributeMaxDynamicSharedMemorySize, 96 * 1024);
+  }
+  switch (L) {
+    case 1: APE_LAUNCH((dec_cross_ffn_kernel<H, TV, 1>), grid, block, lds, s, p); break;
+    case 2: APE_LAUNCH((dec_cross_ffn_kernel<H, TV, 2>), grid, block, lds, s, p); break;
+    case 3: APE_LAUNCH((dec_cross_ffn_kernel<H, TV, 3>), grid, block, lds, s, p); break;
+    case 4: APE_LAUNCH((dec_cross_ffn_kernel<H, TV, 4>), grid, block, lds, s, p); break;
+    default: APE_LAUNCH((dec_cross_ffn_kernel<H, TV, 5>), grid, block, lds, s, p); break;
+  }
+}
+
+extern "C" int ape_hip_dec_cross_ffn(const void* x2p, int ldx2p, const void* x2, int ldx2, const void* qpos, int ldqpos, const void* value, int ldv,
+                                     int v_dt, const int64_t* spatial_shapes, const int64_t* level_start_index, int L, int S, const float* ref_in,
+                                     const void* woffw, int ldwoffw, const float* boffw, const void* wout, int ldwout, const float* bout,
+                                     const float* ln1_w, const float* ln1_b, float ln1_eps, const void* w1, int ldw1, const float* b1,
+                                     const void* w2, int ldw2, const float* b2, int F, const float* ln2_w, const float* ln2_b, float ln2_eps,
+                                     void* out, void* outp, int ldout, int Q, int dt, void* stream) {
+  APE_CHECK_ARG(x2p && x2 && qpos && value && spatial_shapes && level_start_index && ref_in && woffw && boffw && wout && bout && ln1_w && ln1_b &&
+                    w1 && b1 && w2 && b2 && ln2_w && ln2_b && out && outp, "ape_hip_dec_cross_ffn: null pointer");
+  APE_CHECK_ARG(Q > 0 && S > 0 && (dt == APE_DT_BF16 || dt == APE_DT_F16), "ape_hip_dec_cross_ffn: Q >= 1, dtype bf16 (1) or f16 (2), got Q %d dt %d", Q, dt);
+  APE_CHECK_ARG(v_dt == dt || v_dt == APE_DT_F16, "ape_hip_dec_cross_ffn: values in the activations' type or IEEE half, got %d", v_dt);
+  APE_CHECK_ARG(F >= 64 && F <= 2048 && F % 64 == 0, "ape_hip_dec_cross_ffn: FFN width %d not a multiple of 64 in 64..2048", F);
+  APE_CHECK_ARG(ldx2p % 8 == 0 && ldx2 % 4 == 0 && ldqpos % 4 == 0 && ldv % 8 == 0 && ldwoffw % 8 == 0 && ldwout % 8 == 0 && ldw1 % 8 == 0 &&
+                    ldw2 % 8 == 0 && ldout % 4 == 0 && ldx2p >= DF_E && ldx2 >= DF_E && ldqpos >= DF_E && ldwoffw >= DF_E && ldwout >= DF_E &&
+                    ldw1 >= DF_E && ldw2 >= F && ldout >= DF_E,
+                "ape_hip_dec_cross_ffn: leading dimensions (rows of 256 channels, 16-byte rows for the MFMA operands)");
+  APE_CHECK_ARG(al16(x2p) && al16(x2) && al16(qpos) && al16(value) && al16(ref_in) && al16(woffw) && al16(boffw) && al16(wout) && al16(bout) &&
+                    al16(ln1_w) && al16(ln1_b) && al16(w1) && al16(b1) && al16(w2) && al16(b2) && al16(ln2_w) && al16(ln2_b) && al16(out) && al16(outp),
+                "ape_hip_dec_cross_ffn: pointers must be 16-byte aligned");
+  DecCrossParams p;
+  memset(&p, 0, sizeof(p));
+  p.ms.value = value; p.ms.ldv = ldv; p.ms.ref = ref_in; p.ms.refdim = 4; p.ms.S = S; p.ms.Q = Q;
+  if (fill_levels(p.ms, spatial_shapes, level_start_index, L, S)) return -1;
+  APE_CHECK_ARG((uint64_t)S * (uint64_t)ldv * 2 < (1ull << 32) && S < (1 << 24) && ldv * 2 < (1 << 24),
+                "ape_hip_dec_cross_ffn: the value tensor must stay below 4 GiB (S = %d rows of %d elements)", S, ldv);
+  p.ms.pow2 = 1;
+  for (int l = 0; l < L; ++l) {
+    p.ms.pow2 &= ((p.ms.W[l] & (p.ms.W[l] - 1)) == 0 && (p.ms.H[l] & (p.ms.H[l] - 1)) == 0) ? 1 : 0;
+    p.ms.invW[l] = 1.f / (float)p.ms.W[l]; p.ms.invH[l] = 1.f / (float)p.ms.H[l];
+  }
+  p.x2p = x2p; p.x2 = x2; p.qpos = qpos; p.woffw = woffw; p.wout = wout; p.w1 = w1; p.w2 = w2;
+  p.boffw = boffw; p.bout = bout; p.b1 = b1; p.b2 = b2; p.ln1_w = ln1_w; p.ln1_b = ln1_b; p.ln2_w = ln2_w; p.ln2_b = ln2_b;
+  p.out = out; p.outp = outp;
+  p.ldx2p = ldx2p; p.ldx2 = ldx2; p.ldqpos = ldqpos; p.ldwoffw = ldwoffw; p.ldwout = ldwout; p.ldw1 = ldw1; p.ldw2 = ldw2; p.ldout = ldout;
+  p.F = F; p.eps1 = ln1_eps; p.eps2 = ln2_eps;
+  const size_t lds = dec_cross_lds(L, F, 2);
+  hipStream_t s = (hipStream_t)stream;
+  if (dt == APE_DT_F16) launch_dec_cross<f16_t, f16_t>(p, L, lds, s);
+  else if (v_dt == APE_DT_F16) launch_dec_cross<bf16_t, f16_t>(p, L, lds, s);
+  else launch_dec_cross<bf16_t, bf16_t>(p, L, lds, s);
+  APE_CHECK_LAUNCH("ape_hip_dec_cross_ffn");
+  return 0;
+}
+
+extern "C" int ape_hip_dec_box(const void* x, int ldx, const void* w1, int ldw1, const float* b1, const void* w2, int ldw2, const float* b2,
+                               const void* w3, int ldw3, const float* b3, const float* ref, const float* vr4, int L, float eps, float* delta,
+                               float* new_ref, float* ref_in, int Q, int dt, void* stream) {
+  APE_CHECK_ARG(x && w1 && b1 && w2 && b2 && w3 && b3 && ref && vr4 && delta && new_ref && ref_in, "ape_hip_dec_box: null pointer");
+  APE_CHECK_ARG(Q > 0 && L > 0 && (dt == APE_DT_BF16 || dt == APE_DT_F16), "ape_hip_dec_box: Q, L >= 1, dtype bf16 (1) or f16 (2), got Q %d L %d dt %d", Q, L, dt);
+  APE_CHECK_ARG(ldx % 8 == 0 && ldw1 % 8 == 0 && ldw2 % 8 == 0 && ldw3 % 8 == 0 && ldx >= DF_E && ldw1 >= DF_E && ldw2 >= DF_E && ldw3 >= DF_E &&
+                    al16(x) && al16(w1) && al16(b1) && al16(w2) && al16(b2) && al16(w3) && al16(ref) && al16(delta) && al16(new_ref) && al16(ref_in),
+                "ape_hip_dec_box: 16-byte aligned pointers and rows of 256 channels");
+  DecBoxParams p;
+  p.x = x; p.w1 = w1; p.w2 = w2; p.w3 = w3; p.b1 = b1; p.b2 = b2; p.b3 = b3; p.ref = ref; p.vr4 = vr4;
+  p.delta = delta; p.new_ref = new_ref; p.ref_in = ref_in;
+  p.ldx = ldx; p.ldw1 = ldw1; p.ldw2 = ldw2; p.ldw3 = ldw3; p.L = L; p.Q = Q; p.eps = eps;
+  const dim3 grid(ceil_div(Q, DF_Q)), block(DF_THREADS);
+  hipStream_t s = (hipStream_t)stream;
+  if (dt == APE_DT_F16) APE_LAUNCH(dec_box_kernel<f16_t>, grid, block, 0, s, p);
+  else APE_LAUNCH(dec_box_kernel<bf16_t>, grid, block, 0, s, p);
+  APE_CHECK_LAUNCH("ape_hip_dec_box");
+  return 0;
+}
diff --git a/ape_amd/csrc/msda.hip b/ape_amd/csrc/msda.hip
--- a/ape_amd/csrc/msda.hip
+++ b/ape_amd/csrc/msda.hip
@@ -1,33 +1,8 @@
-#include <type_traits>
-
 #include "common.h"
+#include "msda_sample.h"
 #include "../../include/ape_hip.h"
 
-#define MS_HEADS 8
-#define MS_D 32
-#define MS_P 4
-
-struct MsdaParams {
-  const void* value; int ldv;
-  const void* loc;
-  const void* attn;
-  const void* offw; int ldoffw;
-  int offw_f16;
-  const float* ref; int refdim;
-  void* out; int ldout;
-  int S, Q;
-  int H[8], W[8], start[8];
-  float invW[8], invH[8];
-  int pow2;
-};
-
-template <typename TV>
-__device__ __forceinline__ void corner_acc(const TV* __restrict__ vbase, int ldv, int idx, float wgt, float acc[8]) {
-  float v[8];
-  ld8<TV>(vbase + (size_t)idx * ldv, v);
-#pragma unroll
-  for (int c = 0; c < 8; ++c) acc[c] = fmaf(wgt, v[c], acc[c]);
-}
+
 
 template <typename TV>
 __device__ __forceinline__ void sample_acc(const TV* __restrict__ vlvl, int ldv, int H, int W, float lx, float ly,
@@ -128,73 +103,6 @@
   st8<TO>(o, acc);
 }
 
-template <int P> __device__ __forceinline__ float quad_bcast_f(float v) {
-  return __int_as_float(__builtin_amdgcn_mov_dpp(__float_as_int(v), P * 0x55, 0xf, 0xf, true));
-}
-template <int P> __device__ __forceinline__ int quad_bcast_i(int v) { return __builtin_amdgcn_mov_dpp(v, P * 0x55, 0xf, 0xf, true); }
-__device__ __forceinline__ float quad_xor1(float v) { return __int_as_float(__builtin_amdgcn_mov_dpp(__float_as_int(v), 0xB1, 0xf, 0xf, true)); }
-__device__ __forceinline__ float quad_xor2(float v) { return __int_as_float(__builtin_amdgcn_mov_dpp(__float_as_int(v), 0x4E, 0xf, 0xf, true)); }
-
-__device__ __forceinline__ float quad_pick_f(int P, float v) {
-  return P == 0 ? quad_bcast_f<0>(v) : (P == 1 ? quad_bcast_f<1>(v) : (P == 2 ? quad_bcast_f<2>(v) : quad_bcast_f<3>(v)));
-}
-__device__ __forceinline__ int quad_pick_i(int P, int v) {
-  return P == 0 ? quad_bcast_i<0>(v) : (P == 1 ? quad_bcast_i<1>(v) : (P == 2 ? quad_bcast_i<2>(v) : quad_bcast_i<3>(v)));
-}
-
-template <typename TV>
-struct CornerGroup {
-  uint4 raw[4];
-  float w[4];
-};
-
-template <typename TV, int L>
-__device__ __forceinline__ void group_load(const unsigned char* __restrict__ vbase, uint32_t lane_off, const float (&cw)[L][4],
-                                           const int (&ci)[L][4], int s, CornerGroup<TV>& g) {
-  const int l = s >> 2, P = s & 3;
-#pragma unroll
-  for (int c = 0; c < 4; ++c) {
-    g.w[c] = quad_pick_f(P, cw[l][c]);
-    uint32_t off = (uint32_t)quad_pick_i(P, ci[l][c]) + lane_off;
-    asm volatile("" : "+v"(off));
-    g.raw[c] = *reinterpret_cast<const uint4*>(vbase + (size_t)off);
-  }
-}
-
-__device__ __forceinline__ void fma_mix_lo(float& acc, uint32_t d, float w) {
-  asm volatile("v_fma_mix_f32 %0, %1, %2, %0 op_sel:[0,0,0] op_sel_hi:[1,0,0]" : "+v"(acc) : "v"(d), "v"(w));
-}
-__device__ __forceinline__ void fma_mix_hi(float& acc, uint32_t d, float w) {
-  asm volatile("v_fma_mix_f32 %0, %1, %2, %0 op_sel:[1,0,0] op_sel_hi:[1,0,0]" : "+v"(acc) : "v"(d), "v"(w));
-}
-template <typename TV>
-__device__ __forceinline__ void group_fma_half(const CornerGroup<TV>& g, float (&acc)[8]) {
-#pragma unroll
-  for (int c = 0; c < 4; ++c) {
-    const uint32_t d[4] = {g.raw[c].x, g.raw[c].y, g.raw[c].z, g.raw[c].w};
-#pragma unroll
-    for (int e = 0; e < 4; ++e) {
-      fma_mix_lo(acc[2 * e], d[e], g.w[c]);
-      fma_mix_hi(acc[2 * e + 1], d[e], g.w[c]);
-    }
-  }
-}
-
-template <typename TV>
-__device__ __forceinline__ void group_fma(const CornerGroup<TV>& g, f32x2_t (&a2)[4]) {
-#pragma unroll
-  for (int c = 0; c < 4; ++c) {
-    const f32x2_t ww = {g.w[c], g.w[c]};
-    const uint32_t d[4] = {g.raw[c].x, g.raw[c].y, g.raw[c].z, g.raw[c].w};
-#pragma unroll
-    for (int e = 0; e < 4; ++e) {
-      const f32x2_t v2 = {__uint_as_float(d[e] << 16), __uint_as_float(d[e] & 0xffff0000u)};
-      a2[e] = __builtin_elementwise_fma(ww, v2, a2[e]);
-    }
-  }
-#pragma unroll
-  for (int e = 0; e < 4; ++e) asm volatile("" : "+v"(a2[e]));
-}
 
 template <typename TV, typename TO, int L, typename TW = float>
 __global__ __launch_bounds__(256) __attribute__((amdgpu_waves_per_eu(4, 8))) void msda_fused_quad_kernel(const MsdaParams p) {
@@ -219,114 +127,11 @@
   const uint32_t lane_off = (uint32_t)((h * MS_D + sub * 8) * sizeof(TV));
   const uint32_t rowb = (uint32_t)(p.ldv * (int)sizeof(TV));
   constexpr int LP = L * MS_P;
-
   const TW* lg = reinterpret_cast<const TW*>(p.offw) + qg * p.ldoffw + MS_HEADS * LP * 2 + h * LP;
-  float wv[L];
-  float mx = -INFINITY;
-#pragma unroll
-  for (int l = 0; l < L; ++l) { wv[l] = ldf<TW>(lg + l * MS_P + sub); mx = fmaxf(mx, wv[l]); }
-  mx = fmaxf(mx, quad_xor1(mx));
-  mx = fmaxf(mx, quad_xor2(mx));
-  float sum = 0.f;
-#pragma unroll
-  for (int l = 0; l < L; ++l) { wv[l] = expf(wv[l] - mx); sum += wv[l]; }
-  sum += quad_xor1(sum);
-  sum += quad_xor2(sum);
-  const float inv = 1.f / sum;
-  const TW* of = reinterpret_cast<const TW*>(p.offw) + qg * p.ldoffw + h * LP * 2 + sub * 2;
+  const TW* of =reinterpret_cast<const TW*>(p.offw) + qg * p.ldoffw + h * LP * 2 + sub * 2;
   const float* rf = p.ref + qg * L * p.refdim;
-  float cw[L][4];
-  int ci[L][4];
-#pragma unroll
-  for (int l = 0; l < L; ++l) {
-    const int H = p.H[l], W = p.W[l];
-    float2 o;
-    if (sizeof(TW) == 4) {
-      o = *reinterpret_cast<const float2*>(of + l * 8);
-    } else {
-      typedef __attribute__((ext_vector_type(2))) _Float16 h2_t;
-      const h2_t t = *reinterpret_cast<const h2_t*>(of + l * 8);
-      o = make_float2((float)t[0], (float)t[1]);
-    }
-    const float rx = rf[l * p.refdim], ry = rf[l * p.refdim + 1];
-    float lx, ly;
-    if (p.refdim == 2) {
-      if (p.pow2) { lx = rx + o.x * p.invW[l]; ly = ry + o.y * p.invH[l]; }
-      else { lx = rx + o.x / (float)W; ly = ry + o.y / (float)H; }
-    } else {
-      const float rw = rf[l * p.refdim + 2], rh = rf[l * p.refdim + 3];
-      lx = rx + o.x / (float)MS_P * rw * 0.5f; ly = ry + o.y / (float)MS_P * rh * 0.5f;
-    }
-    const float aw = wv[l] * inv;
-    const float h_im = ly * (float)H - 0.5f, w_im = lx * (float)W - 0.5f;
-    const bool inside = h_im > -1.f && w_im > -1.f && h_im < (float)H && w_im < (float)W;
-    const float hf = floorf(h_im), wf = floorf(w_im);
-    const int h_low = (int)hf, w_low = (int)wf;
-    const int h_high = h_low + 1, w_high = w_low + 1;
-    const float lh = h_im - hf, lw = w_im - wf;
-    const float hh = 1.f - lh, hw = 1.f - lw;
-    const bool t_ok = inside && h_low >= 0, b_ok = inside && h_high <= H - 1;
-    const bool l_ok = w_low >= 0, r_ok = w_high <= W - 1;
-    const int base = p.start[l];
-    cw[l][0] = (t_ok && l_ok) ? aw * hh * hw : 0.f; ci[l][0] = (t_ok && l_ok) ? base + h_low * W + w_low : 0;
-    cw[l][1] = (t_ok && r_ok) ? aw * hh * lw : 0.f; ci[l][1] = (t_ok && r_ok) ? base + h_low * W + w_high : 0;
-    cw[l][2] = (b_ok && l_ok) ? aw * lh * hw : 0.f; ci[l][2] = (b_ok && l_ok) ? base + h_high * W + w_low : 0;
-    cw[l][3] = (b_ok && r_ok) ? aw * lh * lw : 0.f; ci[l][3] = (b_ok && r_ok) ? base + h_high * W + w_high : 0;
-    if (sizeof(TV) == 2) {
-#pragma unroll
-      for (int c = 0; c < 4; ++c) ci[l][c] = (int)__umul24((unsigned)ci[l][c], rowb);
-    }
-  }
   float acc[8];
-  if (std::is_same<TV, f16_t>::value) {
-#pragma unroll
-    for (int c = 0; c < 8; ++c) acc[c] = 0.f;
-    CornerGroup<TV> g0, g1;
-    group_load<TV, L>(vbase, lane_off, cw, ci, 0, g0);
-#pragma unroll
-    for (int s = 0; s < L * 4; s += 2) {
-      group_load<TV, L>(vbase, lane_off, cw, ci, s + 1, g1);
-      __builtin_amdgcn_sched_barrier(0);
-      group_fma_half<TV>(g0, acc);
-      __builtin_amdgcn_sched_barrier(0);
-      if (s + 2 < L * 4) group_load<TV, L>(vbase, lane_off, cw, ci, s + 2, g0);
-      __builtin_amdgcn_sched_barrier(0);
-      group_fma_half<TV>(g1, acc);
-      __builtin_amdgcn_sched_barrier(0);
-    }
-  } else if (sizeof(TV) == 2) {
-    f32x2_t a2[4];
-#pragma unroll
-    for (int e = 0; e < 4; ++e) a2[e] = (f32x2_t){0.f, 0.f};
-    CornerGroup<TV> g0, g1;
-    group_load<TV, L>(vbase, lane_off, cw, ci, 0, g0);
-#pragma unroll
-    for (int s = 0; s < L * 4; s += 2) {
-      group_load<TV, L>(vbase, lane_off, cw, ci, s + 1, g1);
-      __builtin_amdgcn_sched_barrier(0);
-      group_fma<TV>(g0, a2);
-      __builtin_amdgcn_sched_barrier(0);
-      if (s + 2 < L * 4) group_load<TV, L>(vbase, lane_off, cw, ci, s + 2, g0);
-      __builtin_amdgcn_sched_barrier(0);
-      group_fma<TV>(g1, a2);
-      __builtin_amdgcn_sched_barrier(0);
-    }
-#pragma unroll
-    for (int e = 0; e < 4; ++e) { acc[2 * e] = a2[e][0]; acc[2 * e + 1] = a2[e][1]; }
-  } else {
-#pragma unroll
-    for (int c = 0; c < 8; ++c) acc[c] = 0.f;
-#pragma unroll
-    for (int s = 0; s < L * 4; ++s) {
-      const int l = s >> 2, P = s & 3;
-#pragma unroll
-      for (int c = 0; c < 4; ++c) {
-        const float w = quad_pick_f(P, cw[l][c]);
-        const int idx = quad_pick_i(P, ci[l][c]);
-        if (w != 0.f) corner_acc<TV>(vb, p.ldv, idx, w, acc);
-      }
-    }
-  }
+  msda_quad_sample<TV, L, TW>(p, lg, of, rf, vb, vbase, lane_off, rowb, sub, acc);
   if (live) {
     TO* o = reinterpret_cast<TO*>(p.out) + qg * p.ldout + h * MS_D + sub * 8;
     st8<TO>(o, acc);
@@ -515,17 +320,6 @@
   return 0;
 }
 
-static int fill_levels(MsdaParams& p, const int64_t* shapes, const int64_t* starts, int L, int S) {
-  if (L < 1 || L > 5) { ape_set_error("msda: num_levels %d not in 1..5", L); return -1; }
-  int64_t tot = 0;
-  for (int l = 0; l < L; ++l) {
-    p.H[l] = (int)shapes[2 * l]; p.W[l] = (int)shapes[2 * l + 1]; p.start[l] = (int)starts[l];
-    if (p.H[l] <= 0 || p.W[l] <= 0 || starts[l] != tot) { ape_set_error("msda: inconsistent level %d (h=%d w=%d start=%lld)", l, p.H[l], p.W[l], (long long)starts[l]); return -1; }
-    tot += (int64_t)p.H[l] * p.W[l];
-  }
-  if (tot != S) { ape_set_error("msda: sum(h*w)=%lld != num_value=%d", (long long)tot, S); return -1; }
-  return 0;
-}
 
 extern "C" int ape_hip_ms_deform_attn_forward(const void* value, int ldv, const int64_t* spatial_shapes,
                                               const int64_t* level_start_index, const void* sampling_loc,
diff --git a/ape_amd/csrc/msda_sample.h b/ape_amd/csrc/msda_sample.h
--- /dev/null
+++ b/ape_amd/csrc/msda_sample.h
@@ -0,0 +1,220 @@
+#pragma once
+#include <type_traits>
+
+#include "common.h"
+
+#define MS_HEADS 8
+#define MS_D 32
+#define MS_P 4
+
+struct MsdaParams {
+  const void* value; int ldv;
+  const void* loc;
+  const void* attn;
+  const void* offw; int ldoffw;
+  int offw_f16;
+  const float* ref; int refdim;
+  void* out; int ldout;
+  int S, Q;
+  int H[8], W[8], start[8];
+  float invW[8], invH[8];
+  int pow2;
+};
+
+template <typename TV>
+__device__ __forceinline__ void corner_acc(const TV* __restrict__ vbase, int ldv, int idx, float wgt, float acc[8]) {
+  float v[8];
+  ld8<TV>(vbase + (size_t)idx * ldv, v);
+#pragma unroll
+  for (int c = 0; c < 8; ++c) acc[c] = fmaf(wgt, v[c], acc[c]);
+}
+
+template <int P> __device__ __forceinline__ float quad_bcast_f(float v) {
+  return __int_as_float(__builtin_amdgcn_mov_dpp(__float_as_int(v), P * 0x55, 0xf, 0xf, true));
+}
+template <int P> __device__ __forceinline__ int quad_bcast_i(int v) { return __builtin_amdgcn_mov_dpp(v, P * 0x55, 0xf, 0xf, true); }
+__device__ __forceinline__ float quad_xor1(float v) { return __int_as_float(__builtin_amdgcn_mov_dpp(__float_as_int(v), 0xB1, 0xf, 0xf, true)); }
+__device__ __forceinline__ float quad_xor2(float v) { return __int_as_float(__builtin_amdgcn_mov_dpp(__float_as_int(v), 0x4E, 0xf, 0xf, true)); }
+
+__device__ __forceinline__ float quad_pick_f(int P, float v) {
+  return P == 0 ? quad_bcast_f<0>(v) : (P == 1 ? quad_bcast_f<1>(v) : (P == 2 ? quad_bcast_f<2>(v) : quad_bcast_f<3>(v)));
+}
+__device__ __forceinline__ int quad_pick_i(int P, int v) {
+  return P == 0 ? quad_bcast_i<0>(v) : (P == 1 ? quad_bcast_i<1>(v) : (P == 2 ? quad_bcast_i<2>(v) : quad_bcast_i<3>(v)));
+}
+
+template <typename TV>
+struct CornerGroup {
+  uint4 raw[4];
+  float w[4];
+};
+
+template <typename TV, int L>
+__device__ __forceinline__ void group_load(const unsigned char* __restrict__ vbase, uint32_t lane_off, const float (&cw)[L][4],
+                                           const int (&ci)[L][4], int s, CornerGroup<TV>& g) {
+  const int l = s >> 2, P = s & 3;
+#pragma unroll
+  for (int c = 0; c < 4; ++c) {
+    g.w[c] = quad_pick_f(P, cw[l][c]);
+    uint32_t off = (uint32_t)quad_pick_i(P, ci[l][c]) + lane_off;
+    asm volatile("" : "+v"(off));
+    g.raw[c] = *reinterpret_cast<const uint4*>(vbase + (size_t)off);
+  }
+}
+
+__device__ __forceinline__ void fma_mix_lo(float& acc, uint32_t d, float w) {
+  asm volatile("v_fma_mix_f32 %0, %1, %2, %0 op_sel:[0,0,0] op_sel_hi:[1,0,0]" : "+v"(acc) : "v"(d), "v"(w));
+}
+__device__ __forceinline__ void fma_mix_hi(float& acc, uint32_t d, float w) {
+  asm volatile("v_fma_mix_f32 %0, %1, %2, %0 op_sel:[1,0,0] op_sel_hi:[1,0,0]" : "+v"(acc) : "v"(d), "v"(w));
+}
+template <typename TV>
+__device__ __forceinline__ void group_fma_half(const CornerGroup<TV>& g, float (&acc)[8]) {
+#pragma unroll
+  for (int c = 0; c < 4; ++c) {
+    const uint32_t d[4] = {g.raw[c].x, g.raw[c].y, g.raw[c].z, g.raw[c].w};
+#pragma unroll
+    for (int e = 0; e < 4; ++e) {
+      fma_mix_lo(acc[2 * e], d[e], g.w[c]);
+      fma_mix_hi(acc[2 * e + 1], d[e], g.w[c]);
+    }
+  }
+}
+
+template <typename TV>
+__device__ __forceinline__ void group_fma(const CornerGroup<TV>& g, f32x2_t (&a2)[4]) {
+#pragma unroll
+  for (int c = 0; c < 4; ++c) {
+    const f32x2_t ww = {g.w[c], g.w[c]};
+    const uint32_t d[4] = {g.raw[c].x, g.raw[c].y, g.raw[c].z, g.raw[c].w};
+#pragma unroll
+    for (int e = 0; e < 4; ++e) {
+      const f32x2_t v2 = {__uint_as_float(d[e] << 16), __uint_as_float(d[e] & 0xffff0000u)};
+      a2[e] = __builtin_elementwise_fma(ww, v2, a2[e]);
+    }
+  }
+#pragma unroll
+  for (int e = 0; e < 4; ++e) asm volatile("" : "+v"(a2[e]));
+}
+
+template <typename TV, int L, typename TW>
+__device__ __forceinline__ void msda_quad_sample(const MsdaParams& p, const TW* lg, const TW* of, const float* rf, const TV* vb,
+                                                 const unsigned char* vbase, uint32_t lane_off, uint32_t rowb, int sub, float (&acc)[8]) {
+  constexpr int LP = L * MS_P;
+
+  float wv[L];
+  float mx = -INFINITY;
+#pragma unroll
+  for (int l = 0; l < L; ++l) { wv[l] = ldf<TW>(lg + l * MS_P + sub); mx = fmaxf(mx, wv[l]); }
+  mx = fmaxf(mx, quad_xor1(mx));
+  mx = fmaxf(mx, quad_xor2(mx));
+  float sum = 0.f;
+#pragma unroll
+  for (int l = 0; l < L; ++l) { wv[l] = expf(wv[l] - mx); sum += wv[l]; }
+  sum += quad_xor1(sum);
+  sum += quad_xor2(sum);
+  const float inv = 1.f / sum;
+  float cw[L][4];
+  int ci[L][4];
+#pragma unroll
+  for (int l = 0; l < L; ++l) {
+    const int H = p.H[l], W = p.W[l];
+    float2 o;
+    if (sizeof(TW) == 4) {
+      o = *reinterpret_cast<const float2*>(of + l * 8);
+    } else {
+      typedef __attribute__((ext_vector_type(2))) _Float16 h2_t;
+      const h2_t t = *reinterpret_cast<const h2_t*>(of + l * 8);
+      o = make_float2((float)t[0], (float)t[1]);
+    }
+    const float rx = rf[l * p.refdim], ry = rf[l * p.refdim + 1];
+    float lx, ly;
+    if (p.refdim == 2) {
+      if (p.pow2) { lx = rx + o.x * p.invW[l]; ly = ry + o.y * p.invH[l]; }
+      else { lx = rx + o.x / (float)W; ly = ry + o.y / (float)H; }
+    } else {
+      const float rw = rf[l * p.refdim + 2], rh = rf[l * p.refdim + 3];
+      lx = rx + o.x / (float)MS_P * rw * 0.5f; ly = ry + o.y / (float)MS_P * rh * 0.5f;
+    }
+    const float aw = wv[l] * inv;
+    const float h_im = ly * (float)H - 0.5f, w_im = lx * (float)W - 0.5f;
+    const bool inside = h_im > -1.f && w_im > -1.f && h_im < (float)H && w_im < (float)W;
+    const float hf = floorf(h_im), wf = floorf(w_im);
+    const int h_low = (int)hf, w_low = (int)wf;
+    const int h_high = h_low + 1, w_high = w_low + 1;
+    const float lh = h_im - hf, lw = w_im - wf;
+    const float hh = 1.f - lh, hw = 1.f - lw;
+    const bool t_ok = inside && h_low >= 0, b_ok = inside && h_high <= H - 1;
+    const bool l_ok = w_low >= 0, r_ok = w_high <= W - 1;
+    const int base = p.start[l];
+    cw[l][0] = (t_ok && l_ok) ? aw * hh * hw : 0.f; ci[l][0] = (t_ok && l_ok) ? base + h_low * W + w_low : 0;
+    cw[l][1] = (t_ok && r_ok) ? aw * hh * lw : 0.f; ci[l][1] = (t_ok && r_ok) ? base + h_low * W + w_high : 0;
+    cw[l][2] = (b_ok && l_ok) ? aw * lh * hw : 0.f; ci[l][2] = (b_ok && l_ok) ? base + h_high * W + w_low : 0;
+    cw[l][3] = (b_ok && r_ok) ? aw * lh * lw : 0.f; ci[l][3] = (b_ok && r_ok) ? base + h_high * W + w_high : 0;
+    if (sizeof(TV) == 2) {
+#pragma unroll
+      for (int c = 0; c < 4; ++c) ci[l][c] = (int)__umul24((unsigned)ci[l][c], rowb);
+    }
+  }
+  if (std::is_same<TV, f16_t>::value) {
+#pragma unroll
+    for (int c = 0; c < 8; ++c) acc[c] = 0.f;
+    CornerGroup<TV> g0, g1;
+    group_load<TV, L>(vbase, lane_off, cw, ci, 0, g0);
+#pragma unroll
+    for (int s = 0; s < L * 4; s += 2) {
+      group_load<TV, L>(vbase, lane_off, cw, ci, s + 1, g1);
+      __builtin_amdgcn_sched_barrier(0);
+      group_fma_half<TV>(g0, acc);
+      __builtin_amdgcn_sched_barrier(0);
+      if (s + 2 < L * 4) group_load<TV, L>(vbase, lane_off, cw, ci, s + 2, g0);
+      __builtin_amdgcn_sched_barrier(0);
+      group_fma_half<TV>(g1, acc);
+      __builtin_amdgcn_sched_barrier(0);
+    }
+  } else if (sizeof(TV) == 2) {
+    f32x2_t a2[4];
+#pragma unroll
+    for (int e = 0; e < 4; ++e) a2[e] = (f32x2_t){0.f, 0.f};
+    CornerGroup<TV> g0, g1;
+    group_load<TV, L>(vbase, lane_off, cw, ci, 0, g0);
+#pragma unroll
+    for (int s = 0; s < L * 4; s += 2) {
+      group_load<TV, L>(vbase, lane_off, cw, ci, s + 1, g1);
+      __builtin_amdgcn_sched_barrier(0);
+      group_fma<TV>(g0, a2);
+      __builtin_amdgcn_sched_barrier(0);
+      if (s + 2 < L * 4) group_load<TV, L>(vbase, lane_off, cw, ci, s + 2, g0);
+      __builtin_amdgcn_sched_barrier(0);
+      group_fma<TV>(g1, a2);
+      __builtin_amdgcn_sched_barrier(0);
+    }
+#pragma unroll
+    for (int e = 0; e < 4; ++e) { acc[2 * e] = a2[e][0]; acc[2 * e + 1] = a2[e][1]; }
+  } else {
+#pragma unroll
+    for (int c = 0; c < 8; ++c) acc[c] = 0.f;
+#pragma unroll
+    for (int s = 0; s < L * 4; ++s) {
+      const int l = s >> 2, P = s & 3;
+#pragma unroll
+      for (int c = 0; c < 4; ++c) {
+        const float w = quad_pick_f(P, cw[l][c]);
+        const int idx = quad_pick_i(P, ci[l][c]);
+        if (w != 0.f) corner_acc<TV>(vb, p.ldv, idx, w, acc);
+      }
+    }
+  }
+}
+
+static int fill_levels(MsdaParams& p, const int64_t* shapes, const int64_t* starts, int L, int S) {
+  if (L < 1 || L > 5) { ape_set_error("msda: num_levels %d not in 1..5", L); return -1; }
+  int64_t tot = 0;
+  for (int l = 0; l < L; ++l) {
+    p.H[l] = (int)shapes[2 * l]; p.W[l] = (int)shapes[2 * l + 1]; p.start[l] = (int)starts[l];
+    if (p.H[l] <= 0 || p.W[l] <= 0 || starts[l] != tot) { ape_set_error("msda: inconsistent level %d (h=%d w=%d start=%lld)", l, p.H[l], p.W[l], (long long)starts[l]); return -1; }
+    tot += (int64_t)p.H[l] * p.W[l];
+  }
+  if (tot != S) { ape_set_error("msda: sum(h*w)=%lld != num_value=%d", (long long)tot, S); return -1; }
+  return 0;
+}
diff --git a/ape_amd/modeling/ape_deta/_containers.py b/ape_amd/modeling/ape_deta/_containers.py
--- a/ape_amd/modeling/ape_deta/_containers.py
+++ b/ape_amd/modeling/ape_deta/_containers.py
@@ -82,7 +82,7 @@
                         wo=pack_matrix(self.attn.out_proj.weight, dt), bo=f32(self.attn.out_proj.bias))
         return self._pack.get(self, dt, build)
 
-    def forward_tokens(self, x, x_pos, dt, vt_buf, out_dtype=None):
+    def forward_tokens(self, x, x_pos, dt, vt_buf, out_dtype=None, query_pos=None, norm=None):
         P = self.packed(dt)
         E, nh = self.embed_dim, self.num_heads
         hd = E // nh
@@ -90,6 +90,8 @@
         qk = ops.gemm(x_pos, P["wqk"], P["bqk"])
         vt = vjob.join()
         o = ops.attention(qk[:, :E], qk[:, E:], vt, batch=1, n=x.shape[0], heads=nh, head_dim=hd, scale=hd ** -0.5)
+        if norm is not None:
+            return ops.dec_attn_out(o, x, query_pos, P["wo"], P["bo"], norm)
         return ops.gemm(o, P["wo"], P["bo"], residual=x, out_dtype=out_dtype or dt)
 
 
diff --git a/ape_amd/modeling/ape_deta/deformable_transformer_vl.py b/ape_amd/modeling/ape_deta/deformable_transformer_vl.py
--- a/ape_amd/modeling/ape_deta/deformable_transformer_vl.py
+++ b/ape_amd/modeling/ape_deta/deformable_transformer_vl.py
@@ -91,9 +91,13 @@
         inter, inter_ref = [], []
         _, ref_in = ops.box_refine(None, reference.contiguous(), vr4)
         refjob = ops._Joined((reference, ref_in))
+        fused = ops.decoder_fusable(query, self.layers[0].ffns[0].layers[0][0].out_features, len(geo.shapes))
         for i, layer in enumerate(self.layers):
-            x1 = layer.attentions[0].forward_tokens(out, outp, dt, vt_buf)
-            x2, x2p = ops.layernorm(x1, *layer.norm_params(0), out_dtype=dt, add=query_pos)
+            if fused:
+                x2, x2p = layer.attentions[0].forward_tokens(out, outp, dt, vt_buf, query_pos=query_pos, norm=layer.norm_params(0))
+            else:
+                x1 = layer.attentions[0].forward_tokens(out, outp, dt, vt_buf)
+                x2, x2p = ops.layernorm(x1, *layer.norm_params(0), out_dtype=dt, add=query_pos)
             reference, ref_in = refjob.join()
             if i > 0:
                 if stages is not None:
@@ -102,21 +106,31 @@
                         reference = forced
                         _, ref_in = ops.box_refine(None, reference.contiguous(), vr4)
                 inter_ref.append(reference)
-            x3 = layer.attentions[1].forward_tokens(x2p, x2, ref_in, geo.shapes, geo.starts, dt,
-                                                    value=value_all[:, i * E:(i + 1) * E])
-            x4 = ops.layernorm(x3, *layer.norm_params(1), out_dtype=dt)
-            x5 = layer.ffns[0].forward_tokens(x4, dt)
-            out, outp = ops.layernorm(x5, *layer.norm_params(2), out_dtype=dt, add=query_pos)
+            if fused:
+                PA, PF = layer.attentions[1].packed(dt), layer.ffns[0].packed(dt)
+                out, outp = ops.dec_cross_ffn(x2p, x2, query_pos, value_all[:, i * E:(i + 1) * E], geo.shapes, geo.starts, ref_in,
+                                              PA["woffw"], PA["boffw"], PA["wout"], PA["bout"], layer.norm_params(1),
+                                              PF["w1"], PF["b1"], PF["w2"], PF["b2"], layer.norm_params(2))
+            else:
+                x3 = layer.attentions[1].forward_tokens(x2p, x2, ref_in, geo.shapes, geo.starts, dt,
+                                                        value=value_all[:, i * E:(i + 1) * E])
+                x4 = ops.layernorm(x3, *layer.norm_params(1), out_dtype=dt)
+                x5 = layer.ffns[0].forward_tokens(x4, dt)
+                out, outp = ops.layernorm(x5, *layer.norm_params(2), out_dtype=dt, add=query_pos)
             if stages is not None:
                 forced = tap(stages, f"dec{i}_out", out)
                 if forced is not out:
                     out, outp = forced, (forced.float() + query_pos.float()).to(dt)
             if self.bbox_embed is not None:
                 def refine(i=i, out=out, reference=reference):
-                    tmp = self.bbox_embed[i].forward_tokens(out, dt, out_dtype=torch.float32)
+                    if fused:
+                        tmp, new_ref, new_ref_in = ops.dec_box(out, self.bbox_embed[i].packed(dt), reference.contiguous(), vr4)
+                    else:
+                        tmp = self.bbox_embed[i].forward_tokens(out, dt, out_dtype=torch.float32)
+                        new_ref, new_ref_in = ops.box_refine(tmp, reference, vr4)
                     if stages is not None:
                         stages[f"dec{i}_delta"] = tmp
-                    return ops.box_refine(tmp, reference, vr4)
+                    return new_ref, new_ref_in
                 refjob = ops.fork(refine)
             inter.append(out)
         reference, _ = refjob.join()
diff --git a/ape_amd/ops.py b/ape_amd/ops.py
--- a/ape_amd/ops.py
+++ b/ape_amd/ops.py
@@ -1114,3 +1114,82 @@
                                       float(norm[2]) if norm is not None else 0.0, _stream())
     _lib.check(rc, "ape_hip_ffn_fused")
     return out
+
+
+_DEC_FUSED = os.environ.get("APE_DEC_FUSED", "1") != "0"
+
+
+def decoder_fusable(x, ffn_dim, levels):
+    return (_DEC_FUSED and x.is_cuda and x.dtype in HALF16 and x.dim() == 2 and x.shape[1] == 256 and x.shape[0] >= 1
+            and 64 <= ffn_dim <= 2048 and ffn_dim % 64 == 0 and 1 <= levels <= 5)
+
+
+def _h16rows(t, name, dt, cols=256):
+    _rowmajor(t, name)
+    if t.dtype != dt or t.shape[1] < cols:
+        raise TypeError(f"ape_amd.ops: {name} must be a {dt} tensor with >= {cols} columns, got {t.dtype} {tuple(t.shape)}")
+    return t
+
+
+def dec_attn_out(o, x, query_pos, wo, bo, norm):
+    dt = x.dtype
+    _dev(o, x, query_pos, wo, bo, norm[0], norm[1])
+    for t, n in ((o, "o"), (x, "x"), (query_pos, "query_pos"), (wo, "wo")):
+        _h16rows(t, n, dt)
+    Q = x.shape[0]
+    x2 = torch.empty((Q, 256), dtype=dt, device=x.device)
+    x2p = torch.empty((Q, 256), dtype=dt, device=x.device)
+    rc = _lib.load().ape_hip_dec_attn_out(_p(o), _ld(o), _p(x), _ld(x), _p(query_pos), _ld(query_pos), _p(wo), _ld(wo), _p(_f32vec(bo, "bo")),
+                                          _p(_f32vec(norm[0], "norm weight")), _p(_f32vec(norm[1], "norm bias")), float(norm[2]),
+                                          _p(x2), _p(x2p), 256, Q, _dt(x), _stream())
+    _lib.check(rc, "ape_hip_dec_attn_out")
+    return x2, x2p
+
+
+def dec_cross_ffn(x2p, x2, query_pos, value, spatial_shapes, level_start_index, ref_in, woffw, boffw, wout, bout, norm1, w1, b1, w2, b2,
+                  norm2):
+    dt = x2.dtype
+    _dev(x2p, x2, query_pos, value, ref_in, woffw, boffw, wout, bout, w1, b1, w2, b2)
+    for t, n in ((x2p, "x2p"), (x2, "x2"), (query_pos, "query_pos"), (woffw, "woffw"), (wout, "wout"), (w1, "w1")):
+        _h16rows(t, n, dt)
+    F = w1.shape[0]
+    _h16rows(w2, "w2", dt, F)
+    _rowmajor(value, "value")
+    shp, st, L = _levels(spatial_shapes, level_start_index)
+    Q, S = x2.shape[0], value.shape[0]
+    if ref_in.dtype != torch.float32 or not ref_in.is_contiguous() or tuple(ref_in.shape) != (Q, L, 4):
+        raise TypeError("ape_amd.ops.dec_cross_ffn: ref_in must be contiguous float32 [Q, L, 4]")
+    if woffw.shape[0] < 96 * L or boffw.numel() < 96 * L or wout.shape[0] != 256 or w2.shape[0] != 256:
+        raise ValueError("ape_amd.ops.dec_cross_ffn: weight shapes")
+    out = torch.empty((Q, 256), dtype=dt, device=x2.device)
+    outp = torch.empty((Q, 256), dtype=dt, device=x2.device)
+    rc = _lib.load().ape_hip_dec_cross_ffn(
+        _p(x2p), _ld(x2p), _p(x2), _ld(x2), _p(query_pos), _ld(query_pos), _p(value), _ld(value), _dt(value), shp, st, L, S, _p(ref_in),
+        _p(woffw), _ld(woffw), _p(_f32vec(boffw, "boffw")), _p(wout), _ld(wout), _p(_f32vec(bout, "bout")),
+        _p(_f32vec(norm1[0], "norm1 weight")), _p(_f32vec(norm1[1], "norm1 bias")), float(norm1[2]),
+        _p(w1), _ld(w1), _p(_f32vec(b1, "b1")), _p(w2), _ld(w2), _p(_f32vec(b2, "b2")), F,
+        _p(_f32vec(norm2[0], "norm2 weight")), _p(_f32vec(norm2[1], "norm2 bias")), float(norm2[2]),
+        _p(out), _p(outp), 256, Q, _dt(x2), _stream())
+    _lib.check(rc, "ape_hip_dec_cross_ffn")
+    return out, outp
+
+
+def dec_box(x, layers, ref, vr4, eps=1e-3):
+    dt = x.dtype
+    (w1, b1), (w2, b2), (w3, b3) = layers
+    _dev(x, w1, b1, w2, b2, w3, b3, ref, vr4)
+    for t, n in ((x, "x"), (w1, "w1"), (w2, "w2"), (w3, "w3")):
+        _h16rows(t, n, dt)
+    if w1.shape[0] != 256 or w2.shape[0] != 256 or w3.shape[0] != 4:
+        raise ValueError("ape_amd.ops.dec_box: a 256 -> 256 -> 256 -> 4 MLP")
+    if ref.dtype != torch.float32 or vr4.dtype != torch.float32 or not ref.is_contiguous() or not vr4.is_contiguous():
+        raise TypeError("ape_amd.ops.dec_box: ref / vr4 must be contiguous float32")
+    Q, L = x.shape[0], vr4.shape[0]
+    delta = torch.empty((Q, 4), dtype=torch.float32, device=x.device)
+    new_ref = torch.empty((Q, 4), dtype=torch.float32, device=x.device)
+    ref_in = torch.empty((Q, L, 4), dtype=torch.float32, device=x.device)
+    rc = _lib.load().ape_hip_dec_box(_p(x), _ld(x), _p(w1), _ld(w1), _p(_f32vec(b1, "b1")), _p(w2), _ld(w2), _p(_f32vec(b2, "b2")),
+                                     _p(w3), _ld(w3), _p(_f32vec(b3, "b3")), _p(ref), _p(vr4), L, float(eps), _p(delta), _p(new_ref),
+                                     _p(ref_in), Q, _dt(x), _stream())
+    _lib.check(rc, "ape_hip_dec_box")
+    return delta, new_ref, ref_in
diff --git a/include/ape_hip.h b/include/ape_hip.h
--- a/include/ape_hip.h
+++ b/include/ape_hip.h
@@ -241,6 +241,19 @@
                       const void* residual, int ldr, void* Y, int ldy, int M, int K, int HID, int N, int w2_permuted, int dt,
                       const float* ln_weight, const float* ln_bias, float ln_eps, void* stream);
 
+int ape_hip_dec_attn_out(const void* o, int ldo, const void* x, int ldx, const void* qpos, int ldqpos, const void* wo, int ldwo,
+                         const float* bo, const float* ln_w, const float* ln_b, float ln_eps, void* x2, void* x2p, int ldy, int Q,
+                         int dt, void* stream);
+int ape_hip_dec_cross_ffn(const void* x2p, int ldx2p, const void* x2, int ldx2, const void* qpos, int ldqpos, const void* value, int ldv,
+                          int v_dt, const int64_t* spatial_shapes, const int64_t* level_start_index, int L, int S, const float* ref_in,
+                          const void* woffw, int ldwoffw, const float* boffw, const void* wout, int ldwout, const float* bout,
+                          const float* ln1_w, const float* ln1_b, float ln1_eps, const void* w1, int ldw1, const float* b1,
+                          const void* w2, int ldw2, const float* b2, int F, const float* ln2_w, const float* ln2_b, float ln2_eps,
+                          void* out, void* outp, int ldout, int Q, int dt, void* stream);
+int ape_hip_dec_box(const void* x, int ldx, const void* w1, int ldw1, const float* b1, const void* w2, int ldw2, const float* b2,
+                    const void* w3, int ldw3, const float* b3, const float* ref, const float* vr4, int L, float eps, float* delta,
+                    float* new_ref, float* ref_in, int Q, int dt, void* stream);
+
 #ifdef __cplusplus
 }
 #endif
```

Result: no change. 114.8 (-0.5%).
